# a1q123456/image_stitching

Hardware: AMD Instinct MI355X
Metric: 4K frames stitched/sec (higher is better)
Workload: dtype u8

## Files before the change

### host/job.cpp

```cpp
#include "job.hpp"
#include <cstring>

namespace mis {

StitchJob::StitchJob(int device, int width, int height, const std::vector<CameraParams>& cameras, const StitchConfig& cfg)
    : JobCore("mis::StitchJob", "", device, nullptr, width, height, cameras, cfg) {}

StitchJob::~StitchJob() {
    mis_image_free(cctx_, &pano_);
    mis_image_free(cctx_, &mask_);
}

void StitchJob::finalize() {
    if (pano_.data && (pano_.width != key_.pano.width || pano_.height != key_.pano.height)) { mis_image_free(cctx_, &pano_); mis_image_free(cctx_, &mask_); pano_ = MisImage{}; mask_ = MisImage{}; }
    if (!pano_.data) { pano_ = MisImage{}; mask_ = MisImage{}; pano_.mem = mask_.mem = MIS_MEM_DEVICE; }
    check(cctx_, mis_blender_blend(blender_, &pano_, &mask_), "mis_blender_blend");
}

JobOutput StitchJob::run(const std::vector<MisImage>& frames) {
    if ((int)frames.size() != n_) throw std::runtime_error("StitchJob::run: one frame per camera");
    JobOutput out;
    check(cctx_, mis_context_wait(cctx_, ctx_), "mis_context_wait");
    const MisImage* work = work_frames(frames);
    prep_.arm([this] { if (spec_ok_) prepare(everyone_); });
    check(ctx_, mis_orb_on_enqueued(orb_, &Hook::fire, &prep_), "mis_orb_on_enqueued");
    std::vector<MisFeatures> feats(n_);
    std::memset(feats.data(), 0, sizeof(MisFeatures) * n_);
    const int rc_f = mis_orb_detect_batch(orb_, work, n_, feats.data());
    mis_orb_on_enqueued(orb_, nullptr, nullptr);
    check(ctx_, rc_f, "mis_orb_detect_batch");
    prep_.finish();
    for (int i = 0; i < n_; i++) { feats[i].img_idx = i; out.num_features.push_back(feats[i].n); }
    const MisMatchParams mp = reset_matches();
    match_.arm([this, &frames] {
        if (!spec_ok_) return;
        fence_knn();
        compose(frames, everyone_, everyone_);
        finalize();
    });
    check(ctx_, mis_match_on_enqueued(ctx_, &Hook::fire, &match_), "mis_match_on_enqueued");
    const int rc = mis_match_pairs_model(ctx_, feats.data(), n_, &mp, model_, nullptr, cfg_.range_width, 0, 1, pairwise_.data());
    mis_match_on_enqueued(ctx_, nullptr, nullptr);
    for (auto& f : feats) mis_features_free(ctx_, &f);
    check(ctx_, rc, "mis_match_pairs_model");
    match_.finish();
    out.confidence.resize((size_t)n_ * n_);
    for (int k = 0; k < n_ * n_; k++) out.confidence[k] = pairwise_[k].confidence;
    std::vector<int> idx(n_);
    int kept = 0;
    check(ctx_, mis_leave_biggest_component(pairwise_.data(), n_, cfg_.conf_thresh, idx.data(), &kept), "mis_leave_biggest_component");
    idx.resize(kept);
    if (kept < 2) throw std::runtime_error("Need more images");
    out.indices = idx;
    out.speculation_kept = spec_ok_ && kept == n_;
    if (!out.speculation_kept) {
        prepare(idx);
        compose(frames, everyone_, idx);
        finalize();
    }
    check(cctx_, mis_context_synchronize(cctx_), "mis_context_synchronize (compose)");
    out.pano = pano_; out.mask = mask_;
    out.num_bands = key_.bands; out.pano_width = key_.pano.width; out.pano_height = key_.pano.height;
    out.matches = pairwise_;
    return out;
}

}
```

### host/job_core.cpp

```cpp
#include "job_core.hpp"
#include <algorithm>
#include <numeric>

namespace mis {

static float median_focal(const std::vector<CameraParams>& cams, const std::vector<int>& idx) {
    std::vector<double> f;
    for (int i : idx) f.push_back(cams[i].focal);
    std::sort(f.begin(), f.end());
    return f.size() % 2 == 1 ? static_cast<float>(f[f.size() / 2]) : static_cast<float>(f[f.size() / 2 - 1] + f[f.size() / 2]) * 0.5f;
}

void JobCore::Hook::fire(void* self_) {
    Hook* self = static_cast<Hook*>(self_);
    self->ran_ = true;
    try { self->body_(); } catch (const std::exception& e) { self->error_ = e.what(); }
}

void JobCore::Hook::arm(std::function<void()> body) {
    body_ = std::move(body);
    ran_ = false;
    error_.clear();
}

void JobCore::Hook::finish() {
    if (!ran_) fire(this);
    if (!error_.empty()) throw std::runtime_error(error_);
}

void JobCore::check(MisContext* c, int rc, const char* what) const {
    if (rc != MIS_OK) throw std::runtime_error(std::string(what) + " failed" + where_ + ": " + mis_last_error(c));
}

JobCore::JobCore(const char* who, std::string where, int device, void* main_stream, int width, int height, const std::vector<CameraParams>& cameras,
                 const StitchConfig& cfg)
    : w_(width), h_(height), n_((int)cameras.size()), wg_(work_geometry(cfg, width, height)), cams_(cameras), cfg_(cfg), everyone_(n_), mstream_(main_stream),
      where_(std::move(where)) {
    std::iota(everyone_.begin(), everyone_.end(), 0);
    if (wg_.scale != 1.0) {
        for (auto& c : cams_) { c.focal *= wg_.scale; c.ppx *= wg_.scale; c.ppy *= wg_.scale; }
        compose_work_aspect_ = 1.0 / wg_.scale;
    }
    try {
        if (cfg_.features_type != "orb" || cfg_.ba_cost_func != "no" || cfg_.expos_comp_type != "no" || cfg_.seam_find_type != "no")
            throw std::runtime_error(std::string(who) + " runs the hot path (ORB, supplied cameras, no seam-scale step); use mis::Stitcher for the other options");
        kind_ = warp_kind(cfg_.warp_type);
        check_range_width(cfg_.range_width);
        model_ = matcher_model(cfg_.matcher_type, cfg_.range_width);
        if (mis_context_create(device, mstream_, &ctx_) != MIS_OK) throw std::runtime_error("mis_context_create failed: no HIP device (there is no CPU fallback)");
        check(ctx_, mis_stream_create(device, 0, &cstream_), "mis_stream_create");
        if (mis_context_create(device, cstream_, &cctx_) != MIS_OK) throw std::runtime_error("mis_context_create (compose stream) failed");
        MisOrbParams op;
        mis_orb_default_params(&op);
        check(ctx_, mis_orb_create(ctx_, &op, wg_.width, wg_.height, &orb_), "mis_orb_create");
    } catch (...) {
        release();
        throw;
    }
    Ks_.resize((size_t)n_ * 9); Rs_.resize((size_t)n_ * 9);
    for (int i = 0; i < n_; i++) {
        CameraParams cc = cams_[i];
        if (compose_work_aspect_ != 1.0) { cc.focal *= compose_work_aspect_; cc.ppx *= compose_work_aspect_; cc.ppy *= compose_work_aspect_; }
        const Mat3<float> K = cc.K().cast<float>(), R = cams_[i].R.cast<float>();
        std::copy(K.m.begin(), K.m.end(), Ks_.begin() + 9 * i);
        std::copy(R.m.begin(), R.m.end(), Rs_.begin() + 9 * i);
    }
    if (kind_ != MIS_WARP_SPHERICAL) {
        const float scale = warp_scale(everyone_);
        MisRect r;
        if (MIS_WARP_ROI_IS_FULL_SCAN(kind_)) {
            std::vector<MisRect> rr((size_t)n_);
            spec_ok_ = n_ == 0 || mis_warper_roi_batch(cctx_, kind_, scale, w_, h_, n_, Ks_.data(), Rs_.data(), rr.data()) == MIS_OK;
        } else
            for (int i = 0; i < n_ && spec_ok_; i++) spec_ok_ = mis_warper_roi(kind_, scale, w_, h_, &Ks_[9 * i], &Rs_[9 * i], &r) == MIS_OK;
    }
}

JobCore::~JobCore() { release(); }

float JobCore::warp_scale(const std::vector<int>& idx) const {
    const float scale = median_focal(cams_, idx);
    return compose_work_aspect_ != 1.0 ? scale * static_cast<float>(compose_work_aspect_) : scale;
}

const MisImage* JobCore::work_frames(const std::vector<MisImage>& frames) {
    if (wg_.scale == 1.0 || frames.empty()) return frames.data();
    if (work_.size() < frames.size()) work_.resize(frames.size(), MisImage{});
    check(ctx_, mis_resize_linear_exact_batch(ctx_, frames.data(), (int)frames.size(), 0, 0, wg_.scale, wg_.scale, work_.data()), "mis_resize_linear_exact_batch");
    return work_.data();
}

void JobCore::release() {
    if (cctx_) mis_context_synchronize(cctx_);
    if (ctx_) mis_context_synchronize(ctx_);
    if (!pairwise_.empty()) mis_matches_free(pairwise_.data(), (int)pairwise_.size());
    if (ctx_) for (auto& im : work_) mis_image_free(ctx_, &im);
    if (blender_) mis_blender_destroy(blender_);
    if (orb_) mis_orb_destroy(orb_);
    if (cctx_) mis_context_destroy(cctx_);
    if (ctx_) mis_context_destroy(ctx_);
    if (cstream_) mis_stream_destroy(cstream_);
    if (mstream_) mis_stream_destroy(mstream_);
}

void JobCore::synchronize() {
    check(ctx_, mis_context_synchronize(ctx_), "mis_context_synchronize");
    check(cctx_, mis_context_synchronize(cctx_), "mis_context_synchronize (compose)");
}

JobCore::Compose JobCore::prepare(const std::vector<int>& idx) {
    const int m = (int)idx.size();
    const float scale = warp_scale(idx);
    std::vector<float> Ks((size_t)m * 9), Rs((size_t)m * 9);
    for (int k = 0; k < m; k++) {
        std::copy(Ks_.begin() + 9 * idx[k], Ks_.begin() + 9 * idx[k] + 9, Ks.begin() + 9 * k);
        std::copy(Rs_.begin() + 9 * idx[k], Rs_.begin() + 9 * idx[k] + 9, Rs.begin() + 9 * k);
    }
    rois_.assign(m, MisRect{});
    check(cctx_, mis_warper_roi_batch(cctx_, kind_, scale, w_, h_, m, Ks.data(), Rs.data(), rois_.data()), "mis_warper_roi_batch");
    std::vector<MisPoint> corners(m);
    std::vector<MisSize> sizes(m);
    for (int k = 0; k < m; k++) { corners[k] = {rois_[k].x, rois_[k].y}; sizes[k] = {rois_[k].width, rois_[k].height}; }
    Compose c;
    check(cctx_, mis_result_roi(corners.data(), sizes.data(), m, &c.pano), "mis_result_roi");
    check(cctx_, mis_blend_config(cfg_.blend_type, cfg_.blend_strength, c.pano.width, c.pano.height, &c.type, &c.bands, &c.sharp), "mis_blend_config");
    if (!blender_ || c.type != key_.type || c.bands != key_.bands || c.sharp != key_.sharp) {
        if (blender_) { mis_blender_destroy(blender_); blender_ = nullptr; }
        check(cctx_, mis_blender_create(cctx_, c.type, c.bands, c.sharp, &blender_), "mis_blender_create");
    }
    key_ = c;
    check(cctx_, mis_blender_prepare(blender_, corners.data(), sizes.data(), m), "mis_blender_prepare");
    return c;
}

void JobCore::fence_knn() {
    const int rc = mis_match_knn_fence(ctx_, cstream_, mis_match_sequence(ctx_), 0);
    if (rc < 0) check(ctx_, rc, "mis_match_knn_fence");
}

void JobCore::compose(const std::vector<MisImage>& frames, const std::vector<int>& frame_ids, const std::vector<int>& idx) {
    std::vector<MisImage> fr;
    std::vector<float> Ks, Rs;
    std::vector<MisRect> rois;
    for (size_t q = 0; q < frame_ids.size(); q++) {
        const auto it = std::find(idx.begin(), idx.end(), frame_ids[q]);
        if (it == idx.end()) continue;
        fr.push_back(frames[q]);
        Ks.insert(Ks.end(), Ks_.begin() + 9 * frame_ids[q], Ks_.begin() + 9 * frame_ids[q] + 9);
        Rs.insert(Rs.end(), Rs_.begin() + 9 * frame_ids[q], Rs_.begin() + 9 * frame_ids[q] + 9);
        rois.push_back(rois_[it - idx.begin()]);
    }
    if (fr.empty()) return;
    check(cctx_, mis_compose_frames_kind(blender_, kind_, fr.data(), (int)fr.size(), warp_scale(idx), Ks.data(), Rs.data(), rois.data()),
          "mis_compose_frames_kind");
}

MisMatchParams JobCore::reset_matches() {
    if (!pairwise_.empty()) { mis_matches_free(pairwise_.data(), (int)pairwise_.size()); pairwise_.clear(); }
    pairwise_.assign((size_t)n_ * n_, MisMatchesInfo{});
    return match_params(model_, cfg_.match_conf);
}

}
```

### host/job_core.hpp

```cpp
#pragma once
#include <functional>
#include <string>
#include <vector>
#include "stitcher.hpp"

namespace mis {

struct JobOutput {
    std::vector<int> indices;
    std::vector<double> confidence;
    std::vector<int> num_features;
    MisImage pano{}, mask{};
    int num_bands = 0, pano_width = 0, pano_height = 0;
    bool speculation_kept = false;
    std::vector<MisMatchesInfo> matches;
};

class JobCore {
protected:
    struct Compose { int type = 0, bands = 0; float sharp = 0; MisRect pano{}; };

    class Hook {
    public:
        static void fire(void* self);
        void arm(std::function<void()> body);
        void finish();
    private:
        std::function<void()> body_;
        bool ran_ = false;
        std::string error_;
    };

    JobCore(const char* who, std::string where, int device, void* main_stream, int width, int height, const std::vector<CameraParams>& cameras,
            const StitchConfig& cfg);
    ~JobCore();
    JobCore(const JobCore&) = delete;
    JobCore& operator=(const JobCore&) = delete;

    void check(MisContext* c, int rc, const char* what) const;
    void synchronize();
    Compose prepare(const std::vector<int>& idx);
    void fence_knn();
    const MisImage* work_frames(const std::vector<MisImage>& frames);
    float warp_scale(const std::vector<int>& idx) const;
    void compose(const std::vector<MisImage>& frames, const std::vector<int>& frame_ids, const std::vector<int>& idx);
    MisMatchParams reset_matches();

    int w_, h_, n_;
    WorkGeometry wg_;
    double compose_work_aspect_ = 1;
    std::vector<CameraParams> cams_;
    std::vector<MisImage> work_;
    StitchConfig cfg_;
    std::vector<int> everyone_;
    int kind_ = MIS_WARP_SPHERICAL;
    int model_ = MIS_MATCH_HOMOGRAPHY;
    bool spec_ok_ = true;
    void* mstream_ = nullptr;
    void* cstream_ = nullptr;
    MisContext* ctx_ = nullptr;
    MisContext* cctx_ = nullptr;
    MisOrb* orb_ = nullptr;
    MisBlender* blender_ = nullptr;
    Compose key_{};
    std::vector<float> Ks_, Rs_;
    std::vector<MisRect> rois_;
    std::vector<MisMatchesInfo> pairwise_;

private:
    void release();
    std::string where_;
};

}
```

### host/sharded_job.cpp

```cpp
#include "sharded_job.hpp"
#include <hip/hip_runtime_api.h>
#include <algorithm>
#include <cstring>
#include <numeric>

namespace mis {

std::vector<int> frame_block(int n, int rank, int world) {
    const int base = n / world, rem = n % world;
    const int lo = rank * base + std::min(rank, rem), cnt = base + (rank < rem ? 1 : 0);
    std::vector<int> out(cnt);
    std::iota(out.begin(), out.end(), lo);
    return out;
}

void* ShardedJob::reserve(DevBuf& b, size_t bytes) {
    bytes = std::max<size_t>(bytes, 256);
    if (b.bytes < bytes) {
        if (b.p) (void)hipFree(b.p);
        b.p = nullptr; b.bytes = 0;
        if (hipMalloc(&b.p, bytes) != hipSuccess) throw std::runtime_error("hipMalloc of an exchange buffer failed");
        b.bytes = bytes;
    }
    return b.p;
}

static void* new_stream(int device) {
    void* s = nullptr;
    if (mis_stream_create(device, 0, &s) != MIS_OK) throw std::runtime_error("mis_stream_create failed: no HIP device (there is no CPU fallback)");
    return s;
}

ShardedJob::ShardedJob(int device, int width, int height, const std::vector<CameraParams>& cameras, Communicator& comm, const StitchConfig& cfg)
    : JobCore("mis::ShardedJob", " on rank " + std::to_string(comm.rank()), device, new_stream(device), width, height, cameras, cfg), comm_(comm) {
    if (n_ % comm_.world() != 0) throw std::runtime_error("the frame count must divide evenly over the ranks");
    mine_ = frame_block(n_, comm_.rank(), comm_.world());
    send_.resize(comm_.world()); recv_.resize(comm_.world());
}

ShardedJob::~ShardedJob() {
    for (DevBuf* b : {&kps_send_, &desc_send_, &kps_all_, &desc_all_, &strip_mine_, &strips_all_, &pano_buf_, &mask_buf_}) if (b->p) (void)hipFree(b->p);
    for (auto& b : send_) if (b.p) (void)hipFree(b.p);
    for (auto& b : recv_) if (b.p) (void)hipFree(b.p);
}

void ShardedJob::prepare_multi_band(const std::vector<int>& idx) {
    if (prepare(idx).type != MIS_BLEND_MULTI_BAND) throw std::runtime_error("mis::ShardedJob exchanges the multi-band blender's pyramids");
}

void ShardedJob::exchange_finalize(const std::vector<int>& idx) {
    const int world = comm_.world(), me = comm_.rank(), bands = key_.bands;
    std::vector<int> lw(bands + 1), lh(bands + 1);
    for (int l = 0; l <= bands; l++) check(cctx_, mis_blender_level_info(blender_, l, &lw[l], &lh[l], nullptr, nullptr), "mis_blender_level_info");
    const int w0 = lw[0], h0 = lh[0];
    const int q = 1 << bands, nq = w0 / q;
    std::vector<std::pair<int, int>> bounds(world);
    for (int k = 0; k < world; k++) bounds[k] = {(int)((long long)k * nq / world) * q, k + 1 < world ? (int)((long long)(k + 1) * nq / world) * q : w0};
    std::vector<std::vector<std::pair<int, int>>> need(world);
    for (int k = 0; k < world; k++) {
        int lo = bounds[k].first, hi = bounds[k].second;
        need[k].push_back({lo, hi});
        for (int l = 1; l <= bands; l++) { lo = std::max(0, (lo >> 1) - 1); hi = std::min(lw[l], ((hi - 1) >> 1) + 2); need[k].push_back({lo, hi}); }
    }
    int px = 1 << 30, py = 1 << 30;
    for (size_t k = 0; k < idx.size(); k++) { px = std::min(px, rois_[k].x); py = std::min(py, rois_[k].y); }
    struct Region { bool any; int x0, y0, x1, y1; };
    std::vector<Region> region(world);
    const int gap = 3 << bands, a = q - 1;
    for (int r = 0; r < world; r++) {
        Region g{false, 1 << 30, 1 << 30, -(1 << 30), -(1 << 30)};
        for (int i : frame_block(n_, r, world)) {
            const auto it = std::find(idx.begin(), idx.end(), i);
            if (it == idx.end()) continue;
            const MisRect& rc = rois_[it - idx.begin()];
            g.any = true;
            g.x0 = std::min(g.x0, rc.x); g.y0 = std::min(g.y0, rc.y); g.x1 = std::max(g.x1, rc.x + rc.width); g.y1 = std::max(g.y1, rc.y + rc.height);
        }
        if (g.any) {
            g.x0 = std::max(0, g.x0 - px - gap) & ~a; g.y0 = std::max(0, g.y0 - py - gap) & ~a;
            g.x1 = std::min(w0, (g.x1 - px + gap + a) & ~a); g.y1 = std::min(h0, (g.y1 - py + gap + a) & ~a);
        }
        region[r] = g;
    }
    auto rects_of = [&](int src, int dst, std::vector<MisLevelRect>& out) -> size_t {
        out.clear();
        size_t off = 0;
        const Region& g = region[src];
        if (!g.any) return 0;
        for (int l = 0; l <= bands; l++) {
            const int x0 = std::max(std::min(g.x0 >> l, lw[l]), need[dst][l].first), x1 = std::min(std::min(-((-g.x1) >> l), lw[l]), need[dst][l].second);
            const int y0 = std::min(g.y0 >> l, lh[l]), y1 = std::min(-((-g.y1) >> l), lh[l]);
            if (x1 <= x0 || y1 <= y0) continue;
            const size_t m = (size_t)(x1 - x0) * (y1 - y0);
            out.push_back(MisLevelRect{l, x0, y0, x1, y1, (unsigned long long)off});
            off += (m * 6 + 15) / 16 * 16 + (m * 4 + 15) / 16 * 16;
        }
        return off;
    };
    std::vector<MisLevelRect> rects;
    std::vector<const void*> sp(world);
    std::vector<void*> rp(world);
    std::vector<size_t> sb(world), rb(world);
    for (int k = 0; k < world; k++) {
        sb[k] = rects_of(me, k, rects);
        sp[k] = reserve(send_[k], sb[k]);
        if (!rects.empty()) check(cctx_, mis_blender_pack_rects(blender_, rects.data(), (int)rects.size(), send_[k].p, send_[k].bytes), "mis_blender_pack_rects");
        rb[k] = rects_of(k, me, rects);
        rp[k] = reserve(recv_[k], rb[k]);
    }
    comm_.all_to_all(sp.data(), sb.data(), rp.data(), rb.data(), cstream_);
    std::vector<MisLevelRect> full;
    for (int l = 0; l <= bands; l++)
        if (need[me][l].second > need[me][l].first) full.push_back(MisLevelRect{l, need[me][l].first, 0, need[me][l].second, lh[l], 0ull});
    if (!full.empty()) check(cctx_, mis_blender_zero_rects(blender_, full.data(), (int)full.size()), "mis_blender_zero_rects");
    for (int r = 0; r < world; r++) {
        rects_of(r, me, rects);
        if (!rects.empty()) check(cctx_, mis_blender_add_rects(blender_, rects.data(), (int)rects.size(), recv_[r].p, recv_[r].bytes), "mis_blender_add_rects");
    }
    const int pw = key_.pano.width, ph = key_.pano.height;
    int cap_w = 0;
    for (int k = 0; k < world; k++) cap_w = std::max(cap_w, std::min(bounds[k].second, pw) - bounds[k].first);
    cap_w = std::max(cap_w, 1);
    const size_t strip_bytes = (size_t)ph * cap_w * 7;
    uint8_t* mine = (uint8_t*)reserve(strip_mine_, strip_bytes);
    const int x0 = bounds[me].first, x1 = std::min(bounds[me].second, pw);
    if (x1 > x0) {
        MisImage img{mine, x1 - x0, ph, 3, (size_t)cap_w * 6, MIS_S16, MIS_MEM_DEVICE};
        MisImage msk{mine + (size_t)ph * cap_w * 6, x1 - x0, ph, 1, (size_t)cap_w, MIS_U8, MIS_MEM_DEVICE};
        check(cctx_, mis_blender_blend_columns(blender_, x0, x1, &img, &msk), "mis_blender_blend_columns");
    }
    uint8_t* all = (uint8_t*)reserve(strips_all_, strip_bytes * world);
    comm_.all_gather(mine, all, strip_bytes, cstream_);
    uint8_t* pano = (uint8_t*)reserve(pano_buf_, (size_t)ph * pw * 6);
    uint8_t* mask = (uint8_t*)reserve(mask_buf_, (size_t)ph * pw);
    for (int k = 0; k < world; k++) {
        const int b0 = bounds[k].first, b1 = std::min(bounds[k].second, pw);
        if (b1 <= b0) continue;
        const uint8_t* base = all + (size_t)k * strip_bytes;
        check(cctx_, mis_copy_2d(cctx_, pano + (size_t)b0 * 6, (size_t)pw * 6, base, (size_t)cap_w * 6, (size_t)(b1 - b0) * 6, ph), "mis_copy_2d");
        check(cctx_, mis_copy_2d(cctx_, mask + b0, (size_t)pw, base + (size_t)ph * cap_w * 6, (size_t)cap_w, (size_t)(b1 - b0), ph), "mis_copy_2d");
    }
    pano_ = MisImage{pano, pw, ph, 3, (size_t)pw * 6, MIS_S16, MIS_MEM_DEVICE};
    mask_ = MisImage{mask, pw, ph, 1, (size_t)pw, MIS_U8, MIS_MEM_DEVICE};
}

JobOutput ShardedJob::run(const std::vector<MisImage>& frames) {
    const int m = (int)mine_.size(), world = comm_.world();
    if ((int)frames.size() != m) throw std::runtime_error("ShardedJob::run: one frame per camera of this rank's block");
    JobOutput out;
    check(cctx_, mis_context_wait(cctx_, ctx_), "mis_context_wait");
    const MisImage* work = work_frames(frames);
    prep_.arm([this] { if (spec_ok_) prepare_multi_band(everyone_); });
    check(ctx_, mis_orb_on_enqueued(orb_, &Hook::fire, &prep_), "mis_orb_on_enqueued");
    std::vector<MisFeatures> local(m);
    std::memset(local.data(), 0, sizeof(MisFeatures) * m);
    const int rc_f = m > 0 ? mis_orb_detect_batch(orb_, work, m, local.data()) : MIS_OK;
    mis_orb_on_enqueued(orb_, nullptr, nullptr);
    check(ctx_, rc_f, "mis_orb_detect_batch");
    prep_.finish();
    std::vector<int> cnt_mine(m), cnt_all(n_);
    for (int k = 0; k < m; k++) cnt_mine[k] = local[k].n;
    comm_.all_gather_host(cnt_mine.data(), cnt_all.data(), sizeof(int) * m);
    const int cap = std::max(1, *std::max_element(cnt_all.begin(), cnt_all.end()));
    const size_t kb = (size_t)cap * sizeof(MisKeyPoint), db = (size_t)cap * 32;
    reserve(kps_send_, kb * m); reserve(desc_send_, db * m); reserve(kps_all_, kb * n_); reserve(desc_all_, db * n_);
    if (m > 0) check(ctx_, mis_features_pack(ctx_, local.data(), m, cap, 32, kps_send_.p, desc_send_.p), "mis_features_pack");
    comm_.all_gather(kps_send_.p, kps_all_.p, kb * m, mstream_);
    comm_.all_gather(desc_send_.p, desc_all_.p, db * m, mstream_);
    std::vector<MisFeatures> feats(n_);
    for (int i = 0; i < n_; i++) {
        MisFeatures& f = feats[i];
        f.img_idx = i; f.img_w = wg_.width; f.img_h = wg_.height; f.n = cnt_all[i];
        f.keypoints = reinterpret_cast<MisKeyPoint*>((uint8_t*)kps_all_.p + kb * i);
        f.descriptors = (uint8_t*)desc_all_.p + db * i;
        f.desc_cols = 32; f.desc_dtype = MIS_U8; f.owner_ = nullptr;
    }
    out.num_features = cnt_all;
    const MisMatchParams mp = reset_matches();
    match_.arm([this, &frames] {
        if (!spec_ok_) return;
        fence_knn();
        compose(frames, mine_, everyone_);
    });
    check(ctx_, mis_match_on_enqueued(ctx_, &Hook::fire, &match_), "mis_match_on_enqueued");
    const int rc = mis_match_pairs_model(ctx_, feats.data(), n_, &mp, model_, nullptr, cfg_.range_width, comm_.rank(), world, pairwise_.data());
    mis_match_on_enqueued(ctx_, nullptr, nullptr);
    for (auto& f : local) mis_features_free(ctx_, &f);
    check(ctx_, rc, "mis_match_pairs_model");
    match_.finish();
    out.confidence.resize((size_t)n_ * n_);
    for (int k = 0; k < n_ * n_; k++) out.confidence[k] = pairwise_[k].confidence;
    comm_.all_reduce_sum_host(out.confidence.data(), out.confidence.size());
    std::vector<int> idx(n_);
    int kept = 0;
    check(ctx_, mis_leave_biggest_component_conf(out.confidence.data(), n_, cfg_.conf_thresh, idx.data(), &kept), "mis_leave_biggest_component_conf");
    idx.resize(kept);
    if (kept < 2) throw std::runtime_error("Need more images");
    out.indices = idx;
    out.speculation_kept = spec_ok_ && kept == n_;
    if (!out.speculation_kept) {
        prepare_multi_band(idx);
        compose(frames, mine_, idx);
    }
    exchange_finalize(idx);
    check(cctx_, mis_context_synchronize(cctx_), "mis_context_synchronize (compose)");
    out.pano = pano_; out.mask = mask_;
    out.num_bands = key_.bands; out.pano_width = key_.pano.width; out.pano_height = key_.pano.height;
    return out;
}

}
```

### image_stitching_amd/_capi.py

```python
import ctypes as C
import os
import re

_HERE = os.path.dirname(os.path.abspath(__file__))
LIB_PATH = os.path.join(_HERE, "libmistitch.so")
HEADER_PATH = os.path.join(os.path.dirname(_HERE), "include", "mistitch.h")

MIS_OK = 0
MIS_FENCE_TIMEOUT = 1
MEM_HOST, MEM_DEVICE = 0, 1
U8, S16, F32 = 0, 1, 2
INTER_NEAREST, INTER_LINEAR = 0, 1
BORDER_CONSTANT, BORDER_REFLECT = 0, 2
BLEND_NO, BLEND_FEATHER, BLEND_MULTI_BAND = 0, 1, 2
WARP_SPHERICAL, WARP_CYLINDRICAL, WARP_PLANE, WARP_MERCATOR, WARP_FISHEYE, WARP_STEREOGRAPHIC = 0, 1, 2, 3, 4, 5


def roi_is_full_scan(kind):
    return WARP_MERCATOR <= kind <= WARP_STEREOGRAPHIC


MATH_LOG, MATH_TAN, MATH_SINH, MATH_ASIN, MATH_ATAN, MATH_EXP = 0, 1, 2, 3, 4, 5
MATCH_HOMOGRAPHY, MATCH_AFFINE_PARTIAL = 0, 1
EXPOS_NO, EXPOS_GAIN, EXPOS_GAIN_BLOCKS, EXPOS_CHANNELS, EXPOS_CHANNELS_BLOCKS = 0, 1, 2, 3, 4


class MisPoint(C.Structure):
    _fields_ = [("x", C.c_int), ("y", C.c_int)]


class MisSize(C.Structure):
    _fields_ = [("width", C.c_int), ("height", C.c_int)]


class MisRect(C.Structure):
    _fields_ = [("x", C.c_int), ("y", C.c_int), ("width", C.c_int), ("height", C.c_int)]


class MisLevelRect(C.Structure):
    _fields_ = [("level", C.c_int), ("x0", C.c_int), ("y0", C.c_int), ("x1", C.c_int), ("y1", C.c_int), ("offset", C.c_ulonglong)]


class MisImage(C.Structure):
    _fields_ = [("data", C.c_void_p), ("width", C.c_int), ("height", C.c_int), ("channels", C.c_int),
                ("stride", C.c_size_t), ("dtype", C.c_int), ("mem", C.c_int)]


class MisKeyPoint(C.Structure):
    _fields_ = [("x", C.c_float), ("y", C.c_float), ("size", C.c_float), ("angle", C.c_float),
                ("response", C.c_float), ("octave", C.c_int)]


class MisOrbParams(C.Structure):
    _fields_ = [("nfeatures", C.c_int), ("scale_factor", C.c_float), ("nlevels", C.c_int),
                ("edge_threshold", C.c_int), ("first_level", C.c_int), ("wta_k", C.c_int),
                ("score_type", C.c_int), ("patch_size", C.c_int), ("fast_threshold", C.c_int)]


class MisSiftParams(C.Structure):
    _fields_ = [("nfeatures", C.c_int), ("n_octave_layers", C.c_int), ("contrast_threshold", C.c_double),
                ("edge_threshold", C.c_double), ("sigma", C.c_double)]


class MisCameraParams(C.Structure):
    _fields_ = [("focal", C.c_double), ("aspect", C.c_double), ("ppx", C.c_double), ("ppy", C.c_double), ("R", C.c_double * 9),
                ("t", C.c_double * 3)]


class MisFeatures(C.Structure):
    _fields_ = [("img_idx", C.c_int), ("img_w", C.c_int), ("img_h", C.c_int), ("n", C.c_int),
                ("keypoints", C.c_void_p), ("descriptors", C.c_void_p), ("desc_cols", C.c_int),
                ("desc_dtype", C.c_int), ("owner_", C.c_void_p)]


class MisMatchParams(C.Structure):
    _fields_ = [("match_conf", C.c_float), ("num_matches_thresh1", C.c_int), ("num_matches_thresh2", C.c_int),
                ("ransac_thresh", C.c_double), ("max_iters", C.c_int), ("confidence", C.c_double)]


class MisCompensatorParams(C.Structure):
    _fields_ = [("type", C.c_int), ("nr_feeds", C.c_int), ("block_width", C.c_int), ("block_height", C.c_int),
                ("nr_gain_filtering_iterations", C.c_int)]


class MisDMatch(C.Structure):
    _fields_ = [("query_idx", C.c_int), ("train_idx", C.c_int), ("img_idx", C.c_int), ("distance", C.c_float)]


class MisMatchesInfo(C.Structure):
    _fields_ = [("src_img_idx", C.c_int), ("dst_img_idx", C.c_int), ("n_matches", C.c_int),
                ("matches", C.POINTER(MisDMatch)), ("inliers_mask", C.POINTER(C.c_uint8)), ("num_inliers", C.c_int),
                ("has_H", C.c_int), ("H", C.c_double * 9), ("confidence", C.c_double)]


_vp, _i, _f, _d = C.c_void_p, C.c_int, C.c_float, C.c_double
_P = C.POINTER

PROTOTYPES = {
    "mis_context_create": (_i, [_i, _vp, _P(_vp)]),
    "mis_stream_create": (_i, [_i, _i, _P(_vp)]),
    "mis_stream_destroy": (_i, [_vp]),
    "mis_context_destroy": (_i, [_vp]),
    "mis_context_synchronize": (_i, [_vp]),
    "mis_context_wait": (_i, [_vp, _vp]),
    "mis_last_error": (C.c_char_p, [_vp]),
    "mis_version": (C.c_char_p, []),
    "mis_image_free": (_i, [_vp, _P(MisImage)]),
    "mis_orb_default_params": (None, [_P(MisOrbParams)]),
    "mis_orb_create": (_i, [_vp, _P(MisOrbParams), _i, _i, _P(_vp)]),
    "mis_orb_destroy": (_i, [_vp]),
    "mis_orb_detect": (_i, [_vp, _P(MisImage), _P(MisFeatures)]),
    "mis_orb_detect_batch": (_i, [_vp, _P(MisImage), _i, _P(MisFeatures)]),
    "mis_orb_on_enqueued": (_i, [_vp, _vp, _vp]),
    "mis_features_download": (_i, [_vp, _P(MisFeatures), _vp, _vp]),
    "mis_features_upload": (_i, [_vp, _i, _i, _i, _vp, _vp, _i, _i, _P(MisFeatures)]),
    "mis_features_free": (_i, [_vp, _P(MisFeatures)]),
    "mis_orb_debug_level": (_i, [_vp, _i, _i, _vp, _P(_i), _P(_i)]),
    "mis_sift_default_params": (None, [_P(MisSiftParams)]),
    "mis_sift_create": (_i, [_vp, _P(MisSiftParams), _i, _i, _P(_vp)]),
    "mis_sift_destroy": (_i, [_vp]),
    "mis_sift_detect": (_i, [_vp, _P(MisImage), _P(MisFeatures)]),
    "mis_sift_detect_batch": (_i, [_vp, _P(MisImage), _i, _P(MisFeatures)]),
    "mis_sift_debug_level": (_i, [_vp, _P(MisImage), _i, _i, _i, _vp, _P(_i), _P(_i)]),
    "mis_sift_debug_counts": (_i, [_vp, _P(C.c_uint)]),
    "mis_match_default_params": (None, [_P(MisMatchParams)]),
    "mis_match_all_pairs": (_i, [_vp, _P(MisFeatures), _i, _P(MisMatchParams), _P(MisMatchesInfo)]),
    "mis_match_pairs_sharded": (_i, [_vp, _P(MisFeatures), _i, _P(MisMatchParams), _i, _i, _P(MisMatchesInfo)]),
    "mis_match_pairs_select": (_i, [_vp, _P(MisFeatures), _i, _P(MisMatchParams), _vp, _i, _i, _i, _P(MisMatchesInfo)]),
    "mis_match_affine_default_params": (None, [_P(MisMatchParams)]),
    "mis_match_pairs_model": (_i, [_vp, _P(MisFeatures), _i, _P(MisMatchParams), _i, _vp, _i, _i, _i, _P(MisMatchesInfo)]),
    "mis_estimate_affine_partial": (_i, [_vp, _vp, _vp, _i, _d, _i, _d, _i, _vp, _vp, _P(_i)]),
    "mis_matches_free": (_i, [_P(MisMatchesInfo), _i]),
    "mis_match_sequence": (C.c_longlong, [_vp]),
    "mis_match_knn_fence": (_i, [_vp, _vp, C.c_longlong, _i]),
    "mis_match_on_enqueued": (_i, [_vp, _vp, _vp]),
    "mis_knn2": (_i, [_vp, _P(MisFeatures), _P(MisFeatures), _vp, _vp]),
    "mis_find_homography": (_i, [_vp, _vp, _vp, _i, _d, _i, _d, _vp, _vp, _P(_i)]),
    "mis_leave_biggest_component": (_i, [_P(MisMatchesInfo), _i, _f, _vp, _P(_i)]),
    "mis_leave_biggest_component_conf": (_i, [_vp, _i, _f, _vp, _P(_i)]),
    "mis_bundle_adjust_reproj": (_i, [_vp, _P(MisFeatures), _P(MisMatchesInfo), _i, _f, C.c_char_p, _P(MisCameraParams)]),
    "mis_wave_correct": (_i, [_vp, _i, _i]),
    "mis_warp_roi": (_i, [_f, _i, _i, _vp, _vp, _P(MisRect)]),
    "mis_warp_spherical": (_i, [_vp, _P(MisImage), _f, _vp, _vp, _i, _i, _P(MisImage), _P(MisPoint)]),
    "mis_warp_roi_batch": (_i, [_vp, _f, _i, _i, _i, _vp, _vp, _P(MisRect)]),
    "mis_warp_spherical_fused_roi": (_i, [_vp, _P(MisImage), _f, _vp, _vp, _P(MisRect), _P(MisImage), _P(MisImage), _P(MisPoint)]),
    "mis_warp_spherical_fused_batch": (_i, [_vp, _P(MisImage), _i, C.c_float, _P(C.c_float), _P(C.c_float), _P(MisRect), _P(MisImage), _P(MisImage), _P(MisPoint)]),
    "mis_warp_spherical_fused_batch_timed": (_i, [_vp, _P(MisImage), _i, C.c_float, _P(C.c_float), _P(C.c_float), _P(MisRect), _P(MisImage), _P(MisImage), _P(MisPoint), _i,
                                               _P(C.c_float)]),
    "mis_debug_math_f32": (_i, [_vp, _i, _vp, _vp, _i]),
    "mis_warper_roi": (_i, [_i, _f, _i, _i, _vp, _vp, _P(MisRect)]),
    "mis_warper_roi_batch": (_i, [_vp, _i, _f, _i, _i, _i, _vp, _vp, _P(MisRect)]),
    "mis_warper_warp": (_i, [_vp, _i, _P(MisImage), _f, _vp, _vp, _i, _i, _P(MisImage), _P(MisPoint)]),
    "mis_warper_warp_roi": (_i, [_vp, _i, _P(MisImage), _f, _vp, _vp, _P(MisRect), _i, _i, _P(MisImage), _P(MisPoint)]),
    "mis_warper_warp_fused": (_i, [_vp, _i, _P(MisImage), _f, _vp, _vp, _P(MisImage), _P(MisImage), _P(MisPoint)]),
    "mis_warper_warp_fused_roi": (_i, [_vp, _i, _P(MisImage), _f, _vp, _vp, _P(MisRect), _P(MisImage), _P(MisImage), _P(MisPoint)]),
    "mis_warper_warp_fused_batch": (_i, [_vp, _i, _P(MisImage), _i, C.c_float, _P(C.c_float), _P(C.c_float), _P(MisRect), _P(MisImage), _P(MisImage), _P(MisPoint)]),
    "mis_warp_spherical_fused": (_i, [_vp, _P(MisImage), _f, _vp, _vp, _P(MisImage), _P(MisImage), _P(MisPoint)]),
    "mis_resize_linear_exact": (_i, [_vp, _P(MisImage), _i, _i, C.c_double, C.c_double, _P(MisImage)]),
    "mis_resize_linear_exact_batch": (_i, [_vp, _P(MisImage), _i, _i, _i, C.c_double, C.c_double, _P(MisImage)]),
    "mis_rotate": (_i, [_vp, _P(MisImage), _i, _P(MisImage)]),
    "mis_seam_mask_apply": (_i, [_vp, _P(MisImage), _P(MisImage)]),
    "mis_compensator_create": (_i, [_vp, _i, _i, _i, _P(_vp)]),
    "mis_compensator_default_params": (None, [_P(MisCompensatorParams)]),
    "mis_compensator_create_ex": (_i, [_vp, _P(MisCompensatorParams), _P(_vp)]),
    "mis_compensator_destroy": (_i, [_vp]),
    "mis_compensator_gains": (_i, [_vp, _i, _P(_d)]),
    "mis_compensator_gain_map_channels": (_i, [_vp, _i, _P(C.c_float), _i, _P(_i), _P(_i), _P(_i)]),
    "mis_compensator_debug_stats": (_i, [_vp, _i, _i, _i, _P(_i), _P(_d), _P(_d)]),
    "mis_compensator_feed": (_i, [_vp, _P(MisPoint), _P(MisImage), _P(MisImage), _i]),
    "mis_compensator_gain_map": (_i, [_vp, _i, _P(C.c_float), _i, _P(_i), _P(_i)]),
    "mis_compensator_apply": (_i, [_vp, _i, _P(MisImage)]),
    "mis_seam_voronoi": (_i, [_vp, _P(MisPoint), _P(MisImage), _i]),
    "mis_seam_dp": (_i, [_vp, _P(MisPoint), _P(MisImage), _P(MisImage), _i, _i]),
    "mis_warp_spherical_fused_timed": (_i, [_vp, _P(MisImage), _f, _vp, _vp, _P(MisImage), _P(MisImage), _P(MisPoint), _i, _P(C.c_float)]),
    "mis_blend_config": (_i, [_i, _f, _i, _i, _P(_i), _P(_i), _P(_f)]),
    "mis_result_roi": (_i, [_P(MisPoint), _P(MisSize), _i, _P(MisRect)]),
    "mis_blender_create": (_i, [_vp, _i, _i, _f, _P(_vp)]),
    "mis_blender_destroy": (_i, [_vp]),
    "mis_blender_prepare": (_i, [_vp, _P(MisPoint), _P(MisSize), _i]),
    "mis_blender_num_bands": (_i, [_vp]),
    "mis_blender_feed": (_i, [_vp, _P(MisImage), _P(MisImage), MisPoint]),
    "mis_blender_feed_batch": (_i, [_vp, _P(MisImage), _P(MisImage), _P(MisPoint), _i]),
    "mis_blender_blend": (_i, [_vp, _P(MisImage), _P(MisImage)]),
    "mis_compose_frames": (_i, [_vp, _P(MisImage), _i, _f, _vp, _vp, _P(MisRect)]),
    "mis_compose_frames_kind": (_i, [_vp, _i, _P(MisImage), _i, _f, _vp, _vp, _P(MisRect)]),
    "mis_blender_blend_columns": (_i, [_vp, _i, _i, _P(MisImage), _P(MisImage)]),
    "mis_blender_pack_rects": (_i, [_vp, _P(MisLevelRect), _i, _vp, C.c_size_t]),
    "mis_blender_add_rects": (_i, [_vp, _P(MisLevelRect), _i, _vp, C.c_size_t]),
    "mis_blender_zero_rects": (_i, [_vp, _P(MisLevelRect), _i]),
    "mis_features_pack": (_i, [_vp, _P(MisFeatures), _i, _i, _i, _vp, _vp]),
    "mis_copy_2d": (_i, [_vp, _vp, C.c_size_t, _vp, C.c_size_t, C.c_size_t, C.c_size_t]),
    "mis_blender_feed_rect": (_i, [_vp, _i, _i, MisPoint, _P(MisRect)]),
    "mis_blender_level_info": (_i, [_vp, _i, _P(_i), _P(_i), _P(_vp), _P(_vp)]),
}


def header_functions():
    txt = open(HEADER_PATH).read()
    txt = re.sub(r"/\*.*?\*/", "", txt, flags=re.S)
    return sorted(set(re.findall(r"\b(mis_[a-z0-9_]+)\s*\(", txt)))


_lib = None


def load():
    global _lib
    if _lib is not None:
        return _lib
    if not os.path.exists(LIB_PATH):
        raise ImportError("libmistitch.so is not built (%s missing): run `python -c 'import __graft_entry__ as g; g.build()'` "
                          "or `make -C image_stitching_amd/csrc`; there is no CPU fallback" % LIB_PATH)
    lib = C.CDLL(LIB_PATH)
    for name, (res, args) in PROTOTYPES.items():
        fn = getattr(lib, name)
        fn.restype = res
        fn.argtypes = args
    _lib = lib
    return lib
```

### image_stitching_amd/csrc/blend.hip

```cpp
#include "common.h"
#include "dev_math.h"
#include <algorithm>
#include <cmath>
#include <utility>
#include <vector>

#define MIS_MAX_BANDS 16

struct MisBlender {
    MisContext* ctx = nullptr;
    int type = MIS_BLEND_MULTI_BAND, actual_bands = 5, num_bands = 0;
    float sharpness = 0.02f;
    MisRect roi{0, 0, 0, 0};
    int fw = 0, fh = 0;
    int lw[MIS_MAX_BANDS + 1], lh[MIS_MAX_BANDS + 1];
    int16_t* lap[MIS_MAX_BANDS + 1];
    float* wgt[MIS_MAX_BANDS + 1];
    uint8_t* dst_mask = nullptr;
    void* pano_mem = nullptr;
    size_t pano_bytes = 0;
    bool prepared = false;
    bool fresh = false;
    void* scratch = nullptr;
    size_t scratch_bytes = 0;
};

namespace {

constexpr float WEIGHT_EPS = 1e-5f;
#ifndef FEED_TAIL_PIXELS_N
#define FEED_TAIL_PIXELS_N 8192
#endif
constexpr size_t FEED_TAIL_PIXELS = FEED_TAIL_PIXELS_N;

__device__ __forceinline__ int16_t sat_s16(int v) { return (int16_t)(v < -32768 ? -32768 : (v > 32767 ? 32767 : v)); }

struct FrameView {
    const int16_t* img;
    size_t istride;
    const uint8_t* mask;
    size_t mstride;
    int w, h;
    int left, top;
    int tw, th;
};

__device__ __forceinline__ int reflect101_near(int p, int len) {
    if ((unsigned)(p + len - 1) < (unsigned)(3 * len - 2)) { const int a = p < 0 ? -p : p; return a >= len ? 2 * len - 2 - a : a; }
    return mis_reflect101(p, len);
}
__device__ __forceinline__ int reflect_near(int p, int len) {
    if ((unsigned)(p + len) < (unsigned)(3 * len)) return mis_reflect1(p, len);
    return mis_reflect(p, len);
}

__device__ __forceinline__ void view_px(const FrameView& v, int tx, int ty, int* c) {
    const int16_t* p = v.img + (size_t)reflect_near(ty - v.top, v.h) * v.istride + 3 * (size_t)reflect_near(tx - v.left, v.w);
    c[0] = p[0]; c[1] = p[1]; c[2] = p[2];
}
__device__ __forceinline__ float view_w(const FrameView& v, int tx, int ty) {
    int x = tx - v.left, y = ty - v.top;
    if ((unsigned)x >= (unsigned)v.w || (unsigned)y >= (unsigned)v.h) return 0.f;
    return (float)v.mask[(size_t)y * v.mstride + x] * (float)(1. / 255.);
}

template <bool OK>
__device__ __forceinline__ void load_px3_t(const int16_t* __restrict__ row, int p, int* c) {
    if (OK) {
        const int e = 3 * p;
        const uint2 d = *reinterpret_cast<const uint2*>(row + (e & ~1));
        const unsigned sh = (unsigned)(e & 1) << 4;
        const unsigned lo = __builtin_amdgcn_alignbit(d.y, d.x, sh);
        c[0] = (int)(int16_t)(unsigned short)lo; c[1] = (int)lo >> 16; c[2] = (int)(int16_t)(unsigned short)(d.y >> sh);
    } else {
        c[0] = row[3 * p]; c[1] = row[3 * p + 1]; c[2] = row[3 * p + 2];
    }
}
__device__ __forceinline__ void load_px3(const int16_t* __restrict__ row, int p, bool ok, int* c) {
    if (ok) load_px3_t<true>(row, p, c); else load_px3_t<false>(row, p, c);
}

constexpr int PD_W = 32, PD_H = 16, PD_SW = 2 * PD_W + 3, PD_SH = 2 * PD_H + 3;

constexpr int PDV_ROW_DW = 104;
static_assert(PDV_ROW_DW * 2 >= 7 + 3 * PD_SW && PDV_ROW_DW % 4 == 0, "an LDS row holds the footprint from any 16-byte phase");
constexpr int PDV_MROW_B = 96;
constexpr int PDV_MROW_DW = (PD_SW + 3 + 3) / 4 + 1;
__device__ __forceinline__ void pd_dma16(const void* base, unsigned voff, uint32_t lds_off) {
    asm volatile("s_mov_b32 m0, %2\n\ts_nop 0\n\tglobal_load_lds_dwordx4 %0, %1" ::"v"(voff), "s"(base), "s"(lds_off) : "memory", "m0");
}

template <bool FROM_VIEW>
__device__ __forceinline__ void pyr_down_view_tile(const FrameView& v, const int16_t* __restrict__ src, const float* __restrict__ wsrc, int psw, int psh,
                                                   int16_t* __restrict__ dst, float* __restrict__ wdst, int dw, int dh, int bx, int by) {
    constexpr int WT_BYTES = (int)sizeof(float) * PD_SH * PD_SW;
    static_assert(WT_BYTES <= (int)sizeof(int16_t) * PD_SH * PDV_ROW_DW * 2, "the weights fit the spent image tile");
    __shared__ __attribute__((aligned(16))) int16_t tile[PD_SH * PDV_ROW_DW * 2];
    __shared__ __attribute__((aligned(16))) uint8_t wmem[FROM_VIEW ? PD_SH * PDV_MROW_B : WT_BYTES];
    __shared__ int vbuf[PD_H * PDV_ROW_DW];
    __shared__ int sflag;
    uint8_t* const mraw = wmem;
    float* const wt = FROM_VIEW ? reinterpret_cast<float*>(tile) : reinterpret_cast<float*>(wmem);
    int moff = 0;
    bool rowchk = false;
    unsigned wide_bits = 0;
    int wconst = 0;
    const int x0 = bx * PD_W, y0 = by * PD_H, t = threadIdx.x;
    const int sw = FROM_VIEW ? v.tw : psw, sh = FROM_VIEW ? v.th : psh;
    const int tx0 = 2 * x0 - 2, ty0 = 2 * y0 - 2;
    const int ix0 = tx0 - v.left, iy0 = ty0 - v.top;
    const bool interior = FROM_VIEW && tx0 >= 0 && ty0 >= 0 && tx0 + PD_SW <= sw && ty0 + PD_SH <= sh && ix0 >= 0 && iy0 >= 0 && ix0 + PD_SW + 12 <= v.w && iy0 + PD_SH <= v.h &&
                          (v.istride & 1) == 0 && ((uintptr_t)v.img & 3) == 0 && (v.mstride & 3) == 0 && ((uintptr_t)v.mask & 3) == 0;
    int toff;
    bool dma = false, mir = false;
    int cs = ix0;
    if (FROM_VIEW && tx0 >= 0 && ty0 >= 0 && tx0 + PD_SW <= sw && ty0 + PD_SH <= sh) {
        bool cols = true;
        if (ix0 >= 0 && ix0 + PD_SW <= v.w) cs = ix0;
        else if (ix0 + PD_SW <= 0 && -ix0 <= v.w) { cs = -ix0 - PD_SW; mir = true; }
        else if (ix0 >= v.w && 2 * v.w - PD_SW - ix0 >= 0) { cs = 2 * v.w - PD_SW - ix0; mir = true; }
        else cols = false;
        const size_t ia = ((size_t)3 * cs * 2) & ~(size_t)15, ma = (size_t)cs & ~(size_t)15;
        dma = cols && (((uintptr_t)v.img | (v.istride * 2)) & 15) == 0 && ia + PDV_ROW_DW * 4 <= v.istride * 2 && (size_t)v.h * v.istride * 2 < (1ull << 32) &&
              (mir || ((((uintptr_t)v.mask | v.mstride) & 15) == 0 && ma + PDV_MROW_B <= v.mstride && (size_t)v.h * v.mstride < (1ull << 32)));
        if (!dma) mir = false;
    }
    if (dma) {
        const size_t ib = (size_t)3 * cs * 2, ia = ib & ~(size_t)15;
        toff = (int)((ib - ia) >> 1);
        moff = cs & 15;
        rowchk = true;
        const uint8_t* ibase = reinterpret_cast<const uint8_t*>(v.img) + ia;
        const uint8_t* mbase = v.mask + ((size_t)cs & ~(size_t)15);
        const uint32_t tile_lds = (uint32_t)(uintptr_t)(__attribute__((address_space(3))) void*)tile;
        const uint32_t mraw_lds = (uint32_t)(uintptr_t)(__attribute__((address_space(3))) void*)mraw;
        const int wave = __builtin_amdgcn_readfirstlane(t >> 6), lane = t & 63;
        constexpr int IPR = PDV_ROW_DW / 4, IP = PD_SH * IPR, MPR = PDV_MROW_B / 16, MP = PD_SH * MPR;
#pragma unroll
        for (int k = 0; k < (IP + 255) / 256; k++) {
            const int p0 = (k * 4 + wave) * 64, p = p0 + lane;
            if (p0 < IP) {
                const int r = min(p / IPR, PD_SH - 1), c = p - r * IPR;
                const int iy = reflect_near(iy0 + r, v.h);
                if (p < IP) pd_dma16(ibase, (unsigned)iy * (unsigned)(v.istride * 2) + (unsigned)c * 16u, tile_lds + (uint32_t)p0 * 16u);
            }
        }
        if (!mir) {
            const int p0 = wave * 64, p = p0 + lane;
            if (p0 < MP) {
                const int r = min(p / MPR, PD_SH - 1), c = p - r * MPR;
                const int iy = min(max(iy0 + r, 0), v.h - 1);
                if (p < MP) pd_dma16(mbase, (unsigned)iy * (unsigned)v.mstride + (unsigned)c * 16u, mraw_lds + (uint32_t)p0 * 16u);
            }
        }
        if (t == 0) sflag = 0;
        asm volatile("s_waitcnt vmcnt(0)" ::: "memory");
        __syncthreads();
        unsigned all1 = mir ? 0u : 0xffffffffu, any = 0u, wide = 0u;
        if (!mir) {
            for (int i = t; i < PD_SH * (PDV_MROW_B / 4); i += 256) {
                const int r = i / (PDV_MROW_B / 4), c = i - r * (PDV_MROW_B / 4);
                const bool row_in = (unsigned)(iy0 + r) < (unsigned)v.h;
                const unsigned d = row_in ? reinterpret_cast<const unsigned*>(mraw)[i] : 0u;
                unsigned in = 0u;
#pragma unroll
                for (int q = 0; q < 4; q++) in |= ((unsigned)(4 * c + q - moff) < (unsigned)PD_SW) ? (0xffu << (8 * q)) : 0u;
                all1 &= d | ~in;
                any |= d & in;
            }
        }
        const int td0 = toff >> 1;
        constexpr int FDW = (3 * PD_SW + 1) / 2 + 1;
        for (int i = t; i < PD_SH * FDW; i += 256) {
            const int r = i / FDW, c = i - r * FDW;
            wide |= reinterpret_cast<const unsigned*>(tile)[r * PDV_ROW_DW + td0 + c];
        }
        const int bits = (__any(all1 != 0xffffffffu) ? 1 : 0) | (__any(any != 0u) ? 2 : 0) | (__any((wide & 0xFF00FF00u) != 0u) ? 4 : 0);
// ... 603 lines not shown
    int16_t* d = (int16_t*)((uint8_t*)dst + (size_t)y * dstride) + 3 * (size_t)x;
    d[0] = m ? s[0] : (int16_t)0; d[1] = m ? s[1] : (int16_t)0; d[2] = m ? s[2] : (int16_t)0;
    dmask[(size_t)y * mstride + x] = (uint8_t)m;
}

__global__ __launch_bounds__(256) void feed_plain_kernel(const int16_t* img, size_t istride, const uint8_t* mask, size_t mstride, int w, int h,
                                                         int16_t* dst, uint8_t* dmask, int pw, int dx, int dy) {
    int x = blockIdx.x * 64 + (threadIdx.x & 63), y = blockIdx.y * 4 + (threadIdx.x >> 6);
    if (x >= w || y >= h) return;
    unsigned m = mask[(size_t)y * mstride + x];
    size_t o = (size_t)(dy + y) * pw + dx + x;
    if (m) {
        const int16_t* s = img + (size_t)y * istride + 3 * (size_t)x;
        dst[o * 3] = s[0]; dst[o * 3 + 1] = s[1]; dst[o * 3 + 2] = s[2];
    }
    dmask[o] |= (uint8_t)m;
}

constexpr int FT_INF = 8192, FT_PX = 16, FT_TB = 256, FS_SEG = 32, FT_MAXCHUNK = 16;

__device__ __forceinline__ int wave_scan_max_incl(int v) {
#pragma unroll
    for (int d = 1; d < 64; d <<= 1) { const int o = __shfl_up(v, d); if ((int)(threadIdx.x & 63) >= d) v = max(v, o); }
    return v;
}
__device__ __forceinline__ int wave_scan_min_incl_rev(int v) {
#pragma unroll
    for (int d = 1; d < 64; d <<= 1) { const int o = __shfl_down(v, d); if ((int)(threadIdx.x & 63) + d < 64) v = min(v, o); }
    return v;
}

__global__ __launch_bounds__(FT_TB) void feather_rows_kernel(const uint8_t* __restrict__ mask, size_t mstride, int w, int h, uint16_t* __restrict__ g, int gp) {
    __shared__ int s_last[FT_TB / 64], s_first[FT_TB / 64], s_cfirst[FT_MAXCHUNK];
    const int y = blockIdx.x, t = threadIdx.x, lane = t & 63, wv = t >> 6;
    const uint8_t* row = mask + (size_t)y * mstride;
    uint16_t* grow = g + (size_t)y * gp;
    const bool vec_in = (((uintptr_t)mask | mstride) & 15) == 0;
    constexpr int NONE_L = -(1 << 20), NONE_R = 1 << 20;
    const int nchunk = (w + FT_TB * FT_PX - 1) / (FT_TB * FT_PX);
    if (nchunk > 1) {
        for (int c = t; c < FT_MAXCHUNK; c += FT_TB) s_cfirst[c] = NONE_R;
        __syncthreads();
        for (int c = 1; c < nchunk; c++) {
            const int x0 = c * FT_TB * FT_PX + t * FT_PX;
            int first = NONE_R;
            for (int i = FT_PX - 1; i >= 0; i--) if (x0 + i < w && row[x0 + i] == 0) first = x0 + i;
            first = wave_scan_min_incl_rev(first);
            if (lane == 0 && first != NONE_R) atomicMin(&s_cfirst[c], first);
        }
        __syncthreads();
    }
    int carry_last = NONE_L;
    for (int c = 0; c < nchunk; c++) {
        const int x0 = c * FT_TB * FT_PX + t * FT_PX;
        unsigned m[FT_PX];
        if (vec_in && x0 + FT_PX <= w) {
            const uint4 q = *reinterpret_cast<const uint4*>(row + x0);
            const unsigned qq[4] = {q.x, q.y, q.z, q.w};
#pragma unroll
            for (int i = 0; i < FT_PX; i++) m[i] = (qq[i >> 2] >> (8 * (i & 3))) & 255u;
        } else {
#pragma unroll
            for (int i = 0; i < FT_PX; i++) m[i] = x0 + i < w ? row[x0 + i] : 1u;
        }
        int last = NONE_L, first = NONE_R;
#pragma unroll
        for (int i = 0; i < FT_PX; i++) if (m[i] == 0 && x0 + i < w) { last = x0 + i; first = min(first, x0 + i); }
        int il = wave_scan_max_incl(last), ir = wave_scan_min_incl_rev(first);
        if (lane == 63) s_last[wv] = il;
        if (lane == 0) s_first[wv] = ir;
        __syncthreads();
        int before = carry_last, behind = NONE_R;
        for (int k = 0; k < wv; k++) before = max(before, s_last[k]);
        for (int k = wv + 1; k < FT_TB / 64; k++) behind = min(behind, s_first[k]);
        const int pl = __shfl_up(il, 1), pr = __shfl_down(ir, 1);
        if (lane > 0) before = max(before, pl);
        if (lane < 63) behind = min(behind, pr);
        int chunk_last = carry_last;
        for (int k = 0; k < FT_TB / 64; k++) chunk_last = max(chunk_last, s_last[k]);
        for (int k = c + 1; k < nchunk; k++) behind = min(behind, s_cfirst[k]);
        __syncthreads();
        carry_last = chunk_last;
        int lz = before;
        int dl[FT_PX];
#pragma unroll
        for (int i = 0; i < FT_PX; i++) { if (m[i] == 0) lz = x0 + i; dl[i] = min(x0 + i - lz, FT_INF); }
        int rz = behind;
        unsigned out[FT_PX];
#pragma unroll
        for (int i = FT_PX - 1; i >= 0; i--) { if (m[i] == 0) rz = x0 + i; out[i] = (unsigned)min(dl[i], min(rz - (x0 + i), FT_INF)); }
        if (x0 + FT_PX <= w && (gp & 7) == 0) {
            uint4 o0, o1;
            o0.x = out[0] | (out[1] << 16); o0.y = out[2] | (out[3] << 16); o0.z = out[4] | (out[5] << 16); o0.w = out[6] | (out[7] << 16);
            o1.x = out[8] | (out[9] << 16); o1.y = out[10] | (out[11] << 16); o1.z = out[12] | (out[13] << 16); o1.w = out[14] | (out[15] << 16);
            reinterpret_cast<uint4*>(grow + x0)[0] = o0; reinterpret_cast<uint4*>(grow + x0)[1] = o1;
        } else {
#pragma unroll
            for (int i = 0; i < FT_PX; i++) if (x0 + i < w) grow[x0 + i] = (uint16_t)out[i];
        }
    }
}

__global__ __launch_bounds__(FT_TB) void feather_colseg_kernel(const uint16_t* __restrict__ g, int gp, int w, int h, uint16_t* __restrict__ F, uint16_t* __restrict__ B) {
    const int x = blockIdx.x * FT_TB + threadIdx.x, s = blockIdx.y;
    if (x >= w) return;
    const int y0 = s * FS_SEG, n = min(FS_SEG, h - y0);
    int f = FT_INF, b = FT_INF;
    unsigned v[FS_SEG];
#pragma unroll
    for (int i = 0; i < FS_SEG; i++) v[i] = g[(size_t)min(y0 + i, h - 1) * gp + x];
#pragma unroll
    for (int i = 0; i < FS_SEG; i++) if (i < n) { f = min(f + 1, (int)v[i]); b = min(b, (int)v[i] + i); }
    F[(size_t)s * w + x] = (uint16_t)min(f, FT_INF);
    B[(size_t)s * w + x] = (uint16_t)min(b, FT_INF);
}

__global__ __launch_bounds__(FT_TB) void feather_feed_kernel(const uint16_t* __restrict__ g, int gp, const uint16_t* __restrict__ F, const uint16_t* __restrict__ B, int nseg,
                                                            const int16_t* __restrict__ img, size_t istride, int w, int h, float sharpness,
                                                            int16_t* __restrict__ dst, float* __restrict__ dwgt, int pw, int dx, int dy) {
    const int x = blockIdx.x * FT_TB + threadIdx.x, s = blockIdx.y;
    if (x >= w) return;
    const int y0 = s * FS_SEG, n = min(FS_SEG, h - y0);
    int cf = FT_INF, cb = FT_INF;
    for (int k = 0; k < s; k++) cf = min((int)F[(size_t)k * w + x], cf + FS_SEG);
    for (int k = nseg - 1; k > s; k--) cb = min((int)B[(size_t)k * w + x], cb + min(FS_SEG, h - k * FS_SEG));
    cf = min(cf, FT_INF); cb = min(cb, FT_INF);
    int d[FS_SEG];
#pragma unroll
    for (int i = 0; i < FS_SEG; i++) d[i] = g[(size_t)min(y0 + i, h - 1) * gp + x];
    int run = cf;
#pragma unroll
    for (int i = 0; i < FS_SEG; i++) { run = min(run + 1, d[i]); d[i] = run; }
    run = cb;
#pragma unroll
    for (int i = FS_SEG - 1; i >= 0; i--) if (i < n) { run = min(run + 1, d[i]); d[i] = run; }
#pragma unroll
    for (int i = 0; i < FS_SEG; i++) {
        if (i >= n) break;
        const float wv0 = (float)min(d[i], FT_INF) * sharpness;
        const float wv = wv0 > 1.f ? 1.f : wv0;
        const int y = y0 + i;
        const size_t o = (size_t)(dy + y) * pw + dx + x;
        const int16_t* sp = img + (size_t)y * istride + 3 * (size_t)x;
        int16_t* dp = dst + o * 3;
        dp[0] = (int16_t)(dp[0] + (int16_t)((float)sp[0] * wv));
        dp[1] = (int16_t)(dp[1] + (int16_t)((float)sp[1] * wv));
        dp[2] = (int16_t)(dp[2] + (int16_t)((float)sp[2] * wv));
        dwgt[o] += wv;
    }
}

inline dim3 grid2d(int w, int h) { return dim3((w + 63) / 64, (h + 3) / 4); }

int release(MisBlender* b, bool free_memory) {
    MisContext* ctx = b->ctx;
    if (free_memory && b->pano_mem) {
        MIS_HIP(ctx, hipStreamSynchronize(ctx->stream));
        MIS_HIP(ctx, hipFree(b->pano_mem));
        b->pano_mem = nullptr; b->pano_bytes = 0;
    }
    b->prepared = false;
    return MIS_OK;
}

int ensure_scratch(MisBlender* b, size_t bytes) {
    MisContext* ctx = b->ctx;
    if (bytes <= b->scratch_bytes) return MIS_OK;
    if (b->scratch) {
        MIS_HIP(ctx, hipStreamSynchronize(ctx->stream));
        MIS_HIP(ctx, hipFree(b->scratch));
        b->scratch = nullptr; b->scratch_bytes = 0;
    }
    MIS_HIP(ctx, hipMalloc(&b->scratch, bytes));
    b->scratch_bytes = bytes;
    return MIS_OK;
}

void feed_tile_rect(const MisBlender* b, int w, int h, MisPoint tl, int* otnx, int* otny, int* owidth, int* oheight) {
    const int nb = b->num_bands, q = 1 << nb, gap = 3 * q;
    const MisRect& R = b->roi;
    int brx_roi = R.x + R.width, bry_roi = R.y + R.height;
    int tnx = std::max(R.x, tl.x - gap), tny = std::max(R.y, tl.y - gap);
    int bnx = std::min(brx_roi, tl.x + w + gap), bny = std::min(bry_roi, tl.y + h + gap);
    tnx = R.x + (((tnx - R.x) >> nb) << nb);
    tny = R.y + (((tny - R.y) >> nb) << nb);
    int width = bnx - tnx, height = bny - tny;
    width += (q - width % q) % q;
    height += (q - height % q) % q;
    bnx = tnx + width; bny = tny + height;
    int dy = std::max(bny - bry_roi, 0), dx = std::max(bnx - brx_roi, 0);
    tnx -= dx; tny -= dy;
    *otnx = tnx; *otny = tny; *owidth = width; *oheight = height;
}

int feed_multiband_batch(MisBlender* b, const MisImage* imgs, const DevView* dimg, const DevView* dmask, const MisPoint* tls, int n) {
    MisContext* ctx = b->ctx;
    const int nb = b->num_bands;
    const MisRect& R = b->roi;
    struct Frame { FrameView v; int x_tl, y_tl, view_ok; };
    std::vector<Frame> fr(n);
    int mtw = 0, mth = 0;
    for (int k = 0; k < n; k++) {
        const int w = imgs[k].width, h = imgs[k].height;
        int tnx, tny, width, height;
        feed_tile_rect(b, w, h, tls[k], &tnx, &tny, &width, &height);
        const int bnx = tnx + width, bny = tny + height;
        FrameView& v = fr[k].v;
        v.img = (const int16_t*)dimg[k].data; v.istride = dimg[k].stride / 2;
        v.mask = (const uint8_t*)dmask[k].data; v.mstride = dmask[k].stride;
        v.w = w; v.h = h; v.left = tls[k].x - tnx; v.top = tls[k].y - tny; v.tw = width; v.th = height;
        const int bottom = bny - tls[k].y - h, right = bnx - tls[k].x - w;
        MIS_CHECK(ctx, v.left >= 0 && v.top >= 0 && bottom >= 0 && right >= 0, MIS_E_INVALID, "frame %d does not fit the prepared panorama roi", k);
        fr[k].x_tl = tnx - R.x; fr[k].y_tl = tny - R.y;
        fr[k].view_ok = ((uintptr_t)v.img & 3) == 0 && (v.istride & 1) == 0 && v.istride >= (size_t)3 * w + 1;
        mtw = std::max(mtw, width); mth = std::max(mth, height);
    }
    dim3 blk(256);
    if (nb == 0) {
        b->fresh = false;
        for (int k = 0; k < n; k++)
            hipLaunchKernelGGL((laplace_accumulate_kernel<true, true>), grid2d(fr[k].v.tw, fr[k].v.th), blk, 0, ctx->stream, fr[k].v, nullptr, nullptr, fr[k].v.tw, fr[k].v.th,
                               (const int16_t*)nullptr, 0, 0, b->lap[0], b->wgt[0], b->lw[0], fr[k].x_tl, fr[k].y_tl);
        MIS_HIP(ctx, hipGetLastError());
        return MIS_OK;
    }
    FeedLayout lay;
    lay.nb = nb;
    size_t region = 0;
    {
        int tw = mtw, th = mth;
        for (int i = 1; i <= nb; i++) {
            tw = (tw + 1) / 2; th = (th + 1) / 2;
            lay.goff[i] = region; region += mis_align_up((size_t)tw * th * 6, 256);
            lay.woff[i] = region; region += mis_align_up((size_t)tw * th * 4, 256);
        }
        lay.goff[0] = lay.woff[0] = 0;
    }
    int rc = ensure_scratch(b, region ? region * n : 256);
    if (rc != MIS_OK) return rc;
    int first = 0;
    for (int k = 0; k < n; k++) {
        int tw[MIS_MAX_BANDS + 1], th[MIS_MAX_BANDS + 1];
        tw[0] = fr[k].v.tw; th[0] = fr[k].v.th;
        for (int i = 1; i <= nb; i++) { tw[i] = (tw[i - 1] + 1) / 2; th[i] = (th[i - 1] + 1) / 2; }
        int f = nb + 1;
        for (int i = nb; i >= 2 && (size_t)tw[i] * th[i] <= FEED_TAIL_PIXELS; i--) f = i;
        if (f >= nb) f = nb + 1;
        first = std::max(first, f);
    }
    lay.first = first;
    for (int g0 = 0; g0 < n; g0 += FB_MAX) {
        const int ng = std::min(FB_MAX, n - g0);
        FeedBatch fb;
        fb.n = ng;
        int gtw = 0, gth = 0;
        for (int k = 0; k < ng; k++) {
            fb.v[k] = fr[g0 + k].v; fb.base[k] = (uint8_t*)b->scratch + (size_t)(g0 + k) * region;
            gtw = std::max(gtw, fb.v[k].tw); gth = std::max(gth, fb.v[k].th);
        }
        for (int k = ng; k < FB_MAX; k++) { fb.v[k] = fb.v[0]; fb.base[k] = fb.base[0]; }
        int lw = (gtw + 1) / 2, lh = (gth + 1) / 2;
        hipLaunchKernelGGL(pyr_down_l1_batch_kernel, dim3((lw + PD_W - 1) / PD_W, (lh + PD_H - 1) / PD_H, ng), blk, 0, ctx->stream, fb, lay);
        for (int i = 1; i < nb && i < first; i++) {
            lw = (lw + 1) / 2; lh = (lh + 1) / 2;
            hipLaunchKernelGGL(pyr_down_level_batch_kernel, dim3((lw + PD_W - 1) / PD_W, (lh + PD_H - 1) / PD_H, ng), blk, 0, ctx->stream, fb, lay, i);
        }
        if (first <= nb) hipLaunchKernelGGL(feed_tail_build_kernel, dim3(ng), dim3(1024), 0, ctx->stream, fb, lay);
    }
    for (int g0 = 0; g0 < n; g0 += FB_MAX) {
        const int ng = std::min(FB_MAX, n - g0);
        FeedGather ga;
        ga.n = ng; ga.nb = nb; ga.fresh = b->fresh ? 1 : 0;
        int x0 = INT32_MAX, y0 = INT32_MAX, x1 = INT32_MIN, y1 = INT32_MIN;
        for (int k = 0; k < FB_MAX; k++) {
            const Frame& f = fr[g0 + (k < ng ? k : 0)];
            ga.base[k] = (uint8_t*)b->scratch + (size_t)(g0 + (k < ng ? k : 0)) * region;
            ga.v[k] = f.v; ga.x_tl[k] = f.x_tl; ga.y_tl[k] = f.y_tl; ga.view_ok[k] = f.view_ok;
            if (k < ng) { x0 = std::min(x0, f.x_tl); y0 = std::min(y0, f.y_tl); x1 = std::max(x1, f.x_tl + f.v.tw); y1 = std::max(y1, f.y_tl + f.v.th); }
        }
        ga.bx0 = x0; ga.by0 = y0; ga.bw = x1 - x0; ga.bh = y1 - y0;
        int nblk = 0;
        for (int i = 0; i <= nb; i++) {
            ga.lap[i] = b->lap[i]; ga.wgt[i] = b->wgt[i]; ga.pw[i] = b->lw[i];
            ga.blk_off[i] = nblk;
            if (i < nb) nblk += (((ga.bw >> (i + 1)) + FG_BX - 1) / FG_BX) * (((ga.bh >> (i + 1)) + FG_BY - 1) / FG_BY);
            else nblk += ((ga.bw >> i) * (ga.bh >> i) + 255) / 256;
        }
        ga.blk_off[nb + 1] = nblk;
        hipLaunchKernelGGL(feed_gather_kernel, dim3(nblk), blk, 0, ctx->stream, ga, lay);
        b->fresh = false;
    }
    MIS_HIP(ctx, hipGetLastError());
    return MIS_OK;
}

int feed_feather(MisBlender* b, const DevView& dimg, const DevView& dmask, int w, int h, MisPoint tl) {
    MisContext* ctx = b->ctx;
    MIS_CHECK(ctx, w <= FT_MAXCHUNK * FT_TB * FT_PX, MIS_E_UNSUPPORTED, "feather blender: frames wider than %d pixels", FT_MAXCHUNK * FT_TB * FT_PX);
    const int gp = (w + 7) & ~7;
    const int nseg = (h + FS_SEG - 1) / FS_SEG;
    const size_t g_bytes = mis_align_up((size_t)gp * h * 2, 256), e_bytes = mis_align_up((size_t)nseg * w * 2, 256);
    int rc = ensure_scratch(b, g_bytes + 2 * e_bytes);
    if (rc != MIS_OK) return rc;
    uint16_t* g = (uint16_t*)b->scratch;
    uint16_t* F = (uint16_t*)((uint8_t*)b->scratch + g_bytes);
    uint16_t* B = (uint16_t*)((uint8_t*)b->scratch + g_bytes + e_bytes);
    hipLaunchKernelGGL(feather_rows_kernel, dim3(h), dim3(FT_TB), 0, ctx->stream, (const uint8_t*)dmask.data, dmask.stride, w, h, g, gp);
    const dim3 cg((w + FT_TB - 1) / FT_TB, nseg);
    hipLaunchKernelGGL(feather_colseg_kernel, cg, dim3(FT_TB), 0, ctx->stream, (const uint16_t*)g, gp, w, h, F, B);
    hipLaunchKernelGGL(feather_feed_kernel, cg, dim3(FT_TB), 0, ctx->stream, (const uint16_t*)g, gp, (const uint16_t*)F, (const uint16_t*)B, nseg,
                       (const int16_t*)dimg.data, dimg.stride / 2, w, h, b->sharpness, b->lap[0], b->wgt[0], b->lw[0], tl.x - b->roi.x, tl.y - b->roi.y);
    MIS_HIP(ctx, hipGetLastError());
    return MIS_OK;
}

}

extern "C" int mis_blend_config(int blend_type, float blend_strength, int pano_w, int pano_h, int* type_out, int* num_bands, float* sharpness) {
    if (!type_out || !num_bands || !sharpness) return MIS_E_INVALID;
    float blend_width = sqrtf((float)(pano_w * pano_h)) * blend_strength / 100.f;
    *num_bands = 0; *sharpness = 0.f; *type_out = blend_type;
    if (blend_width < 1.f) *type_out = MIS_BLEND_NO;
    else if (blend_type == MIS_BLEND_MULTI_BAND) *num_bands = (int)(ceil(logf(blend_width) / log(2.)) - 1.);
    else if (blend_type == MIS_BLEND_FEATHER) *sharpness = 1.f / blend_width;
    return MIS_OK;
}

extern "C" int mis_result_roi(const MisPoint* c, const MisSize* s, int n, MisRect* roi) {
    if (!c || !s || !roi || n < 1) return MIS_E_INVALID;
    int tlx = INT32_MAX, tly = INT32_MAX, brx = INT32_MIN, bry = INT32_MIN;
    for (int i = 0; i < n; i++) {
        tlx = std::min(tlx, c[i].x); tly = std::min(tly, c[i].y);
        brx = std::max(brx, c[i].x + s[i].width); bry = std::max(bry, c[i].y + s[i].height);
    }
    roi->x = tlx; roi->y = tly; roi->width = brx - tlx; roi->height = bry - tly;
    return MIS_OK;
}

extern "C" int mis_blender_create(MisContext* ctx, int type, int num_bands, float sharpness, MisBlender** out) {
    if (!ctx || !out) return MIS_E_INVALID;
    MIS_CHECK(ctx, type == MIS_BLEND_NO || type == MIS_BLEND_FEATHER || type == MIS_BLEND_MULTI_BAND, MIS_E_INVALID, "unknown blender type %d", type);
    MisBlender* b = new MisBlender();
    b->ctx = ctx; b->type = type; b->actual_bands = num_bands; b->sharpness = sharpness;
    for (int i = 0; i <= MIS_MAX_BANDS; i++) { b->lap[i] = nullptr; b->wgt[i] = nullptr; }
    *out = b;
    return MIS_OK;
}

extern "C" int mis_blender_destroy(MisBlender* b) {
    if (!b) return MIS_OK;
    hipSetDevice(b->ctx->device);
    release(b, true);
    if (b->scratch) { hipStreamSynchronize(b->ctx->stream); hipFree(b->scratch); }
    delete b;
    return MIS_OK;
}

extern "C" int mis_blender_num_bands(const MisBlender* b) { return b ? b->num_bands : MIS_E_INVALID; }

extern "C" int mis_blender_prepare(MisBlender* b, const MisPoint* corners, const MisSize* sizes, int n) {
    if (!b) return MIS_E_INVALID;
    MisContext* ctx = b->ctx;
    MIS_CHECK(ctx, corners && sizes && n >= 1, MIS_E_INVALID, "prepare needs at least one corner/size");
    MIS_HIP(ctx, hipSetDevice(ctx->device));
    int rc = release(b, false);
    if (rc != MIS_OK) return rc;
    mis_result_roi(corners, sizes, n, &b->roi);
    MIS_CHECK(ctx, b->roi.width > 0 && b->roi.height > 0, MIS_E_INVALID, "empty panorama roi");
    b->fw = b->roi.width; b->fh = b->roi.height;
    b->num_bands = 0;
    if (b->type == MIS_BLEND_MULTI_BAND) {
        double max_len = (double)std::max(b->roi.width, b->roi.height);
        b->num_bands = std::min(b->actual_bands, (int)ceil(log(max_len) / log(2.0)));
        MIS_CHECK(ctx, b->num_bands >= 0 && b->num_bands <= MIS_MAX_BANDS, MIS_E_INVALID, "number of bands %d out of range", b->num_bands);
        int q = 1 << b->num_bands;
        b->roi.width += (q - b->roi.width % q) % q;
        b->roi.height += (q - b->roi.height % q) % q;
    }
    b->lw[0] = b->roi.width; b->lh[0] = b->roi.height;
    for (int i = 1; i <= b->num_bands; i++) { b->lw[i] = (b->lw[i - 1] + 1) / 2; b->lh[i] = (b->lh[i - 1] + 1) / 2; }
    size_t total = 0, loff[MIS_MAX_BANDS + 1], woff[MIS_MAX_BANDS + 1], moff = 0;
    for (int i = 0; i <= b->num_bands; i++) {
        size_t px = (size_t)b->lw[i] * b->lh[i];
        loff[i] = total; total += mis_align_up(px * 6, 256);
        woff[i] = total; total += mis_align_up(px * 4, 256);
    }
    if (b->type == MIS_BLEND_NO) { moff = total; total += mis_align_up((size_t)b->lw[0] * b->lh[0], 256); }
    if (total > b->pano_bytes) {
        if ((rc = release(b, true)) != MIS_OK) return rc;
        MIS_HIP(ctx, hipMalloc(&b->pano_mem, total));
        b->pano_bytes = total;
    }
    MIS_HIP(ctx, hipMemsetAsync(b->pano_mem, 0, total, ctx->stream));
    for (int i = 0; i <= b->num_bands; i++) {
        b->lap[i] = (int16_t*)((uint8_t*)b->pano_mem + loff[i]);
        b->wgt[i] = (float*)((uint8_t*)b->pano_mem + woff[i]);
    }
    b->dst_mask = b->type == MIS_BLEND_NO ? (uint8_t*)b->pano_mem + moff : nullptr;
    b->prepared = true;
    b->fresh = true;
    return MIS_OK;
}

static int feed_check(MisBlender* b, const MisImage* img, const MisImage* mask, MisPoint tl) {
    MisContext* ctx = b->ctx;
    MIS_CHECK(ctx, img && mask && img->dtype == MIS_S16 && img->channels == 3 && mask->dtype == MIS_U8 && mask->channels == 1,
              MIS_E_INVALID, "feed needs a 16SC3 image and an 8U mask");
    MIS_CHECK(ctx, img->width == mask->width && img->height == mask->height, MIS_E_INVALID, "image / mask size mismatch");
    MIS_CHECK(ctx, tl.x >= b->roi.x && tl.y >= b->roi.y && tl.x + img->width <= b->roi.x + b->fw && tl.y + img->height <= b->roi.y + b->fh,
              MIS_E_INVALID, "frame at (%d,%d) %dx%d lies outside the prepared roi", tl.x, tl.y, img->width, img->height);
    MIS_CHECK(ctx, img->stride % 2 == 0, MIS_E_INVALID, "16SC3 stride must be even");
    return MIS_OK;
}

extern "C" int mis_blender_feed(MisBlender* b, const MisImage* img, const MisImage* mask, MisPoint tl) {
    if (!b) return MIS_E_INVALID;
    MisContext* ctx = b->ctx;
    MIS_CHECK(ctx, b->prepared, MIS_E_STATE, "feed before prepare");
    int rc = feed_check(b, img, mask, tl);
    if (rc != MIS_OK) return rc;
    MIS_HIP(ctx, hipSetDevice(ctx->device));
    DevView di, dm;
    if ((rc = di.read(ctx, img)) != MIS_OK || (rc = dm.read(ctx, mask)) != MIS_OK) return rc;
    const int w = img->width, h = img->height;
    if (b->type != MIS_BLEND_MULTI_BAND) b->fresh = false;
    if (b->type == MIS_BLEND_MULTI_BAND) rc = feed_multiband_batch(b, img, &di, &dm, &tl, 1);
    else if (b->type == MIS_BLEND_FEATHER) rc = feed_feather(b, di, dm, w, h, tl);
    else {
        hipLaunchKernelGGL(feed_plain_kernel, grid2d(w, h), dim3(256), 0, ctx->stream, (const int16_t*)di.data, di.stride / 2,
                           (const uint8_t*)dm.data, dm.stride, w, h, b->lap[0], b->dst_mask, b->lw[0], tl.x - b->roi.x, tl.y - b->roi.y);
        rc = hipGetLastError() == hipSuccess ? MIS_OK : mis_set_error(ctx, MIS_E_HIP, "feed_plain launch failed");
    }
    return rc;
}

extern "C" int mis_blender_feed_batch(MisBlender* b, const MisImage* imgs, const MisImage* masks, const MisPoint* tls, int n) {
    if (!b) return MIS_E_INVALID;
    MisContext* ctx = b->ctx;
    MIS_CHECK(ctx, b->prepared, MIS_E_STATE, "feed before prepare");
    MIS_CHECK(ctx, n >= 0 && (n == 0 || (imgs && masks && tls)), MIS_E_INVALID, "null argument");
    if (n == 0) return MIS_OK;
    if (b->type != MIS_BLEND_MULTI_BAND) {
        for (int k = 0; k < n; k++) { int rc = mis_blender_feed(b, &imgs[k], &masks[k], tls[k]); if (rc != MIS_OK) return rc; }
        return MIS_OK;
    }
    int rc = MIS_OK;
    for (int k = 0; k < n; k++) if ((rc = feed_check(b, &imgs[k], &masks[k], tls[k])) != MIS_OK) return rc;
    MIS_HIP(ctx, hipSetDevice(ctx->device));
    std::vector<DevView> di(n), dm(n);
    for (int k = 0; k < n; k++)
        if ((rc = di[k].read(ctx, &imgs[k])) != MIS_OK || (rc = dm[k].read(ctx, &masks[k])) != MIS_OK) return rc;
    return feed_multiband_batch(b, imgs, di.data(), dm.data(), tls, n);
}

extern "C" int mis_compose_frames_kind(MisBlender* b, int kind, const MisImage* frames, int n, float scale, const float* Ks, const float* Rs,
                                       const MisRect* rois) {
    if (!b) return MIS_E_INVALID;
    MisContext* ctx = b->ctx;
    MIS_CHECK(ctx, kind >= MIS_WARP_SPHERICAL && kind <= MIS_WARP_STEREOGRAPHIC, MIS_E_UNSUPPORTED, "unknown warp kind %d", kind);
    MIS_CHECK(ctx, b->prepared, MIS_E_STATE, "compose before prepare");
    MIS_CHECK(ctx, frames && Ks && Rs && rois && n >= 0, MIS_E_INVALID, "null argument");
    MIS_HIP(ctx, hipSetDevice(ctx->device));
    std::vector<MisImage> imgs(n), msks(n);
    std::vector<MisPoint> tls(n);
    std::vector<std::pair<void*, size_t>> blocks;
    int rc = MIS_OK;
    for (int i = 0; i < n && rc == MIS_OK; i++) {
        const MisRect& r = rois[i];
        if (!(r.width > 0 && r.height > 0)) { rc = mis_set_error(ctx, MIS_E_INVALID, "frame %d: empty warp roi", i); break; }
        const size_t ipitch = mis_align_up((size_t)r.width * 6 + 2, 256), mpitch = mis_align_up((size_t)r.width, 256);
        const size_t ibytes = ipitch * r.height, mbytes = mpitch * r.height;
        void* blk = nullptr; size_t got = 0;
        if ((rc = mis_pool_alloc(ctx, ibytes + mbytes, &blk, &got)) != MIS_OK) break;
        blocks.emplace_back(blk, got);
        imgs[i] = MisImage{blk, r.width, r.height, 3, ipitch, MIS_S16, MIS_MEM_DEVICE};
        msks[i] = MisImage{(uint8_t*)blk + ibytes, r.width, r.height, 1, mpitch, MIS_U8, MIS_MEM_DEVICE};
    }
    if (rc == MIS_OK && n > 0) rc = mis_warper_warp_fused_batch(ctx, kind, frames, n, scale, Ks, Rs, rois, imgs.data(), msks.data(), tls.data());
    if (rc == MIS_OK) rc = mis_blender_feed_batch(b, imgs.data(), msks.data(), tls.data(), n);
    for (auto& bl : blocks) mis_pool_free(ctx, bl.first, bl.second);
    return rc;
}

extern "C" int mis_compose_frames(MisBlender* b, const MisImage* frames, int n, float scale, const float* Ks, const float* Rs, const MisRect* rois) {
    return mis_compose_frames_kind(b, MIS_WARP_SPHERICAL, frames, n, scale, Ks, Rs, rois);
}

static int blend_columns(MisBlender* b, int x0, int x1, MisImage* dst, MisImage* dmask) {
    MisContext* ctx = b->ctx;
    MIS_CHECK(ctx, b->prepared, MIS_E_STATE, "blend before prepare");
    x1 = std::min(x1, b->fw);
    MIS_CHECK(ctx, x0 >= 0 && x0 < x1, MIS_E_INVALID, "empty column range %d..%d (panorama width %d)", x0, x1, b->fw);
    MIS_HIP(ctx, hipSetDevice(ctx->device));
    DevView dd, dm;
    int rc;
    if ((rc = dd.write(ctx, dst, x1 - x0, b->fh, 3, MIS_S16)) != MIS_OK) return rc;
    if ((rc = dm.write(ctx, dmask, x1 - x0, b->fh, 1, MIS_U8)) != MIS_OK) return rc;
    MIS_CHECK(ctx, dd.stride % 2 == 0, MIS_E_INVALID, "16SC3 stride must be even");
    const int nb = b->num_bands;
    if (b->type != MIS_BLEND_NO) {
        int lo[MIS_MAX_BANDS + 1], hi[MIS_MAX_BANDS + 1];
        lo[0] = x0; hi[0] = x1;
        for (int l = 1; l <= nb; l++) { lo[l] = std::max(0, (lo[l - 1] >> 1) - 1); hi[l] = std::min(b->lw[l], ((hi[l - 1] - 1) >> 1) + 2); }
        size_t n = (size_t)b->lw[nb] * b->lh[nb];
        hipLaunchKernelGGL(normalize_kernel, dim3((unsigned)((n + 255) / 256)), dim3(256), 0, ctx->stream, b->lap[nb], b->wgt[nb], n);
        for (int i = nb; i > 0; i--) {
            MIS_CHECK(ctx, b->lw[i - 1] == 2 * b->lw[i] && b->lh[i - 1] == 2 * b->lh[i], MIS_E_STATE, "pyramid level %d is not twice level %d", i - 1, i);
            const int cx0 = lo[i - 1] >> 1, cx1 = ((hi[i - 1] - 1) >> 1) + 1;
            if (i == 1) {
                const int vec = (b->lw[0] & 1) == 0 && (x0 & 1) == 0 && dd.stride % 4 == 0 && ((uintptr_t)dd.data & 3) == 0 && dm.stride % 2 == 0 && ((uintptr_t)dm.data & 1) == 0;
                hipLaunchKernelGGL(collapse2x2_final_kernel, grid2d(cx1 - cx0, b->lh[1]), dim3(256), 0, ctx->stream, (const int16_t*)b->lap[0], (const float*)b->wgt[0], b->lw[0],
                                   (const int16_t*)b->lap[1], b->lw[1], b->lh[1], cx0, cx1, x0, x1 - x0, b->fh, (int16_t*)dd.data, dd.stride, (uint8_t*)dm.data, dm.stride, vec);
                break;
            }
            hipLaunchKernelGGL(collapse2x2_kernel, grid2d(cx1 - cx0, b->lh[i]), dim3(256), 0, ctx->stream, b->lap[i - 1], b->wgt[i - 1], b->lw[i - 1], b->lh[i - 1],
                               (const int16_t*)b->lap[i], b->lw[i], b->lh[i], cx0, cx1);
        }
    }
    if (b->type == MIS_BLEND_NO || nb == 0)
    hipLaunchKernelGGL(finalize_kernel, grid2d(x1 - x0, b->fh), dim3(256), 0, ctx->stream, b->lap[0], b->wgt[0], b->dst_mask, b->lw[0], x1 - x0,
                       b->fh, (int16_t*)dd.data, dd.stride, (uint8_t*)dm.data, dm.stride, x0);
    MIS_HIP(ctx, hipGetLastError());
    if ((rc = dd.commit()) != MIS_OK || (rc = dm.commit()) != MIS_OK) return rc;
    b->prepared = false;
    return MIS_OK;
}

extern "C" int mis_blender_blend(MisBlender* b, MisImage* dst, MisImage* dmask) {
    if (!b) return MIS_E_INVALID;
    return blend_columns(b, 0, b->fw, dst, dmask);
}

extern "C" int mis_blender_blend_columns(MisBlender* b, int x0, int x1, MisImage* dst, MisImage* dmask) {
    if (!b) return MIS_E_INVALID;
    return blend_columns(b, x0, x1, dst, dmask);
}

struct RectBatch { int n; MisLevelRect r[MIS_MAX_BANDS + 1]; int16_t* lap[MIS_MAX_BANDS + 1]; float* wgt[MIS_MAX_BANDS + 1]; int pw[MIS_MAX_BANDS + 1]; };
template <int MODE>
__global__ __launch_bounds__(256) void rect_exchange_kernel(RectBatch rb, uint8_t* buf) {
    const MisLevelRect r = rb.r[blockIdx.z];
    const int w = r.x1 - r.x0, h = r.y1 - r.y0;
    const int y = blockIdx.y, x = blockIdx.x * 256 + threadIdx.x;
    if (y >= h) return;
    int16_t* lap = rb.lap[blockIdx.z] + ((size_t)(r.y0 + y) * rb.pw[blockIdx.z] + r.x0) * 3;
    float* wgt = rb.wgt[blockIdx.z] + (size_t)(r.y0 + y) * rb.pw[blockIdx.z] + r.x0;
    int16_t* bl = reinterpret_cast<int16_t*>(buf + r.offset) + (size_t)y * w * 3;
    float* bw = reinterpret_cast<float*>(buf + r.offset + (((size_t)w * h * 6 + 15) & ~(size_t)15)) + (size_t)y * w;
    if (x < 3 * w) {
        if (MODE == 0) bl[x] = lap[x];
        else if (MODE == 1) lap[x] = (int16_t)(lap[x] + bl[x]);
        else lap[x] = 0;
    }
    if (x < w) {
        if (MODE == 0) bw[x] = wgt[x];
        else if (MODE == 1) wgt[x] = wgt[x] + bw[x];
        else wgt[x] = 0.f;
    }
}

static int rect_exchange(MisBlender* b, const MisLevelRect* rects, int n, void* buf, size_t bytes, int mode) {
    if (b && mode == 1) b->fresh = false;
    if (!b) return MIS_E_INVALID;
    MisContext* ctx = b->ctx;
    MIS_CHECK(ctx, b->prepared && b->type != MIS_BLEND_NO, MIS_E_STATE, "no prepared accumulator pyramids");
    MIS_CHECK(ctx, rects && n >= 0 && (buf || mode == 2), MIS_E_INVALID, "null argument");
    MIS_HIP(ctx, hipSetDevice(ctx->device));
    for (int i0 = 0; i0 < n; i0 += MIS_MAX_BANDS + 1) {
        RectBatch rb;
        rb.n = std::min(n - i0, MIS_MAX_BANDS + 1);
        int maxw = 0, maxh = 0;
        for (int i = 0; i < rb.n; i++) {
            const MisLevelRect& r = rects[i0 + i];
            MIS_CHECK(ctx, r.level >= 0 && r.level <= b->num_bands && r.x0 >= 0 && r.y0 >= 0 && r.x0 <= r.x1 && r.y0 <= r.y1 && r.x1 <= b->lw[r.level] && r.y1 <= b->lh[r.level],
                      MIS_E_INVALID, "rectangle %d outside level %d", i0 + i, r.level);
            const size_t px = (size_t)(r.x1 - r.x0) * (r.y1 - r.y0);
            MIS_CHECK(ctx, mode == 2 || r.offset + ((px * 6 + 15) & ~(size_t)15) + ((px * 4 + 15) & ~(size_t)15) <= bytes, MIS_E_INVALID, "rectangle %d overruns the buffer", i0 + i);
            rb.r[i] = r; rb.lap[i] = b->lap[r.level]; rb.wgt[i] = b->wgt[r.level]; rb.pw[i] = b->lw[r.level];
            maxw = std::max(maxw, r.x1 - r.x0); maxh = std::max(maxh, r.y1 - r.y0);
        }
        if (maxw == 0 || maxh == 0) continue;
        const dim3 grid((3 * maxw + 255) / 256, maxh, rb.n);
        if (mode == 0) hipLaunchKernelGGL(rect_exchange_kernel<0>, grid, dim3(256), 0, ctx->stream, rb, (uint8_t*)buf);
        else if (mode == 1) hipLaunchKernelGGL(rect_exchange_kernel<1>, grid, dim3(256), 0, ctx->stream, rb, (uint8_t*)buf);
        else hipLaunchKernelGGL(rect_exchange_kernel<2>, grid, dim3(256), 0, ctx->stream, rb, (uint8_t*)buf);
    }
    MIS_HIP(ctx, hipGetLastError());
    return MIS_OK;
}

extern "C" int mis_blender_pack_rects(MisBlender* b, const MisLevelRect* rects, int n, void* dev_buf, size_t bytes) { return rect_exchange(b, rects, n, dev_buf, bytes, 0); }
extern "C" int mis_blender_add_rects(MisBlender* b, const MisLevelRect* rects, int n, const void* dev_buf, size_t bytes) { return rect_exchange(b, rects, n, (void*)dev_buf, bytes, 1); }
extern "C" int mis_blender_zero_rects(MisBlender* b, const MisLevelRect* rects, int n) { return rect_exchange(b, rects, n, nullptr, 0, 2); }

extern "C" int mis_blender_feed_rect(const MisBlender* b, int width, int height, MisPoint tl, MisRect* tile) {
    if (!b || !tile || !b->prepared || width < 1 || height < 1) return MIS_E_INVALID;
    if (b->type != MIS_BLEND_MULTI_BAND) { tile->x = tl.x; tile->y = tl.y; tile->width = width; tile->height = height; return MIS_OK; }
    feed_tile_rect(b, width, height, tl, &tile->x, &tile->y, &tile->width, &tile->height);
    return MIS_OK;
}

extern "C" int mis_blender_level_info(const MisBlender* b, int level, int* width, int* height, void** lap_dev, void** weight_dev) {
    if (!b || level < 0 || level > b->num_bands) return MIS_E_INVALID;
    if (width) *width = b->lw[level];
    if (height) *height = b->lh[level];
    if (lap_dev) *lap_dev = b->lap[level];
    if (weight_dev) *weight_dev = b->wgt[level];
    if (lap_dev || weight_dev) const_cast<MisBlender*>(b)->fresh = false;
    return MIS_OK;
}
```

### image_stitching_amd/csrc/orb.hip

```cpp
#include "common.h"
#include "dev_math.h"
#include <algorithm>
#include <cmath>
#include <mutex>
#include <unordered_map>

#define ORB_MAX_LEVELS 16
#define ORB_BORDER 32

namespace {

struct LevelDesc {
    int w, h;
    int pp;
    int sp;
    size_t pad_off;
    size_t map_off;
    float scale;
    int nfeat;
    int n2;
    int tiles_x, tiles_y, tile_off;
    int cap1, cand_off;
    int cap2, fin_off;
    int tab_off;
// ... 722 lines not shown
#pragma unroll
    for (int k = 0; k < TR / 4; k++) {
        const int r = r0 + k, py = ty0 + r;
        if (py >= ph) break;
        const int x = px - ORB_BORDER, y = py - ORB_BORDER;
        uint8_t o;
        if ((unsigned)x < (unsigned)d.w && (unsigned)y < (unsigned)d.h) {
            int acc = 0;
#pragma unroll
            for (int j = 0; j < 7; j++) acc += kq[j] * hv[k + j];
            o = (uint8_t)((acc + (1 << 15)) >> 16);
        } else o = tile[(r + 3) * TP + c + 4];
        dst[(size_t)py * d.pp + px] = o;
    }
}

__global__ __launch_bounds__(256) void describe_kernel(Levels L, const uint8_t* blur, const MisKeyPoint* kps, const uint32_t* kp_lxy,
                                                       const int* n_ptr, const int8_t* pattern, uint8_t* desc) {
    const int i = blockIdx.x * 8 + (threadIdx.x >> 5), b = threadIdx.x & 31;
    if (i >= *n_ptr) return;
    const MisKeyPoint kp = kps[i];
    const LevelDesc& d = L.d[kp.octave];
    const float inv = 1.f / d.scale;
    const int cx = mis_round_f(kp.x * inv), cy = mis_round_f(kp.y * inv);
    float ang = kp.angle * (float)(3.14159265358979323846 / 180.f);
    float sa, ca;
    mis_sincosf(ang, &sa, &ca);
    const int pp = d.pp;
    const uint8_t* ctr = blur + d.pad_off + (size_t)(cy + ORB_BORDER) * pp + (cx + ORB_BORDER);
    const int8_t* pat = pattern + b * 32;
    int val = 0;
#pragma unroll
    for (int bit = 0; bit < 8; bit++) {
        float x0 = (float)pat[4 * bit], y0 = (float)pat[4 * bit + 1], x1 = (float)pat[4 * bit + 2], y1 = (float)pat[4 * bit + 3];
        int ix0 = mis_round_f(x0 * ca - y0 * sa), iy0 = mis_round_f(x0 * sa + y0 * ca);
        int ix1 = mis_round_f(x1 * ca - y1 * sa), iy1 = mis_round_f(x1 * sa + y1 * ca);
        int t0 = ctr[iy0 * pp + ix0], t1 = ctr[iy1 * pp + ix1];
        val |= (t0 < t1) << bit;
    }
    desc[(size_t)i * 32 + b] = (uint8_t)val;
}

constexpr int DD_R = 28, DD_P = DD_R + 3, DD_N = 2 * DD_P + 1, DD_ROW_DW = (DD_N + 3 + 3) / 4, DD_PITCH = 4 * DD_ROW_DW + 4;
struct UMax16 { int v[16]; };
__global__ __launch_bounds__(256) void describe_direct_kernel(Levels L, const uint8_t* pad, OrbIO io, const int8_t* pattern, const int* umax, UMax16 um16, size_t ws) {
    __shared__ __attribute__((aligned(16))) uint8_t patch[4][DD_N * DD_PITCH];
    const int wave = threadIdx.x >> 6, lane = threadIdx.x & 63;
    const int i = blockIdx.x * 4 + wave, fr = blockIdx.y;
    WS_OFF(pad, fr, ws);
    MisKeyPoint* kps = io.kps[fr];
    const uint32_t* kp_lxy = io.lxy[fr];
    const int* n_ptr = io.n_dev[fr];
    uint8_t* desc = io.desc[fr];
    if (i >= *n_ptr) return;
    const MisKeyPoint kp = kps[i];
    const LevelDesc& d = L.d[kp.octave];
    const float inv = 1.f / d.scale;
    const int cx = mis_round_f(kp.x * inv), cy = mis_round_f(kp.y * inv);
    const int pp = d.pp;
    const uint8_t* org = pad + d.pad_off + (size_t)(cy + ORB_BORDER - DD_P) * pp + (cx + ORB_BORDER - DD_P);
    const int shift = (int)((uintptr_t)org & 3);
    const uint8_t* abase = org - shift;
    uint8_t* P = patch[wave];
    for (int k = lane; k < DD_N * DD_ROW_DW; k += 64) {
        const int r = k / DD_ROW_DW, c = k - r * DD_ROW_DW;
        reinterpret_cast<unsigned*>(P + r * DD_PITCH)[c] = *reinterpret_cast<const unsigned*>(abase + (size_t)r * pp + 4 * c);
    }
    __builtin_amdgcn_fence(__ATOMIC_ACQ_REL, "wavefront");
    __builtin_amdgcn_wave_barrier();
    const int c0 = DD_P * DD_PITCH + DD_P + shift;
    float kp_angle;
    {
        const int hp = L.half_patch;
        const uint8_t* ctr = P + c0;
        int m01 = 0, m10 = 0;
        const int u = lane - hp;
        if (lane <= 2 * hp) {
            m10 = u * ctr[u];
            if (hp <= 15) {
#pragma unroll 3
                for (int v = 1; v <= hp; ++v) {
                    const int vp = ctr[u + v * DD_PITCH], vm = ctr[u - v * DD_PITCH];
                    const bool in = abs(u) <= um16.v[v];
                    m10 += in ? u * (vp + vm) : 0;
                    m01 += in ? v * (vp - vm) : 0;
                }
            } else {
                for (int v = 1; v <= hp; ++v) {
                    if (abs(u) <= umax[v]) {
                        const int vp = ctr[u + v * DD_PITCH], vm = ctr[u - v * DD_PITCH];
                        m10 += u * (vp + vm);
                        m01 += v * (vp - vm);
                    }
                }
            }
        }
#pragma unroll
        for (int o = 32; o > 0; o >>= 1) { m01 += __shfl_xor(m01, o); m10 += __shfl_xor(m10, o); }
        kp_angle = mis_fast_atan2((float)m01, (float)m10);
        if (lane == 0) kps[i].angle = kp_angle;
    }
    float ang = kp_angle * (float)(3.14159265358979323846 / 180.f);
    float sa, ca;
    mis_sincosf(ang, &sa, &ca);
    const int b = lane & 31, h = lane >> 5;
    const int8_t* pat = pattern + b * 32 + h * 16;
    const unsigned* P32 = reinterpret_cast<const unsigned*>(P);
    auto blurred = [&](int ix, int iy) {
        const int a = c0 + (iy - 3) * DD_PITCH + (ix - 3);
        const bool inside = (unsigned)(cx + ix) < (unsigned)d.w && (unsigned)(cy + iy) < (unsigned)d.h;
        const unsigned* q = P32 + (a >> 2);
        const unsigned sh = (unsigned)(a & 3) << 3;
        const int kq[7] = {18, 34, 48, 56, 48, 34, 18};
        unsigned acc = 0, centre = 0;
#pragma unroll
        for (int j = 0; j < 7; j++) {
            const unsigned d0 = q[j * (DD_PITCH / 4)], d1 = q[j * (DD_PITCH / 4) + 1], d2 = q[j * (DD_PITCH / 4) + 2];
            const unsigned lo = __builtin_amdgcn_alignbit(d1, d0, sh), hi = __builtin_amdgcn_alignbit(d2, d1, sh);
            const unsigned hs = __builtin_amdgcn_udot4(lo, 0x38302212u, __builtin_amdgcn_udot4(hi, 0x00122230u, 0u, false), false);
            acc += (unsigned)kq[j] * hs;
            if (j == 3) centre = lo >> 24;
        }
        return inside ? (int)((acc + (1u << 15)) >> 16) : (int)centre;
    };
    int val = 0;
#ifndef DD_UNROLL
#define DD_UNROLL 1
#endif
#pragma unroll DD_UNROLL
    for (int bit = 0; bit < 4; bit++) {
        float x0 = (float)pat[4 * bit], y0 = (float)pat[4 * bit + 1], x1 = (float)pat[4 * bit + 2], y1 = (float)pat[4 * bit + 3];
        int ix0 = mis_round_f(x0 * ca - y0 * sa), iy0 = mis_round_f(x0 * sa + y0 * ca);
        int ix1 = mis_round_f(x1 * ca - y1 * sa), iy1 = mis_round_f(x1 * sa + y1 * ca);
        const int t0 = blurred(ix0, iy0), t1 = blurred(ix1, iy1);
        val |= (t0 < t1) << (bit + 4 * h);
    }
    val |= __shfl_xor(val, 32);
    if (h == 0) desc[(size_t)i * 32 + b] = (uint8_t)val;
}

constexpr int ORB_GATHER_MAX = 96;
struct GatherPtrs { const int* p[ORB_GATHER_MAX]; };
__global__ void gather_ints_kernel(GatherPtrs g, int n, int* __restrict__ out) {
    const int i = blockIdx.x * blockDim.x + threadIdx.x;
    if (i < n) out[i] = *g.p[i];
}

}

struct MisOrb {
    MisContext* ctx = nullptr;
    void (*enqueued_cb)(void*) = nullptr;
    void* enqueued_user = nullptr;
    MisOrbParams p;
    int max_w = 0, max_h = 0;
    int cur_w = 0, cur_h = 0;
    Levels L;
    Work w;
    size_t ws_stride = 0;
    int ws_frames = 0;
    int umax_host[64] = {0};
    int8_t pattern_host[1024] = {0};
    void* mem = nullptr;
    size_t pad_bytes = 0, map_bytes = 0;
    int cand_total = 0, fin_total = 0, tab_total = 0, surv_total = 0, out_cap = 0;
    std::vector<int> tab_host;
    int* host_counts = nullptr;
    bool direct_describe = false;
};

namespace {

void linear_exact_coeffs(int dlen, int slen, int* ofs, int* m1) {
    double inv = (double)dlen / (double)slen, scale = 1.0 / inv;
    for (int i = 0; i < dlen; i++) {
        double v = ((double)i + 0.5) * scale - 0.5;
        int iv = (int)floor(v);
        if (iv < 0) { ofs[i] = 0; m1[i] = 0; }
        else if (iv >= slen - 1) { ofs[i] = slen - 1; m1[i] = 0; }
        else { ofs[i] = iv; m1[i] = (int)lrint((v - (double)iv) * 256.0); }
    }
}

constexpr int ORB_MAX_LEVEL_FEATURES = 2048 - 128;

inline float level_scale(const MisOrbParams& p, int l) { return (float)pow((double)p.scale_factor, (double)l); }
inline int level_dim(int len, float sc) { return (int)lrint((double)((float)len / sc)); }

void level_budgets(const MisOrbParams& p, int* nfeat) {
    float factor = (float)(1.0 / (double)p.scale_factor);
    float nd = (float)p.nfeatures * (1 - factor) / (1 - (float)pow((double)factor, (double)p.nlevels));
    int sum = 0;
    for (int l = 0; l < p.nlevels - 1; l++) { nfeat[l] = (int)lrintf(nd); sum += nfeat[l]; nd *= factor; }
    nfeat[p.nlevels - 1] = std::max(p.nfeatures - sum, 0);
}

int check_level_sizes(MisContext* ctx, const MisOrbParams& p, int w, int h) {
    for (int l = 0; l < p.nlevels; l++) {
        const float sc = level_scale(p, l);
        MIS_CHECK(ctx, level_dim(w, sc) >= 1 && level_dim(h, sc) >= 1, MIS_E_UNSUPPORTED,
                  "ORB level %d of a %dx%d frame is empty (scale_factor %g, nlevels %d)", l, w, h, (double)p.scale_factor, p.nlevels);
    }
    return MIS_OK;
}

void plan_levels(MisOrb* o, int w, int h) {
    Levels& L = o->L;
    const MisOrbParams& p = o->p;
    L.n = p.nlevels; L.fast_t = p.fast_threshold; L.patch = p.patch_size; L.half_patch = p.patch_size / 2; L.edge = p.edge_threshold;
    size_t pad_off = 0, map_off = 0;
    int cand_off = 0, fin_off = 0, tab_off = 0, surv_off = 0;
    int nfeat[ORB_MAX_LEVELS];
    level_budgets(p, nfeat);
    for (int l = 0; l < L.n; l++) {
        LevelDesc& d = L.d[l];
        float sc = level_scale(p, l);
        d.scale = sc;
        d.w = level_dim(w, sc);
        d.h = level_dim(h, sc);
        d.pp = (int)mis_align_up((size_t)d.w + 2 * ORB_BORDER, 64);
        d.sp = (int)mis_align_up((size_t)d.w, 64);
        d.pad_off = pad_off; pad_off += (size_t)d.pp * (d.h + 2 * ORB_BORDER);
        d.map_off = map_off; map_off += (size_t)d.sp * d.h;
        d.nfeat = nfeat[l];
        d.n2 = p.score_type == 0 ? 2 * d.nfeat : d.nfeat;
        d.tiles_x = (d.w + FT_COLS - 1) / FT_COLS; d.tiles_y = (d.h + FT_ROWS - 1) / FT_ROWS;
        d.tile_off = surv_off; surv_off += d.tiles_x * d.tiles_y;
        d.cap1 = 4 * d.n2 + 4096;
        d.cap2 = std::min(d.nfeat + 128, 2048);
        d.cand_off = cand_off; cand_off += d.cap1;
        d.fin_off = fin_off; fin_off += d.cap2;
        d.tab_off = tab_off; tab_off += (2 * ((d.w + 3) & ~3) + 2 * d.h + 3) & ~3;
    }
    o->pad_bytes = pad_off; o->map_bytes = map_off; o->cand_total = cand_off; o->fin_total = fin_off; o->tab_total = tab_off; o->surv_total = surv_off;
    o->tab_host.assign(tab_off, 0);
    for (int l = 1; l < L.n; l++) {
        int* t = o->tab_host.data() + L.d[l].tab_off;
        const int dw4 = (L.d[l].w + 3) & ~3;
        linear_exact_coeffs(L.d[l].w, L.d[l - 1].w, t, t + dw4);
        linear_exact_coeffs(L.d[l].h, L.d[l - 1].h, t + 2 * dw4, t + 2 * dw4 + L.d[l].h);
    }
}

int upload_tables(MisOrb* o) {
    MisContext* ctx = o->ctx;
    if (o->tab_total)
        MIS_HIP(ctx, hipMemcpyAsync(o->w.tab, o->tab_host.data(), sizeof(int) * o->tab_total, hipMemcpyHostToDevice, ctx->stream));
    MIS_HIP(ctx, hipStreamSynchronize(ctx->stream));
    return MIS_OK;
}

std::mutex g_feat_mutex;
std::unordered_map<void*, size_t> g_feat_sizes;

int alloc_features(MisContext* ctx, int cap, int desc_cols, int desc_dtype, MisFeatures* f) {
    size_t kb = mis_align_up(sizeof(MisKeyPoint) * (size_t)cap, 256), db = mis_align_up((size_t)cap * desc_cols * mis_dtype_size(desc_dtype), 256);
    size_t lb = mis_align_up(sizeof(uint32_t) * (size_t)cap, 256);
    void* mem = nullptr;
    size_t got = 0;
    int rc = mis_pool_alloc(ctx, kb + db + lb + 256, &mem, &got);
    if (rc != MIS_OK) return rc;
    f->keypoints = (MisKeyPoint*)mem;
    f->descriptors = (uint8_t*)mem + kb;
    f->desc_cols = desc_cols; f->desc_dtype = desc_dtype;
    f->owner_ = mem;
    f->n = 0;
    std::lock_guard<std::mutex> lock(g_feat_mutex);
    g_feat_sizes[mem] = got;
    return MIS_OK;
}

inline uint32_t* feat_lxy(const MisFeatures* f, int cap) {
    size_t kb = mis_align_up(sizeof(MisKeyPoint) * (size_t)cap, 256), db = mis_align_up((size_t)cap * f->desc_cols * mis_dtype_size(f->desc_dtype), 256);
    return (uint32_t*)((uint8_t*)f->owner_ + kb + db);
}
inline int* feat_count(const MisFeatures* f, int cap) {
    size_t kb = mis_align_up(sizeof(MisKeyPoint) * (size_t)cap, 256), db = mis_align_up((size_t)cap * f->desc_cols * mis_dtype_size(f->desc_dtype), 256);
    size_t lb = mis_align_up(sizeof(uint32_t) * (size_t)cap, 256);
    return (int*)((uint8_t*)f->owner_ + kb + db + lb);
}

int enqueue_detect_group(MisOrb* o, const DevView* img, int w, int h, MisFeatures* out, int ng) {
    MisContext* ctx = o->ctx;
    const Levels& L = o->L;
    const Work& W = o->w;
    hipStream_t st = ctx->stream;
    const LevelDesc& d0 = L.d[0];
    const size_t ws = o->ws_stride;
    const unsigned nf = (unsigned)ng;
    OrbIO io;
    for (int k = 0; k < ORB_BATCH; k++) {
        const int q = k < ng ? k : 0;
        io.src[k] = (const uint8_t*)img[q].data; io.sstride[k] = img[q].stride;
        io.aligned[k] = (img[q].stride % 4 == 0) && ((uintptr_t)img[q].data % 4 == 0);
        io.kps[k] = out[q].keypoints; io.lxy[k] = feat_lxy(&out[q], o->out_cap); io.n_dev[k] = feat_count(&out[q], o->out_cap);
        io.desc[k] = (uint8_t*)out[q].descriptors;
    }
    MIS_HIP(ctx, hipMemset2DAsync(W.hist, ws ? ws : sizeof(int) * (256 * HIST_COPIES * ORB_MAX_LEVELS + 4 * ORB_MAX_LEVELS), 0,
                                  sizeof(int) * (256 * HIST_COPIES * ORB_MAX_LEVELS + 4 * ORB_MAX_LEVELS), nf, st));
    hipLaunchKernelGGL(gray_kernel, dim3((w + 1023) / 1024, (h + GRAY_ROWS - 1) / GRAY_ROWS, nf), dim3(256), 0, st, io, w, h, W.pad + d0.pad_off, d0.pp, ws);
    for (int l = 1; l < L.n; l++) {
        const LevelDesc &s = L.d[l - 1], &d = L.d[l];
        hipLaunchKernelGGL(resize_kernel, dim3((d.w + 255) / 256, (d.h + 4 * RS_ROWS - 1) / (4 * RS_ROWS), nf), dim3(256), 0, st, W.pad + s.pad_off, s.w, s.h, s.pp, W.pad + d.pad_off, d.w,
                           d.h, d.pp, W.tab + d.tab_off, ws);
    }
    const int pw0 = d0.w + 2 * ORB_BORDER, ph0 = d0.h + 2 * ORB_BORDER;
// ... 32 lines not shown
    MIS_CHECK(ctx, bgr->width <= o->max_w && bgr->height <= o->max_h && bgr->width >= 64 && bgr->height >= 64, MIS_E_INVALID,
              "image %dx%d outside the finder's range (64x64 .. %dx%d)", bgr->width, bgr->height, o->max_w, o->max_h);
    return MIS_OK;
}

int replan_if_needed(MisOrb* o, int w, int h) {
    if (w == o->cur_w && h == o->cur_h) return MIS_OK;
    const int rc = check_level_sizes(o->ctx, o->p, w, h);
    if (rc != MIS_OK) return rc;
    MIS_HIP(o->ctx, hipStreamSynchronize(o->ctx->stream));
    plan_levels(o, w, h);
    o->cur_w = w; o->cur_h = h;
    return upload_tables(o);
}

int orb_alloc_workspace(MisOrb* o, int frames) {
    MisContext* ctx = o->ctx;
    size_t off = 0;
    auto carve = [&](size_t bytes) { size_t o_ = off; off += mis_align_up(bytes, 256); return o_; };
    const bool frame_blur = !o->direct_describe;
    size_t o_pad = carve(o->pad_bytes), o_blur = frame_blur ? carve(o->pad_bytes) : 0;
    size_t o_hist = carve(sizeof(int) * (256 * HIST_COPIES * ORB_MAX_LEVELS + 4 * ORB_MAX_LEVELS)), o_flags = carve(256);
    size_t o_sxy = carve(sizeof(uint32_t) * FT_SLOTS * (size_t)o->surv_total), o_ssc = carve(FT_SLOTS * (size_t)o->surv_total), o_tc = carve(sizeof(int) * (size_t)o->surv_total);
    size_t o_cxy = carve(sizeof(uint32_t) * o->cand_total), o_cr = carve(sizeof(float) * o->cand_total);
    size_t o_fxy = carve(sizeof(uint32_t) * o->fin_total), o_fr = carve(sizeof(float) * o->fin_total);
    size_t o_tab = carve(sizeof(int) * (o->tab_total + 4)), o_umax = carve(sizeof(int) * 64), o_pat = carve(1024);
    const size_t tail = mis_align_up(o->map_bytes, 256) + (frame_blur ? 0 : mis_align_up(o->pad_bytes, 256));
    void* mem = nullptr;
    if (hipMalloc(&mem, off * (size_t)frames + tail) != hipSuccess) return mis_set_error(ctx, MIS_E_NOMEM, "hipMalloc of %zu bytes failed", off * (size_t)frames + tail);
    o->mem = mem; o->ws_stride = off; o->ws_frames = frames;
    uint8_t* m = (uint8_t*)o->mem;
    uint8_t* shared = m + off * (size_t)frames;
    Work& W = o->w;
    W.pad = m + o_pad; W.nms = shared; W.blur = frame_blur ? m + o_blur : shared + mis_align_up(o->map_bytes, 256); W.score = nullptr;
    W.hist = (int*)(m + o_hist); W.thr = W.hist + 256 * HIST_COPIES * ORB_MAX_LEVELS; W.cnt1 = W.thr + ORB_MAX_LEVELS; W.cnt2 = W.cnt1 + ORB_MAX_LEVELS;
    W.surv_xy = (uint32_t*)(m + o_sxy); W.surv_sc = m + o_ssc; W.tile_cnt = (int*)(m + o_tc);
    W.flags = (int*)(m + o_flags);
    W.cand_xy = (uint32_t*)(m + o_cxy); W.cand_resp = (float*)(m + o_cr); W.fin_xy = (uint32_t*)(m + o_fxy); W.fin_resp = (float*)(m + o_fr);
    W.tab = (int*)(m + o_tab); W.umax = (int*)(m + o_umax); W.pattern = (int8_t*)(m + o_pat);
    return MIS_OK;
}

int orb_init_workspace(MisOrb* o) {
    MisContext* ctx = o->ctx;
    const Work& W = o->w;
    MIS_HIP(ctx, hipMemcpyAsync(W.umax, o->umax_host, sizeof(o->umax_host), hipMemcpyHostToDevice, ctx->stream));
    MIS_HIP(ctx, hipMemcpyAsync(W.pattern, o->pattern_host, sizeof(o->pattern_host), hipMemcpyHostToDevice, ctx->stream));
    MIS_HIP(ctx, hipMemset2DAsync(W.flags, o->ws_stride, 0, 256, (size_t)o->ws_frames, ctx->stream));
    MIS_HIP(ctx, hipStreamSynchronize(ctx->stream));
    return upload_tables(o);
}

int orb_ensure_frames(MisOrb* o, int frames) {
    frames = std::min(frames, ORB_BATCH);
    if (o->ws_frames >= frames) return MIS_OK;
    MisContext* ctx = o->ctx;
    MIS_HIP(ctx, hipStreamSynchronize(ctx->stream));
    void* old = o->mem;
    const Work oldw = o->w;
    const size_t olds = o->ws_stride;
    const int oldf = o->ws_frames;
    int rc = MIS_E_NOMEM;
    for (int f = frames; f > oldf; f = std::max(oldf, f / 2)) {
        if ((rc = orb_alloc_workspace(o, f)) == MIS_OK) break;
    }
    if (rc != MIS_OK) {
        o->mem = old; o->w = oldw; o->ws_stride = olds; o->ws_frames = oldf;
        return oldf >= 1 ? MIS_OK : rc;
    }
    if (old) MIS_HIP(ctx, hipFree(old));
    return orb_init_workspace(o);
}

}

int mis_feat_block_alloc(MisContext* ctx, size_t bytes, void** out, MisContext* errs) {
    size_t got = 0;
    const int rc = mis_pool_alloc(ctx, bytes, out, &got, errs);
    if (rc != MIS_OK) return rc;
    std::lock_guard<std::mutex> lock(g_feat_mutex);
    g_feat_sizes[*out] = got;
    return MIS_OK;
}


extern "C" void mis_orb_default_params(MisOrbParams* p) {
    if (p) *p = MisOrbParams{4000, 1.2f, 8, 1, 0, 2, 0, 40, 20};
}

extern "C" int mis_orb_create(MisContext* ctx, const MisOrbParams* p, int max_w, int max_h, MisOrb** out) {
    if (!ctx || !out) return MIS_E_INVALID;
    MIS_CHECK(ctx, p, MIS_E_INVALID, "null params");
    MIS_CHECK(ctx, p->nlevels >= 1 && p->nlevels <= ORB_MAX_LEVELS && p->first_level == 0 && p->wta_k == 2 && p->patch_size >= 2 &&
                       p->patch_size <= 40 && p->nfeatures >= 1 && p->scale_factor > 1.f && (p->score_type == 0 || p->score_type == 1) &&
                       p->edge_threshold >= 0 && p->fast_threshold >= 1 && p->fast_threshold < 255,
              MIS_E_UNSUPPORTED, "unsupported ORB parameters (need first_level 0, wta_k 2, patch <= 40, nlevels <= 16)");
    MIS_CHECK(ctx, p->patch_size != 31, MIS_E_UNSUPPORTED, "ORB patch_size 31 (OpenCV's fixed bit_pattern_31_) is not supported");
    {
        int nfeat[ORB_MAX_LEVELS];
        level_budgets(*p, nfeat);
        for (int l = 0; l < p->nlevels; l++)
            MIS_CHECK(ctx, nfeat[l] <= ORB_MAX_LEVEL_FEATURES, MIS_E_UNSUPPORTED,
                      "ORB nfeatures %d gives level %d a budget of %d keypoints (at most %d per level)", p->nfeatures, l, nfeat[l], ORB_MAX_LEVEL_FEATURES);
    }
    MIS_CHECK(ctx, max_w >= 64 && max_h >= 64 && max_w <= 32767 && max_h <= 32767, MIS_E_INVALID, "bad maximum size");
    if (int rc = check_level_sizes(ctx, *p, max_w, max_h)) return rc;
    MIS_HIP(ctx, hipSetDevice(ctx->device));
    MisOrb* o = new MisOrb();
    o->ctx = ctx; o->p = *p; o->max_w = max_w; o->max_h = max_h;
    plan_levels(o, max_w, max_h);
    o->out_cap = o->fin_total;
    int umax[64] = {0};
    {
        int hp = p->patch_size / 2, v, v0;
        int vmax = (int)floor((double)((float)hp * sqrtf(2.f) / 2 + 1));
        int vmin = (int)ceil((double)((float)hp * sqrtf(2.f) / 2));
        for (v = 0; v <= vmax; ++v) umax[v] = (int)lrint(sqrt((double)hp * hp - (double)v * v));
        for (v = hp, v0 = 0; v >= vmin; --v) {
            while (umax[v0] == umax[v0 + 1]) ++v0;
            umax[v] = v0;
            ++v0;
        }
    }
    int8_t pat[1024];
    {
        uint64_t state = 0x34985739u;
        auto next = [&]() { state = (uint64_t)(uint32_t)state * 4164903690u + (uint32_t)(state >> 32); return (uint32_t)state; };
        int hp = p->patch_size / 2;
        for (int i = 0; i < 1024; i++) pat[i] = (int8_t)(int)(next() % (uint32_t)(2 * hp + 1) + (uint32_t)(-hp));
    }
    {
        int max_sq = 0;
        for (int i = 0; i < 512; i++) max_sq = std::max(max_sq, (int)pat[2 * i] * pat[2 * i] + (int)pat[2 * i + 1] * pat[2 * i + 1]);
        const int reach = (int)floor(sqrt((double)max_sq) + 0.5);
        o->direct_describe = reach <= DD_R && 3 + ORB_BORDER >= DD_P;
    }
    int rc0 = orb_alloc_workspace(o, 1);
    if (rc0 != MIS_OK) { delete o; return rc0; }
    memcpy(o->umax_host, umax, sizeof(umax));
    memcpy(o->pattern_host, pat, sizeof(pat));
    o->cur_w = max_w; o->cur_h = max_h;
    int rc = orb_init_workspace(o);
    if (rc != MIS_OK) { hipFree(o->mem); delete o; return rc; }
    *out = o;
    return MIS_OK;
}

extern "C" int mis_orb_destroy(MisOrb* o) {
    if (!o) return MIS_OK;
    hipSetDevice(o->ctx->device);
    hipStreamSynchronize(o->ctx->stream);
    if (o->mem) hipFree(o->mem);
    if (o->host_counts) hipHostFree(o->host_counts);
    delete o;
    return MIS_OK;
}


extern "C" int mis_orb_detect_batch(MisOrb* o, const MisImage* imgs, int n, MisFeatures* out) {
    if (!o) return MIS_E_INVALID;
    MisContext* ctx = o->ctx;
    MIS_CHECK(ctx, imgs && out && n >= 1, MIS_E_INVALID, "null argument");
    MIS_HIP(ctx, hipSetDevice(ctx->device));
    int rc;
    for (int i = 0; i < n; i++) {
        if ((rc = check_image(o, &imgs[i])) != MIS_OK) return rc;
        MIS_CHECK(ctx, imgs[i].width == imgs[0].width && imgs[i].height == imgs[0].height, MIS_E_INVALID, "batch frames must share one size");
    }
    if ((rc = replan_if_needed(o, imgs[0].width, imgs[0].height)) != MIS_OK) return rc;
    if ((rc = orb_ensure_frames(o, n)) != MIS_OK) return rc;
    std::vector<DevView> dimg(n);
    for (int i = 0; i < n; i++) memset(&out[i], 0, sizeof(MisFeatures));
    auto fail = [&](int code) {
        hipStreamSynchronize(ctx->stream);
        for (int i = 0; i < n; i++)
            if (out[i].keypoints || out[i].descriptors) mis_features_free(ctx, &out[i]);
        return code;
    };
    for (int i = 0; i < n; i++) {
        out[i].img_idx = i; out[i].img_w = imgs[i].width; out[i].img_h = imgs[i].height;
        if ((rc = alloc_features(ctx, o->out_cap, 32, MIS_U8, &out[i])) != MIS_OK) return fail(rc);
        if ((rc = dimg[i].read(ctx, &imgs[i])) != MIS_OK) return fail(rc);
    }
    const bool trace = getenv("MIS_ORB_TRACE") != nullptr;
    const auto t_enq0 = std::chrono::steady_clock::now();
    for (int g0 = 0; g0 < n; g0 += o->ws_frames) {
        const int ng = std::min(o->ws_frames, n - g0);
        if ((rc = enqueue_detect_group(o, &dimg[g0], imgs[0].width, imgs[0].height, &out[g0], ng)) != MIS_OK) return fail(rc);
    }
    if (trace) fprintf(stderr, "orb batch: %d frames enqueued in %.0f us\n", n, (double)std::chrono::duration_cast<std::chrono::microseconds>(std::chrono::steady_clock::now() - t_enq0).count());
    if (o->enqueued_cb) {
        void (*cb)(void*) = o->enqueued_cb;
        void* user = o->enqueued_user;
        o->enqueued_cb = nullptr; o->enqueued_user = nullptr;
        cb(user);
        MIS_HIP(ctx, hipSetDevice(ctx->device));
    }
    std::vector<int> counts(n);
    const int nl = o->ws_frames;
    std::vector<int> ws_flags(nl, 0);
    if (!o->host_counts) MIS_HIP(ctx, hipHostMalloc((void**)&o->host_counts, sizeof(int) * ORB_GATHER_MAX, hipHostMallocMapped));
    for (int i0 = 0; i0 < n + nl; i0 += ORB_GATHER_MAX) {
        const int m = std::min(ORB_GATHER_MAX, n + nl - i0);
        GatherPtrs gp;
        for (int k = 0; k < m; k++)
            gp.p[k] = i0 + k < n ? feat_count(&out[i0 + k], o->out_cap) : (const int*)((const char*)o->w.flags + (size_t)(i0 + k - n) * o->ws_stride);
        int* dev_view = nullptr;
        MIS_HIP(ctx, hipHostGetDevicePointer((void**)&dev_view, o->host_counts, 0));
        hipLaunchKernelGGL(gather_ints_kernel, dim3(1), dim3(ORB_GATHER_MAX), 0, ctx->stream, gp, m, dev_view);
        MIS_HIP(ctx, hipStreamSynchronize(ctx->stream));
        for (int k = 0; k < m; k++) (i0 + k < n ? counts[i0 + k] : ws_flags[i0 + k - n]) = o->host_counts[k];
    }
    int flags = 0;
    for (int k = 0; k < nl; k++) flags |= ws_flags[k];
    if (flags) hipMemset2DAsync(o->w.flags, o->ws_stride, 0, sizeof(int), (size_t)nl, ctx->stream);
    for (int i = 0; i < n; i++) out[i].n = counts[i];
    if (flags) {
        return mis_set_error(ctx, MIS_E_OVERFLOW, "ORB candidate buffers overflowed (flags %d): too many tied scores", flags);
    }
    return MIS_OK;
}

extern "C" int mis_orb_detect(MisOrb* o, const MisImage* bgr, MisFeatures* out) { return mis_orb_detect_batch(o, bgr, 1, out); }

extern "C" int mis_orb_on_enqueued(MisOrb* o, void (*fn)(void*), void* user) {
    if (!o) return MIS_E_INVALID;
    o->enqueued_cb = fn; o->enqueued_user = user;
    return MIS_OK;
}

extern "C" int mis_features_download(MisContext* ctx, const MisFeatures* f, MisKeyPoint* kps, void* desc) {
    if (!ctx || !f) return MIS_E_INVALID;
    MIS_HIP(ctx, hipSetDevice(ctx->device));
    if (f->n > 0) {
        if (kps) MIS_HIP(ctx, hipMemcpyAsync(kps, f->keypoints, sizeof(MisKeyPoint) * (size_t)f->n, hipMemcpyDeviceToHost, ctx->stream));
        if (desc) MIS_HIP(ctx, hipMemcpyAsync(desc, f->descriptors, (size_t)f->n * f->desc_cols * mis_dtype_size(f->desc_dtype), hipMemcpyDeviceToHost, ctx->stream));
    }
    MIS_HIP(ctx, hipStreamSynchronize(ctx->stream));
    return MIS_OK;
}

extern "C" int mis_features_upload(MisContext* ctx, int img_w, int img_h, int n, const MisKeyPoint* kps, const void* desc, int desc_cols,
                                   int desc_dtype, MisFeatures* out) {
    if (!ctx || !out) return MIS_E_INVALID;
    MIS_CHECK(ctx, n >= 0 && (n == 0 || (kps && desc)) && desc_cols > 0 && (desc_dtype == MIS_U8 || desc_dtype == MIS_F32), MIS_E_INVALID,
              "bad feature arrays");
    MIS_HIP(ctx, hipSetDevice(ctx->device));
    memset(out, 0, sizeof(*out));
    out->img_w = img_w; out->img_h = img_h;
    int rc = alloc_features(ctx, std::max(n, 1), desc_cols, desc_dtype, out);
    if (rc != MIS_OK) return rc;
    if (n) {
        MIS_HIP(ctx, hipMemcpyAsync(out->keypoints, kps, sizeof(MisKeyPoint) * (size_t)n, hipMemcpyHostToDevice, ctx->stream));
        MIS_HIP(ctx, hipMemcpyAsync(out->descriptors, desc, (size_t)n * desc_cols * mis_dtype_size(desc_dtype), hipMemcpyHostToDevice, ctx->stream));
        MIS_HIP(ctx, hipStreamSynchronize(ctx->stream));
    }
    out->n = n;
    return MIS_OK;
}

extern "C" int mis_features_free(MisContext* ctx, MisFeatures* f) {
    if (!ctx || !f) return MIS_E_INVALID;
    if (f->owner_) {
        size_t bytes = 0;
        {
            std::lock_guard<std::mutex> lock(g_feat_mutex);
            auto it = g_feat_sizes.find(f->owner_);
            if (it != g_feat_sizes.end()) { bytes = it->second; g_feat_sizes.erase(it); }
        }
        if (bytes) mis_pool_free(ctx, f->owner_, bytes);
        else {
            MIS_HIP(ctx, hipSetDevice(ctx->device));
            MIS_HIP(ctx, hipStreamSynchronize(ctx->stream));
            MIS_HIP(ctx, hipFree(f->owner_));
        }
    }
    f->owner_ = nullptr; f->keypoints = nullptr; f->descriptors = nullptr; f->n = 0;
    return MIS_OK;
}

extern "C" int mis_orb_debug_level(MisOrb* o, int level, int which, uint8_t* host_out, int* width, int* height) {
    if (!o) return MIS_E_INVALID;
    MisContext* ctx = o->ctx;
    MIS_CHECK(ctx, level >= 0 && level < o->L.n && which >= 0 && which <= 2, MIS_E_INVALID, "bad level / selector");
    const LevelDesc& d = o->L.d[level];
    int w = which == 2 ? d.w + 2 * ORB_BORDER : d.w, h = which == 2 ? d.h + 2 * ORB_BORDER : d.h;
    if (width) *width = w;
    if (height) *height = h;
    if (!host_out) return MIS_OK;
    MIS_HIP(ctx, hipSetDevice(ctx->device));
    const uint8_t* src;
    size_t pitch;
    if (which == 0) { src = o->w.pad + d.pad_off + (size_t)ORB_BORDER * d.pp + ORB_BORDER; pitch = d.pp; }
    else if (which == 1) {
        MIS_HIP(ctx, hipMemsetAsync(o->w.nms + d.map_off, 0, (size_t)d.sp * d.h, ctx->stream));
        hipLaunchKernelGGL(nms_raster_kernel, dim3(256), dim3(64), 0, ctx->stream, d, o->w.tile_cnt, o->w.surv_xy, o->w.surv_sc, o->w.nms);
        src = o->w.nms + d.map_off; pitch = d.sp;
    }
    else {
        if (o->direct_describe) {
            const int pw0 = o->L.d[0].w + 2 * ORB_BORDER, ph0 = o->L.d[0].h + 2 * ORB_BORDER;
            hipLaunchKernelGGL(blur_kernel, dim3((pw0 + 63) / 64, (ph0 + 31) / 32, o->L.n), dim3(256), 0, ctx->stream, o->L, o->w.pad, o->w.blur);
        }
        src = o->w.blur + d.pad_off; pitch = d.pp;
    }
    MIS_HIP(ctx, hipMemcpy2DAsync(host_out, w, src, pitch, w, h, hipMemcpyDeviceToHost, ctx->stream));
    MIS_HIP(ctx, hipStreamSynchronize(ctx->stream));
    return MIS_OK;
}

#ifdef MIS_ORB_STATS
extern "C" int mis_debug_orb_stats(unsigned long long* out, int reset) {
    hipDeviceSynchronize();
    hipMemcpyFromSymbol(out, HIP_SYMBOL(g_orb_stats), sizeof(unsigned long long) * 8);
    if (reset) { unsigned long long z[8] = {0}; hipMemcpyToSymbol(HIP_SYMBOL(g_orb_stats), z, sizeof(z)); }
    return 0;
}
#endif
```

### image_stitching_amd/distributed.py

```python
import ctypes as C
import os
import time

import numpy as np
import torch

from . import _capi as capi
from . import stitching as st


def frame_block(n, rank, world):
    base, rem = divmod(n, world)
    lo = rank * base + min(rank, rem)
    return list(range(lo, lo + base + (1 if rank < rem else 0)))


class Comm:

    def __init__(self, rank=0, world=1, group=None, always_collective=False):
        self.rank, self.world, self.group = rank, world, group
        self._stage = False
        self._solo = world == 1 and not always_collective
        if not self._solo:
            import torch.distributed as dist
# ... 114 lines not shown

    def feature_counts(self, feats):
        return torch.tensor([len(f) for f in feats], dtype=torch.int32, device=self.ctx.device)

    def pack_features(self, feats, cap):
        m = len(feats)
        dev = self.ctx.device
        rb = self._row_bytes(feats)
        kps = torch.empty((m, cap * 24), dtype=torch.uint8, device=dev)
        desc = torch.empty((m, cap * rb), dtype=torch.uint8, device=dev)
        if m:
            arr = (capi.MisFeatures * m)()
            for k, f in enumerate(feats):
                C.memmove(C.byref(arr[k]), C.byref(f.raw), C.sizeof(capi.MisFeatures))
            self.ctx.check(self.ctx.lib.mis_features_pack(self.ctx.h, arr, m, int(cap), int(rb), C.c_void_p(kps.data_ptr()), C.c_void_p(desc.data_ptr())))
        return kps, desc

    def _row_bytes(self, feats=None):
        return 512 if self.cfg.features_type == "sift" else 32

    def unpack_features(self, kps_all, desc_all, counts_all):
        self._keep = [kps_all, desc_all, counts_all]
        counts = counts_all.cpu().tolist()
        w, h = self.work_size
        sift = self.cfg.features_type == "sift"
        out = []
        for i, n in enumerate(counts):
            raw = capi.MisFeatures()
            raw.img_idx, raw.img_w, raw.img_h, raw.n = i, w, h, int(n)
            raw.keypoints = kps_all[i].data_ptr()
            raw.descriptors = desc_all[i].data_ptr()
            raw.desc_cols, raw.desc_dtype, raw.owner_ = (128, capi.F32, None) if sift else (32, capi.U8, None)
            out.append(st.ImageFeatures(self.ctx, raw))
        return out

    def match(self, feats, rank, world):
        return self.matcher(feats, rank, world)

    def confidence_tensor(self, pm, n, on_device=True):
        t = torch.from_numpy(pm.confidences()).view(n, n)
        return t.to(self.ctx.device) if on_device else t

    def refine_cameras(self, feats, pm, indices, cams):
        return st.refine_cameras(self.ctx, feats, pm, indices, cams, self.cfg)

    def match_entries(self, pm, conf_thresh):
        out = []
        n = pm.n
        for i in range(n):
            for j in range(i + 1, n):
                raw = pm._mis[i * n + j]
                if raw.src_img_idx < 0:
                    continue
                m = pm[i * n + j]
                strong = m.confidence > conf_thresh
                out.append((i, j, m.matches if strong else m.matches[:0], m.inliers_mask if strong else m.inliers_mask[:0], m.num_inliers, m.H is not None,
                            m.H, m.confidence))
        return out

    def matches_from_entries(self, per_rank, n):
        return st.PairwiseMatches.from_entries(self.ctx, n, [e for entries in per_rank for e in entries])

    def seam_local(self, frames, cams, scale):
        return [st.seam_scale_warp(self.cctx, self.cfg, self.frame_size, f, c, scale, self.work_scale) for f, c in zip(frames, cams)]

    def seam_pack(self, item, cap):
        _, iw, mw = item
        buf = torch.zeros(cap * 4, dtype=torch.uint8, device=self.ctx.device)
        n = mw.numel()
        buf[:3 * n] = iw.reshape(-1)
        buf[3 * cap:3 * cap + n] = mw.reshape(-1)
        return buf

    def seam_unpack(self, buf, w, h, cap):
        return buf[:3 * w * h].view(h, w, 3), buf[3 * cap:3 * cap + w * h].view(h, w)

    def seam_global(self, corners, images, masks):
        self._seam = st.seam_solve(self.cctx, self.cfg, corners, images, masks)

    def warp_feed_seam_many(self, frames, cams, rois, ks):
        if not frames:
            return
        warped = self.warper.warp_fused_batch(frames, cams, rois)
        compensator, seam_masks = self._seam
        for (tl, img_s, mask), k in zip(warped, ks):
            if compensator is not None:
                compensator.apply(k, tl, img_s, mask)
            st.seam_mask_apply(self.cctx, seam_masks[k], mask)
        self.blender.feed_batch([w[1] for w in warped], [w[2] for w in warped], [w[0] for w in warped])

    def warp_feed_seam(self, frame, cam, roi, k):
        tl, img_s, mask = self.warper.warp_fused(frame, cam["K"], cam["R"], roi)
        compensator, seam_masks = self._seam
        if compensator is not None:
            compensator.apply(k, tl, img_s, mask)
        st.seam_mask_apply(self.cctx, seam_masks[k], mask)
        self.blender.feed(img_s, mask, tl)

    def warp_roi(self, scale, cam, size=None):
        if capi.roi_is_full_scan(self.kind):
            return self.warp_rois(scale, [cam], size)[0]
        return st.warp_roi(scale, size or self.frame_size, cam["K"], cam["R"], self.kind)

    def warp_rois(self, scale, cams, size=None):
        return st.warp_rois(self.cctx, scale, size or self.frame_size, cams, self.kind)

    def resize_frame(self, frame, f):
        return st.resize(self.cctx, frame, fx=f, fy=f)

    def begin_compose(self, scale, corners, sizes):
        x, y, pw, ph = st.result_roi(corners, sizes)
        btype, bands, sharp = st.blend_config(self.cfg.blend_type, self.cfg.blend_strength, (pw, ph))
        key = (btype, bands, sharp)
        if self.blender is None or getattr(self, "_blender_key", None) != key:
            self._blender_key = key
            self.blender = {capi.BLEND_MULTI_BAND: lambda: st.MultiBandBlender(self.cctx, bands),
                            capi.BLEND_FEATHER: lambda: st.FeatherBlender(self.cctx, sharp), capi.BLEND_NO: lambda: st.Blender(self.cctx)}[btype]()
        self.blender.prepare(corners, sizes)
        self.warper = st.RotationWarper(self.cctx, scale, self.kind)
        self.pano_size = (pw, ph)
        return btype, bands

    def warp_feed(self, frame, cam, roi):
        tl, img_s, mask = self.warper.warp_fused(frame, cam["K"], cam["R"], roi)
        self.blender.feed(img_s, mask, tl)

    def match_fence_target(self):
        return int(self.ctx.lib.mis_match_sequence(self.ctx.h)) + 1

    def on_match_enqueued(self, fn):
        if fn is None:
            self._enqueued_fn = None
            self.ctx.lib.mis_match_on_enqueued(self.ctx.h, None, None)
            return
        self._enqueued_fn = fn
        if getattr(self, "_enqueued_cb", None) is None:
            self._enqueued_cb = C.CFUNCTYPE(None, C.c_void_p)(self._run_enqueued)
        self.ctx.check(self.ctx.lib.mis_match_on_enqueued(self.ctx.h, C.cast(self._enqueued_cb, C.c_void_p), None))

    def _run_enqueued(self, _user):
        fn, self._enqueued_fn = getattr(self, "_enqueued_fn", None), None
        if fn is not None:
            fn()

    def compose_after_knn(self, target_seq):
        rc = self.ctx.lib.mis_match_knn_fence(self.ctx.h, self._compose_stream_handle, target_seq, 50)
        if rc == 1:
            self.fence_timeouts = getattr(self, "fence_timeouts", 0) + 1
        elif rc != 0:
            self.ctx.check(rc)

    def warp_feed_many(self, frames, cams, rois):
        self.blender.compose_frames(frames, self.warper.scale, cams, rois, self.kind)

    def accumulators(self):
        out = []
        dev = self.ctx.device
        nb = self.ctx.lib.mis_blender_num_bands(self.blender.h)
        for l in range(nb + 1):
            w, h, lp, wp = C.c_int(), C.c_int(), C.c_void_p(), C.c_void_p()
            self.cctx.check(self.cctx.lib.mis_blender_level_info(self.blender.h, l, C.byref(w), C.byref(h), C.byref(lp), C.byref(wp)))
            out.append((dev_tensor(lp.value, (h.value, w.value * 3), "<i2", dev), dev_tensor(wp.value, (h.value, w.value), "<f4", dev)))
        return out

    def finalize(self):
        return self.blender.blend()

    def num_bands(self):
        return self.ctx.lib.mis_blender_num_bands(self.blender.h)

    def level_sizes(self):
        out = []
        for l in range(self.num_bands() + 1):
            w, h = C.c_int(), C.c_int()
            self.cctx.check(self.cctx.lib.mis_blender_level_info(self.blender.h, l, C.byref(w), C.byref(h), None, None))
            out.append((w.value, h.value))
        return out

    @staticmethod
    def _rect_array(rects):
        return (capi.MisLevelRect * max(len(rects), 1))(*[capi.MisLevelRect(*r) for r in rects])

    def pack_rects(self, rects, nbytes):
        buf = torch.empty(max(int(nbytes), 16), dtype=torch.uint8, device=self.ctx.device)
        if rects:
            self.cctx.check(self.cctx.lib.mis_blender_pack_rects(self.blender.h, self._rect_array(rects), len(rects), C.c_void_p(buf.data_ptr()), buf.numel()))
        return buf[:int(nbytes)]

    def add_rects(self, rects, buf):
        if rects:
            self.cctx.check(self.cctx.lib.mis_blender_add_rects(self.blender.h, self._rect_array(rects), len(rects), C.c_void_p(buf.data_ptr()), buf.numel()))

    def zero_rects(self, rects):
        if rects:
            self.cctx.check(self.cctx.lib.mis_blender_zero_rects(self.blender.h, self._rect_array(rects), len(rects)))

    def finalize_columns(self, x0, x1):
        w, h = self.blender._size
        x1 = min(x1, w)
        dst = st._empty_image(self.cctx, h, x1 - x0, 3, torch.int16)
        msk = st._empty_image(self.cctx, h, x1 - x0, 1, torch.uint8)
        d, m = st.as_image(dst), st.as_image(msk)
        self.cctx.check(self.cctx.lib.mis_blender_blend_columns(self.blender.h, int(x0), int(x1), C.byref(d), C.byref(m)))
        return dst, msk

    def strip_to_bytes(self, img, msk, cap_w):
        h, w = msk.shape
        out = torch.zeros(h * cap_w * 7, dtype=torch.uint8, device=self.ctx.device)
        lib, cx = self.cctx.lib, self.cctx
        cx.check(lib.mis_copy_2d(cx.h, C.c_void_p(out.data_ptr()), cap_w * 6, C.c_void_p(img.data_ptr()), img.stride(0) * 2, w * 6, h))
        cx.check(lib.mis_copy_2d(cx.h, C.c_void_p(out.data_ptr() + h * cap_w * 6), cap_w, C.c_void_p(msk.data_ptr()), msk.stride(0), w, h))
        return out

    def assemble(self, strips, bounds, cap_w, size):
        w, h = size
        pano = st._empty_image(self.cctx, h, w, 3, torch.int16)
        mask = st._empty_image(self.cctx, h, w, 1, torch.uint8)
        lib, cx = self.cctx.lib, self.cctx
        for k, (x0, x1) in enumerate(bounds):
            x1 = min(x1, w)
            if x1 <= x0:
                continue
            base = strips[k].data_ptr()
            cx.check(lib.mis_copy_2d(cx.h, C.c_void_p(pano.data_ptr() + x0 * 6), pano.stride(0) * 2, C.c_void_p(base), cap_w * 6, (x1 - x0) * 6, h))
            cx.check(lib.mis_copy_2d(cx.h, C.c_void_p(mask.data_ptr() + x0), mask.stride(0), C.c_void_p(base + h * cap_w * 6), cap_w, x1 - x0, h))
        return pano, mask

    def sync(self):
        torch.cuda.synchronize(self.ctx.device)


class StitchJob:

    def __init__(self, ctx, frame_size, cameras, rank=0, world_size=1, group=None, engine=None, config=None, force_collectives=False, always_collective=False):
        self.cfg = config or st.StitchConfig.hot_path()
        st.check_seam_config(self.cfg)
        self.kind = st.check_warp_config(self.cfg)
        st.check_range_config(self.cfg)
        st.check_matcher_config(self.cfg)
        self.engine = engine or HipEngine(ctx, frame_size, self.cfg)
        engine_warp = getattr(self.engine, "warp_type", "spherical")
        if engine_warp != self.cfg.warp_type:
            raise NotImplementedError("warp_type %r: the engine %s warps %r only" % (self.cfg.warp_type, type(self.engine).__name__, engine_warp))
        engine_range = getattr(self.engine, "range_width", -1)
        if engine_range != self.cfg.range_width:
            raise NotImplementedError("range_width %r: the engine %s matches with range_width %r only" % (self.cfg.range_width, type(self.engine).__name__, engine_range))
        engine_matcher = getattr(self.engine, "matcher_type", "homography")
        if engine_matcher != self.cfg.matcher_type:
            raise NotImplementedError("matcher_type %r: the engine %s matches with matcher_type %r only" % (self.cfg.matcher_type, type(self.engine).__name__, engine_matcher))
        self.work_scale, self.work_size = st.work_geometry(self.cfg, frame_size)
        if self.work_scale != 1.0 and getattr(self.engine, "work_scale", 1.0) != self.work_scale:
            raise NotImplementedError("work_megapix %r (work scale %.6f): the engine %s does not resize frames to work scale"
                                      % (self.cfg.work_megapix, self.work_scale, type(self.engine).__name__))
        self.cams0 = cameras
        self.work_cams0 = cameras if self.work_scale == 1.0 else [st.scaled_camera(c, self.work_scale) for c in cameras]
        self.cams = self.work_cams0
        self.n = len(cameras)
        self.rank, self.world = rank, world_size
        self.comm = Comm(rank, world_size, group, always_collective)
        self.my_frames = frame_block(self.n, rank, world_size)
        self.frame_size = frame_size
        self.scale = st.Stitcher.warped_image_scale(self.cams)
        self.force_collectives = force_collectives
        self.seam_needed = self.cfg.expos_comp_type != "no" or self.cfg.seam_find_type != "no"
        counts = {len(frame_block(self.n, r, world_size)) for r in range(world_size)}
        if len(counts) != 1:
            raise ValueError("the frame count must divide evenly over the ranks")

    def stage_features(self, frames):
        return self.engine.detect([frames[i] for i in self.my_frames])

    def stage_gather(self, local_feats):
        if self.world == 1 and not self.force_collectives:
            return local_feats
        counts_all = self.comm.all_gather(self.engine.feature_counts(local_feats)).flatten(0, 1)
        cap = max(int(counts_all.max()), 1)
        kps, desc = self.engine.pack_features(local_feats, cap)
        kps_all = self.comm.all_gather(kps).flatten(0, 1)
        desc_all = self.comm.all_gather(desc).flatten(0, 1)
        return self.engine.unpack_features(kps_all, desc_all, counts_all)

    def stage_match(self, feats):
        pm = self.engine.match(feats, self.rank, self.world)
        if self.world == 1 and not self.force_collectives and isinstance(self.engine, HipEngine):
            return pm, self.engine.confidence_tensor(pm, self.n, on_device=False)
        conf = self.engine.confidence_tensor(pm, self.n)
        conf = self.comm.all_reduce_sum(conf)
        return pm, conf

    def stage_prune(self, conf):
        return [int(i) for i in st.leaveBiggestComponentConf(conf.cpu().numpy().reshape(self.n, self.n), self.cfg.conf_thresh)]

    def stage_compose_prepare(self, indices):
        eng = self.engine
        self.scale = st.Stitcher.warped_image_scale([self.cams[i] for i in indices])
        g = st.compose_geometry(self.cfg, self.frame_size, self.scale, self.work_scale)
        self._geom = g
        ccams = {i: st.scaled_camera(self.cams[i], g.aspect) for i in indices} if g.aspect != 1.0 else {i: self.cams[i] for i in indices}
        if g.size != tuple(self.frame_size) and not hasattr(eng, "resize_frame"):
            raise NotImplementedError("this engine does not resize frames (compose_megapix > 0 needs resize_frame)")
        if hasattr(eng, "warp_rois"):
            rois = dict(zip(indices, eng.warp_rois(g.warp_scale, [ccams[i] for i in indices], g.size)))
        else:
            rois = {i: eng.warp_roi(g.warp_scale, ccams[i], g.size) for i in indices}
        corners = [(rois[i][0], rois[i][1]) for i in indices]
        sizes = [(rois[i][2], rois[i][3]) for i in indices]
        btype, bands = eng.begin_compose(g.warp_scale, corners, sizes)
        self._compose_indices, self._compose_rois, self._compose_cams = indices, rois, ccams
        return btype, bands

    def stage_compose(self, frames, indices, prepared=None):
        eng = self.engine
        btype, bands = prepared if prepared is not None else self.stage_compose_prepare(indices)
        rois, ccams, g = self._compose_rois, self._compose_cams, self._geom
        mine = [i for i in self.my_frames if i in rois]
        cframes = {i: eng.resize_frame(frames[i], g.compose_scale) for i in mine} if g.size != tuple(self.frame_size) else frames
        if self.seam_needed:
            marks = getattr(self, "marks", None)
            if marks is not None:
                marks.append(("compose: sized", time.perf_counter()))
            self.stage_seam(frames, indices)
            if marks is not None:
                marks.append(("compose: seams solved", time.perf_counter()))
            if hasattr(eng, "warp_feed_seam_many"):
                eng.warp_feed_seam_many([cframes[i] for i in mine], [ccams[i] for i in mine], [rois[i] for i in mine], [indices.index(i) for i in mine])
            else:
                for i in mine:
                    eng.warp_feed_seam(cframes[i], ccams[i], rois[i], indices.index(i))
            return btype, bands
        if hasattr(eng, "warp_feed_many"):
            eng.warp_feed_many([cframes[i] for i in mine], [ccams[i] for i in mine], [rois[i] for i in mine])
        else:
            for i in mine:
                eng.warp_feed(cframes[i], ccams[i], rois[i])
        return btype, bands

    def stage_seam(self, frames, indices):
        eng = self.engine
        mine = [i for i in self.my_frames if i in indices]
        local = eng.seam_local([frames[i] for i in mine], [self.cams[i] for i in mine], self.scale)
        if getattr(self, "marks", None) is not None:
            self.marks.append(("compose: seam-scale warps enqueued", time.perf_counter()))
        if self.world == 1 and not self.force_collectives:
            items = local
        else:
            per = len(self.my_frames)
            meta = torch.zeros((per, 5), dtype=torch.int32)
            for k, (i, it) in enumerate(zip(mine, local)):
                meta[k] = torch.tensor([i, it[0][0], it[0][1], it[2].shape[1], it[2].shape[0]], dtype=torch.int32)
            meta[len(mine):, 0] = -1
            dev = torch.device(getattr(eng, "exchange_device", None) or (local[0][1].device if local else "cpu"))
            meta_all = self.comm.all_gather(meta.to(dev)).flatten(0, 1).cpu()
            cap = max(int((meta_all[:, 3] * meta_all[:, 4]).max()), 1)
            bufs = [eng.seam_pack(it, cap) for it in local] + [torch.zeros(cap * 4, dtype=torch.uint8, device=dev) for _ in range(per - len(mine))]
            all_bufs = self.comm.all_gather(torch.stack(bufs)).flatten(0, 1)
            by_index = {}
            for row, buf in zip(meta_all.tolist(), all_bufs):
                if row[0] >= 0:
                    iw, mw = eng.seam_unpack(buf, row[3], row[4], cap)
                    by_index[row[0]] = ((row[1], row[2]), iw, mw)
            items = [by_index[i] for i in indices]
        eng.seam_global([it[0] for it in items], [it[1] for it in items], [it[2] for it in items])

    def rank_region(self, r, indices, rois, bands, w0, h0):
        mine = [i for i in frame_block(self.n, r, self.world) if i in rois]
        if not mine:
            return None
        px = min(rois[i][0] for i in indices)
        py = min(rois[i][1] for i in indices)
        gap, a = 3 << bands, (1 << bands) - 1
        x0 = max(0, min(rois[i][0] for i in mine) - px - gap) & ~a
        y0 = max(0, min(rois[i][1] for i in mine) - py - gap) & ~a
        x1 = min(w0, (max(rois[i][0] + rois[i][2] for i in mine) - px + gap + a) & ~a)
        y1 = min(h0, (max(rois[i][1] + rois[i][3] for i in mine) - py + gap + a) & ~a)
        return x0, y0, x1, y1

    @staticmethod
    def strip_bounds(w0, bands, world):
        q = 1 << bands
        nq = w0 // q
        c = [(k * nq // world) * q for k in range(world)] + [w0]
        return [(c[k], c[k + 1]) for k in range(world)]

    @staticmethod
    def need_ranges(strip, level_sizes):
        lo, hi = strip
        out = [(lo, hi)]
        for l in range(1, len(level_sizes)):
            lo, hi = max(0, (lo >> 1) - 1), min(level_sizes[l][0], ((hi - 1) >> 1) + 2)
            out.append((lo, hi))
        return out

    @staticmethod
    def exchange_rects(region, need, level_sizes):
        rects, off = [], 0
        if region is None:
            return rects, 0
        rx0, ry0, rx1, ry1 = region
        for l, ((lw, lh), (nlo, nhi)) in enumerate(zip(level_sizes, need)):
            x0, x1 = max(min(rx0 >> l, lw), nlo), min(min(-((-rx1) >> l), lw), nhi)
            y0, y1 = min(ry0 >> l, lh), min(-((-ry1) >> l), lh)
            if x1 <= x0 or y1 <= y0:
                continue
            m = (x1 - x0) * (y1 - y0)
            rects.append((l, x0, y0, x1, y1, off))
            off += (m * 6 + 15) // 16 * 16 + (m * 4 + 15) // 16 * 16
        return rects, off

    def stage_reduce_finalize(self):
        eng = self.engine
        sizes = eng.level_sizes()
        bands = len(sizes) - 1
        w0, h0 = sizes[0]
        indices, rois = self._compose_indices, self._compose_rois
        world = self.world
        bounds = self.strip_bounds(w0, bands, world)
        needs = [self.need_ranges(bnd, sizes) for bnd in bounds]
        regions = [self.rank_region(r, indices, rois, bands, w0, h0) for r in range(world)]
        plan = [[self.exchange_rects(regions[r], needs[k], sizes) for k in range(world)] for r in range(world)]
        me = self.rank
        send = [eng.pack_rects(*plan[me][k]) for k in range(world)]
        recv = self.comm.all_to_all_bytes(send, [plan[r][me][1] for r in range(world)])
        full_h = [(l, lo, 0, hi, sizes[l][1], 0) for l, (lo, hi) in enumerate(needs[me]) if hi > lo]
        eng.zero_rects(full_h)
        for r in range(world):
            eng.add_rects(plan[r][me][0], recv[r])
        pw, ph = eng.pano_size
        x0, x1 = bounds[me][0], min(bounds[me][1], pw)
        cap_w = max(min(b1, pw) - b0 for b0, b1 in bounds)
        if x1 > x0:
            img, msk = eng.finalize_columns(x0, x1)
            mine = eng.strip_to_bytes(img, msk, cap_w)
        else:
            mine = torch.zeros(ph * cap_w * 7, dtype=torch.uint8, device=send[0].device)
        strips = self.comm.all_gather(mine)
        if self.rank != 0:
            return None, None
        return eng.assemble(strips, bounds, cap_w, (pw, ph))

    def stage_finalize(self):
        if self.rank == 0:
            return self.engine.finalize()
        return None, None

    def stage_exchange_finalize(self):
        if self.world == 1 and not self.force_collectives:
            return self.stage_finalize()
        side = getattr(self.engine, "compose_stream", None)
        if side is None:
            return self.stage_reduce_finalize()
        with torch.cuda.stream(side):
            return self.stage_reduce_finalize()

    def speculation_roi_ok(self):
        if self.kind == capi.WARP_SPHERICAL:
            return True
        g = st.compose_geometry(self.cfg, self.frame_size, st.Stitcher.warped_image_scale(self.cams), self.work_scale)
        try:
            if capi.roi_is_full_scan(self.kind) and hasattr(self.engine, "warp_rois"):
                self.engine.warp_rois(g.warp_scale, [st.scaled_camera(c, g.aspect) if g.aspect != 1.0 else c for c in self.cams], g.size)
                return True
            for c in self.cams:
                c = st.scaled_camera(c, g.aspect) if g.aspect != 1.0 else c
                st.warp_roi(g.warp_scale, g.size, c["K"], c["R"], self.kind)
        except st.MisError:
            return False
        return True

    def _compose_on_side_stream(self, frames, indices, prepared=None):
        eng = self.engine
        if getattr(eng, "compose_stream", None) is None:
            return self.stage_compose(frames, indices, prepared)
        with torch.cuda.stream(eng.compose_stream):
            return self.stage_compose(frames, indices, prepared)

    def run(self, frames):
        marks = self.marks = [("start", time.perf_counter())] if os.environ.get("MIS_JOB_TRACE") else None

        def mark(name):
            if marks is not None:
                marks.append((name, time.perf_counter()))
        refine = self.cfg.ba_cost_func != "no"
        solo_rank = self.world == 1 and not self.force_collectives
        spec = getattr(self.engine, "speculative_compose", False) and not refine and (not self.seam_needed or solo_rank)
        spec = spec and self.speculation_roi_ok()
        prepared = None
        side = getattr(self.engine, "compose_stream", None)
        if side is not None:
            side.wait_stream(torch.cuda.current_stream(self.engine.ctx.device))
        if spec:
            finder = getattr(self.engine, "finder", None)
            box0 = {}

            def prep():
                try:
                    with torch.cuda.stream(self.engine.compose_stream):
                        box0["p"] = self.stage_compose_prepare(list(range(self.n)))
                except BaseException as e:
                    box0["e"] = e
            hooked = hasattr(finder, "on_enqueued") and len(self.my_frames) > 0
            if hooked:
                finder.on_enqueued(prep)
            else:
                prep()
            try:
                local = self.stage_features(frames)
            finally:
                if hooked:
                    finder.on_enqueued(None)
            if "p" not in box0 and "e" not in box0:
                prep()
            if "e" in box0:
                raise box0["e"]
            prepared = box0["p"]
            feats = self.stage_gather(local)
        else:
            feats = self.stage_gather(self.stage_features(frames))
        mark("features")
        if spec:
            import threading
            everyone = list(range(self.n))
            box = {}

            fence = self.engine.match_fence_target() if hasattr(self.engine, "match_fence_target") else None

            solo = self.world == 1 and not self.force_collectives

            def work():
                try:
                    if fence is not None:
                        self.engine.compose_after_knn(fence)
                    mark("compose: fence passed")
                    box["r"] = self._compose_on_side_stream(frames, everyone, prepared)
                    mark("compose: enqueued")
                    if solo:
                        with torch.cuda.stream(self.engine.compose_stream):
                            box["f"] = self.stage_finalize()
                    mark("compose: finalise enqueued")
                except BaseException as e:
                    box["e"] = e
            if hasattr(self.engine, "on_match_enqueued"):
                self.engine.on_match_enqueued(work)
                try:
                    pm, conf = self.stage_match(feats)
                finally:
                    self.engine.on_match_enqueued(None)
                mark("match returned")
                if not box:
                    work()
                indices = self.stage_prune(conf)
                mark("pruned")
            else:
                th = threading.Thread(target=work)
                th.start()
                try:
                    pm, conf = self.stage_match(feats)
                    indices = self.stage_prune(conf)
                finally:
                    th.join()
            if "e" in box:
                raise box["e"]
            if indices == everyone and "f" in box:
                (btype, bands), (pano, mask) = box["r"], box["f"]
            else:
                btype, bands = box["r"] if indices == everyone else self._compose_on_side_stream(frames, indices)
                with torch.cuda.stream(self.engine.compose_stream):
                    pano, mask = self.stage_exchange_finalize()
            box.clear()
        else:
            pm, conf = self.stage_match(feats)
            indices = self.stage_prune(conf)
            if refine:
                if self.cfg.ba_cost_func != "reproj":
                    raise ValueError("ba_cost_func must be 'no' or 'reproj'")
                if self.world > 1 or self.force_collectives:
                    pm = self.engine.matches_from_entries(self.comm.all_gather_objects(self.engine.match_entries(pm, self.cfg.conf_thresh)), self.n)
                refined = self.engine.refine_cameras(feats, pm, indices, self.work_cams0)
                self.cams = list(self.work_cams0)
                for i, c in zip(indices, refined):
                    self.cams[i] = c
                self.scale = st.Stitcher.warped_image_scale([self.cams[i] for i in indices])
            btype, bands = self._compose_on_side_stream(frames, indices)
            pano, mask = self.stage_exchange_finalize()
        self.engine.sync()
        mark("synchronised")
        return {"pano": pano, "mask": mask, "indices": indices, "confidence": conf, "matches": pm, "features": feats,
                "pano_size": self.engine.pano_size, "num_bands": bands}

    def breakdown(self, frames, reps=3):
        out = {}

        def timed(name, fn):
            self.engine.sync()
            t0 = time.perf_counter()
            r = fn()
            self.engine.sync()
            out[name] = out.get(name, 0.0) + (time.perf_counter() - t0) * 1e3 / reps
            return r
        for _ in range(reps):
            lf = timed("features (detect+describe)", lambda: self.stage_features(frames))
            feats = timed("feature all-gather", lambda: self.stage_gather(lf))
            pm, conf = timed("match + RANSAC", lambda: self.stage_match(feats))
            idx = timed("prune (host)", lambda: self.stage_prune(conf))
            side = getattr(self.engine, "compose_stream", None)

            def on_side(fn):
                if side is None:
                    return fn()
                with torch.cuda.stream(side):
                    return fn()
            timed("warp + blend feed", lambda: on_side(lambda: self.stage_compose(frames, idx)))
            timed("blend exchange + finalise", lambda: on_side(self.stage_exchange_finalize))
        return out
```

### image_stitching_amd/stitching.py

```python
import ctypes as C
import math
from dataclasses import dataclass, field

import numpy as np

from . import _capi as capi

try:
    import torch
except Exception:
    torch = None


class MisError(RuntimeError):
    def __init__(self, code, text):
        super().__init__("libmistitch error %d: %s" % (code, text))
        self.code = code


KP_DTYPE = np.dtype([("x", "f4"), ("y", "f4"), ("size", "f4"), ("angle", "f4"), ("response", "f4"), ("octave", "i4")])
DMATCH_DTYPE = np.dtype([("query_idx", "i4"), ("train_idx", "i4"), ("img_idx", "i4"), ("distance", "f4")])

_TORCH_DT = {}
if torch is not None:
# ... 320 lines not shown
            self.close()
        except Exception:
            pass

    def feed(self, corners, images, masks):
        n = len(images)
        cs = (capi.MisPoint * n)(*[capi.MisPoint(int(c[0]), int(c[1])) for c in corners])
        im = (capi.MisImage * n)(*[as_image(i) for i in images])
        mk = (capi.MisImage * n)(*[as_image(m) for m in masks])
        self.ctx.check(self.ctx.lib.mis_compensator_feed(self.h, cs, im, mk, n))

    def gains(self, index):
        g = (C.c_double * 3)()
        self.ctx.check(self.ctx.lib.mis_compensator_gains(self.h, index, g))
        return np.array(g[:], np.float64)

    def gain_map(self, index):
        bx, by, ch = C.c_int(), C.c_int(), C.c_int()
        self.ctx.check(self.ctx.lib.mis_compensator_gain_map_channels(self.h, index, None, 0, C.byref(bx), C.byref(by), C.byref(ch)))
        out = np.zeros((by.value, bx.value) if ch.value == 1 else (by.value, bx.value, ch.value), np.float32)
        self.ctx.check(self.ctx.lib.mis_compensator_gain_map_channels(self.h, index, out.ctypes.data_as(C.POINTER(C.c_float)), out.size, None, None, None))
        return out

    def debug_stats(self, i, j, channel=0):
        n, a, b = C.c_int(), C.c_double(), C.c_double()
        self.ctx.check(self.ctx.lib.mis_compensator_debug_stats(self.h, i, j, channel, C.byref(n), C.byref(a), C.byref(b)))
        return n.value, a.value, b.value

    def apply(self, index, corner, image, mask=None):
        img = as_image(image)
        self.ctx.check(self.ctx.lib.mis_compensator_apply(self.h, index, C.byref(img)))
        return image


class GainCompensator(_Compensator):
    TYPE = capi.EXPOS_GAIN

    def __init__(self, ctx, nr_feeds=1):
        self._create(ctx, nr_feeds)


class ChannelsCompensator(_Compensator):
    TYPE = capi.EXPOS_CHANNELS

    def __init__(self, ctx, nr_feeds=1):
        self._create(ctx, nr_feeds)


class BlocksGainCompensator(_Compensator):
    TYPE = capi.EXPOS_GAIN_BLOCKS

    def __init__(self, ctx, bl_width=64, bl_height=64, nr_gain_filtering_iterations=2, nr_feeds=1):
        self._create(ctx, nr_feeds, bl_width, bl_height, nr_gain_filtering_iterations)


class BlocksChannelsCompensator(_Compensator):
    TYPE = capi.EXPOS_CHANNELS_BLOCKS

    def __init__(self, ctx, bl_width=64, bl_height=64, nr_gain_filtering_iterations=2, nr_feeds=1):
        self._create(ctx, nr_feeds, bl_width, bl_height, nr_gain_filtering_iterations)


EXPOS_COMP_TYPES = ("no", "gain", "gain_blocks", "channels_blocks")


def make_compensator(ctx, cfg):
    t, feeds = cfg.expos_comp_type, cfg.expos_comp_nr_feeds
    blocks = (cfg.expos_comp_block_size, cfg.expos_comp_block_size, cfg.expos_comp_nr_filtering, feeds)
    if t == "gain":
        return GainCompensator(ctx, feeds)
    if t == "gain_blocks":
        return BlocksGainCompensator(ctx, *blocks)
    if t == "channels_blocks":
        return BlocksChannelsCompensator(ctx, *blocks)
    return None


class NoSeamFinder:

    def find(self, images, corners, masks):
        return masks


class VoronoiSeamFinder:

    def __init__(self, ctx):
        self.ctx = ctx

    def find(self, images, corners, masks):
        n = len(masks)
        cs = (capi.MisPoint * n)(*[capi.MisPoint(int(c[0]), int(c[1])) for c in corners])
        mk = (capi.MisImage * n)(*[as_image(m) for m in masks])
        self.ctx.check(self.ctx.lib.mis_seam_voronoi(self.ctx.h, cs, mk, n))
        return masks


class DpSeamFinder:
    COLOR = 0

    def __init__(self, ctx, cost_func=0):
        self.ctx, self.cost_func = ctx, cost_func

    def find(self, images, corners, masks):
        n = len(masks)
        cs = (capi.MisPoint * n)(*[capi.MisPoint(int(c[0]), int(c[1])) for c in corners])
        im = (capi.MisImage * n)(*[as_image(i) for i in images])
        mk = (capi.MisImage * n)(*[as_image(m) for m in masks])
        self.ctx.check(self.ctx.lib.mis_seam_dp(self.ctx.h, cs, im, mk, n, int(self.cost_func)))
        return masks


def result_roi(corners, sizes):
    lib = capi.load()
    n = len(corners)
    cs = (capi.MisPoint * n)(*[capi.MisPoint(int(c[0]), int(c[1])) for c in corners])
    ss = (capi.MisSize * n)(*[capi.MisSize(int(s[0]), int(s[1])) for s in sizes])
    r = capi.MisRect()
    rc = lib.mis_result_roi(cs, ss, n, C.byref(r))
    if rc != capi.MIS_OK:
        raise MisError(rc, "mis_result_roi: invalid arguments")
    return r.x, r.y, r.width, r.height


def blend_config(blend_type, blend_strength, pano_size):
    lib = capi.load()
    t, nb, sh = C.c_int(), C.c_int(), C.c_float()
    lib.mis_blend_config(int(blend_type), float(blend_strength), int(pano_size[0]), int(pano_size[1]), C.byref(t),
                         C.byref(nb), C.byref(sh))
    return t.value, nb.value, sh.value


class Blender:

    def __init__(self, ctx, btype=capi.BLEND_NO, num_bands=5, sharpness=0.02):
        self.ctx = ctx
        h = C.c_void_p()
        ctx.check(ctx.lib.mis_blender_create(ctx.h, btype, num_bands, sharpness, C.byref(h)))
        self.h = h
        self.type = btype
        self._size = None

    @staticmethod
    def createDefault(ctx, btype):
        return {capi.BLEND_NO: Blender, capi.BLEND_FEATHER: FeatherBlender, capi.BLEND_MULTI_BAND: MultiBandBlender}[btype](ctx)

    def prepare(self, corners, sizes):
        n = len(corners)
        cs = (capi.MisPoint * n)(*[capi.MisPoint(int(c[0]), int(c[1])) for c in corners])
        ss = (capi.MisSize * n)(*[capi.MisSize(int(s[0]), int(s[1])) for s in sizes])
        self.ctx.check(self.ctx.lib.mis_blender_prepare(self.h, cs, ss, n))
        x, y, w, h = result_roi(corners, sizes)
        self._size = (w, h)

    def compose_frames(self, frames, scale, cameras, rois, kind=capi.WARP_SPHERICAL):
        n = len(frames)
        if n == 0:
            return
        arr = (capi.MisImage * n)(*[as_image(f) for f in frames])
        Ks = np.ascontiguousarray(np.stack([np.asarray(c["K"], np.float32).reshape(9) for c in cameras]))
        Rs = np.ascontiguousarray(np.stack([np.asarray(c["R"], np.float32).reshape(9) for c in cameras]))
        rr = (capi.MisRect * n)(*[capi.MisRect(int(r[0]), int(r[1]), int(r[2]), int(r[3])) for r in rois])
        self.ctx.check(self.ctx.lib.mis_compose_frames_kind(self.h, int(kind), arr, n, float(scale), Ks.ctypes.data_as(C.c_void_p),
                                                            Rs.ctypes.data_as(C.c_void_p), rr))

    def feed(self, img, mask, tl):
        i, m = as_image(img), as_image(mask)
        self.ctx.check(self.ctx.lib.mis_blender_feed(self.h, C.byref(i), C.byref(m), capi.MisPoint(int(tl[0]), int(tl[1]))))

    def feed_batch(self, imgs, masks, tls):
        n = len(imgs)
        im = (capi.MisImage * n)(*[as_image(i) for i in imgs])
        mk = (capi.MisImage * n)(*[as_image(m) for m in masks])
        ts = (capi.MisPoint * n)(*[capi.MisPoint(int(t[0]), int(t[1])) for t in tls])
        self.ctx.check(self.ctx.lib.mis_blender_feed_batch(self.h, im, mk, ts, n))

    def blend(self):
        if self._size is None:
            raise MisError(-5, "blend before prepare")
        w, h = self._size
        dst = _empty_image(self.ctx, h, w, 3, torch.int16)
        msk = _empty_image(self.ctx, h, w, 1, torch.uint8)
        d, m = as_image(dst), as_image(msk)
        self.ctx.check(self.ctx.lib.mis_blender_blend(self.h, C.byref(d), C.byref(m)))
        return dst, msk

    def level(self, i):
        w, h, lp, wp = C.c_int(), C.c_int(), C.c_void_p(), C.c_void_p()
        self.ctx.check(self.ctx.lib.mis_blender_level_info(self.h, i, C.byref(w), C.byref(h), C.byref(lp), C.byref(wp)))
        self.ctx.synchronize()
        n = w.value * h.value
        lap = np.empty((h.value, w.value, 3), np.int16)
        wgt = np.empty((h.value, w.value), np.float32)
        _memcpy_dtoh(lap, lp.value, n * 6)
        _memcpy_dtoh(wgt, wp.value, n * 4)
        return lap, wgt

    def close(self):
        if getattr(self, "h", None) and self.ctx.h:
            self.ctx.lib.mis_blender_destroy(self.h)
        self.h = None

    def __del__(self):
        try:
            self.close()
        except Exception:
            pass


class MultiBandBlender(Blender):

    def __init__(self, ctx, num_bands=5):
        super().__init__(ctx, capi.BLEND_MULTI_BAND, num_bands, 0.0)

    def numBands(self):
        return self.ctx.lib.mis_blender_num_bands(self.h)


class FeatherBlender(Blender):

    def __init__(self, ctx, sharpness=0.02):
        super().__init__(ctx, capi.BLEND_FEATHER, 0, sharpness)


_hip = None


def _memcpy_dtoh(dst_np, dev_ptr, nbytes):
    global _hip
    if _hip is None:
        _hip = C.CDLL("libamdhip64.so")
        _hip.hipMemcpy.argtypes = [C.c_void_p, C.c_void_p, C.c_size_t, C.c_int]
    rc = _hip.hipMemcpy(dst_np.ctypes.data_as(C.c_void_p), C.c_void_p(dev_ptr), nbytes, 2)
    if rc:
        raise RuntimeError("hipMemcpy D2H failed: %d" % rc)


class ImageFeatures:

    def __init__(self, ctx, raw):
        self.ctx, self.raw = ctx, raw

    @property
    def img_idx(self):
        return self.raw.img_idx

    @img_idx.setter
    def img_idx(self, v):
        self.raw.img_idx = int(v)

    @property
    def img_size(self):
        return self.raw.img_w, self.raw.img_h

    def __len__(self):
        return self.raw.n

    def download(self):
        n = self.raw.n
        kps = np.zeros(n, KP_DTYPE)
        dt = np.uint8 if self.raw.desc_dtype == capi.U8 else np.float32
        desc = np.zeros((n, self.raw.desc_cols), dt)
        if n:
            self.ctx.check(self.ctx.lib.mis_features_download(self.ctx.h, C.byref(self.raw), kps.ctypes.data_as(C.c_void_p),
                                                              desc.ctypes.data_as(C.c_void_p)))
        return kps, desc

    @staticmethod
    def upload(ctx, img_size, kps, desc, img_idx=0):
        kps = np.ascontiguousarray(kps, KP_DTYPE)
        desc = np.ascontiguousarray(desc)
        raw = capi.MisFeatures()
        ctx.check(ctx.lib.mis_features_upload(ctx.h, int(img_size[0]), int(img_size[1]), len(kps),
                                              kps.ctypes.data_as(C.c_void_p), desc.ctypes.data_as(C.c_void_p), desc.shape[1],
                                              _NP_DT[desc.dtype], C.byref(raw)))
        raw.img_idx = img_idx
        return ImageFeatures(ctx, raw)

    def close(self):
        if self.raw is not None and self.ctx.h:
            self.ctx.lib.mis_features_free(self.ctx.h, C.byref(self.raw))
        self.raw = None

    def __del__(self):
        try:
            self.close()
        except Exception:
            pass


def orb_params(**kw):
    p = capi.MisOrbParams()
    capi.load().mis_orb_default_params(C.byref(p))
    for k, v in kw.items():
        setattr(p, k, v)
    return p


class OrbFeatureFinder:

    def __init__(self, ctx, max_size, params=None):
        self.ctx = ctx
        self.params = params or orb_params()
        h = C.c_void_p()
        ctx.check(ctx.lib.mis_orb_create(ctx.h, C.byref(self.params), int(max_size[0]), int(max_size[1]), C.byref(h)))
        self.h = h

    def detect(self, img):
        raw = capi.MisFeatures()
        i = as_image(img)
        self.ctx.check(self.ctx.lib.mis_orb_detect(self.h, C.byref(i), C.byref(raw)))
        return ImageFeatures(self.ctx, raw)

    def on_enqueued(self, fn):
        if fn is None:
            self._enqueued_fn = None
            self.ctx.lib.mis_orb_on_enqueued(self.h, None, None)
            return
        self._enqueued_fn = fn
        if getattr(self, "_enqueued_cb", None) is None:
            self._enqueued_cb = C.CFUNCTYPE(None, C.c_void_p)(self._run_enqueued)
        self.ctx.check(self.ctx.lib.mis_orb_on_enqueued(self.h, C.cast(self._enqueued_cb, C.c_void_p), None))

    def _run_enqueued(self, _user):
        fn, self._enqueued_fn = getattr(self, "_enqueued_fn", None), None
        if fn is not None:
            fn()

    def detect_batch(self, imgs):
        n = len(imgs)
        arr = (capi.MisImage * n)(*[as_image(i) for i in imgs])
        raws = (capi.MisFeatures * n)()
        self.ctx.check(self.ctx.lib.mis_orb_detect_batch(self.h, arr, n, raws))
        out = []
        for k in range(n):
            r = capi.MisFeatures()
            C.memmove(C.byref(r), C.byref(raws[k]), C.sizeof(capi.MisFeatures))
            r.img_idx = k
            out.append(ImageFeatures(self.ctx, r))
        return out

    def debug_level(self, level, which):
        w, h = C.c_int(), C.c_int()
        self.ctx.check(self.ctx.lib.mis_orb_debug_level(self.h, level, which, None, C.byref(w), C.byref(h)))
        out = np.zeros((h.value, w.value), np.uint8)
        self.ctx.check(self.ctx.lib.mis_orb_debug_level(self.h, level, which, out.ctypes.data_as(C.c_void_p), C.byref(w), C.byref(h)))
        return out

    def close(self):
        if getattr(self, "h", None) and self.ctx.h:
            self.ctx.lib.mis_orb_destroy(self.h)
        self.h = None

    def __del__(self):
        try:
            self.close()
        except Exception:
            pass


class SiftFeatureFinder:

    def __init__(self, ctx, max_size, params=None):
        self.ctx = ctx
        p = capi.MisSiftParams()
        ctx.lib.mis_sift_default_params(C.byref(p))
        for k, v in (params or {}).items():
            setattr(p, k, v)
        self.params = p
        h = C.c_void_p()
        ctx.check(ctx.lib.mis_sift_create(ctx.h, C.byref(p), int(max_size[0]), int(max_size[1]), C.byref(h)))
        self.h = h

    def detect(self, img):
        raw = capi.MisFeatures()
        i = as_image(img)
        self.ctx.check(self.ctx.lib.mis_sift_detect(self.h, C.byref(i), C.byref(raw)))
        return ImageFeatures(self.ctx, raw)

    def detect_batch(self, imgs):
        n = len(imgs)
        if n == 0:
            return []
        arr = (capi.MisImage * n)(*[as_image(im) for im in imgs])
        raws = (capi.MisFeatures * n)()
        self.ctx.check(self.ctx.lib.mis_sift_detect_batch(self.h, arr, n, raws))
        out = []
        for k in range(n):
            raw = capi.MisFeatures()
            C.memmove(C.byref(raw), C.byref(raws[k]), C.sizeof(capi.MisFeatures))
            out.append(ImageFeatures(self.ctx, raw))
        return out

    def debug_level(self, img, octave, layer, dog=False):
        i = as_image(img)
        w, h = C.c_int(), C.c_int()
        self.ctx.check(self.ctx.lib.mis_sift_debug_level(self.h, C.byref(i), octave, layer, int(dog), None, C.byref(w), C.byref(h)))
        out = np.zeros((h.value, w.value), np.float32)
        self.ctx.check(self.ctx.lib.mis_sift_debug_level(self.h, C.byref(i), octave, layer, int(dog), out.ctypes.data_as(C.c_void_p), C.byref(w), C.byref(h)))
        return out

    def debug_counts(self):
        c = (C.c_uint * 4)()
        self.ctx.check(self.ctx.lib.mis_sift_debug_counts(self.h, c))
        return dict(candidates=int(c[0]), raw=int(c[1]), keypoints=int(c[2]), refined=int(c[3]))

    def close(self):
        if getattr(self, "h", None) and self.ctx.h:
            self.ctx.lib.mis_sift_destroy(self.h)
        self.h = None

    def __del__(self):
        try:
            self.close()
        except Exception:
            pass


def computeImageFeatures(finder, img, img_idx=0):
    f = finder.detect(img)
    f.img_idx = img_idx
    return f


@dataclass
class MatchesInfo:
    src_img_idx: int = -1
    dst_img_idx: int = -1
    matches: np.ndarray = field(default_factory=lambda: np.zeros(0, DMATCH_DTYPE))
    inliers_mask: np.ndarray = field(default_factory=lambda: np.zeros(0, np.uint8))
    num_inliers: int = 0
    H: np.ndarray = None
    confidence: float = 0.0


def _unpack_mi(mi):
    n = mi.n_matches
    out = MatchesInfo(mi.src_img_idx, mi.dst_img_idx)
    if n and mi.matches:
        out.matches = np.frombuffer((C.c_char * (n * 16)).from_address(C.addressof(mi.matches.contents)), DMATCH_DTYPE).copy()
    if n and mi.inliers_mask:
        out.inliers_mask = np.frombuffer((C.c_char * n).from_address(C.addressof(mi.inliers_mask.contents)), np.uint8).copy()
    out.num_inliers = mi.num_inliers
    out.H = np.array(list(mi.H), np.float64).reshape(3, 3) if mi.has_H else None
    out.confidence = mi.confidence
    return out


class PairwiseMatches:

    def __init__(self, ctx, mis, n):
        self._ctx, self._mis, self.n = ctx, mis, n
        self._cache = {}

    @classmethod
    def from_entries(cls, ctx, n, entries):
        mis = (capi.MisMatchesInfo * (n * n))()
        keep = []
        for k in range(n * n):
            mis[k].src_img_idx = mis[k].dst_img_idx = -1
        for i, j, matches, mask, num_inliers, has_H, H, conf in entries:
            mm = np.ascontiguousarray(matches, DMATCH_DTYPE)
            mk = np.ascontiguousarray(mask, np.uint8)
            sw = mm.copy()
            sw["query_idx"], sw["train_idx"] = mm["train_idx"], mm["query_idx"]
            Hd = np.asarray(H, np.float64).reshape(3, 3) if has_H else None
            for (a, b, arr, Hm) in ((i, j, mm, Hd), (j, i, sw, np.linalg.inv(Hd) if has_H else None)):
                e = mis[a * n + b]
                e.src_img_idx, e.dst_img_idx, e.n_matches = a, b, len(arr)
                e.matches = C.cast(arr.ctypes.data, C.POINTER(capi.MisDMatch)) if len(arr) else None
                e.inliers_mask = C.cast(mk.ctypes.data, C.POINTER(C.c_uint8)) if len(mk) else None
                e.num_inliers, e.has_H, e.confidence = int(num_inliers), 1 if has_H else 0, float(conf)
                if has_H:
                    for q, v in enumerate(Hm.reshape(9)):
                        e.H[q] = v
            keep += [mm, mk, sw]
        obj = cls(ctx, mis, n)
        obj._keep, obj._borrowed = keep, True
        return obj

# ... 448 lines not shown
```

### include/mistitch.h

```cpp
#ifndef MISTITCH_H
#define MISTITCH_H

#include <stddef.h>
#include <stdint.h>

#ifdef __cplusplus
extern "C" {
#endif

#define MIS_OK 0
#define MIS_E_INVALID (-1)
#define MIS_E_HIP (-2)
#define MIS_E_NOMEM (-3)
#define MIS_E_OVERFLOW (-4)
#define MIS_E_STATE (-5)
#define MIS_E_UNSUPPORTED (-6)
#define MIS_FENCE_TIMEOUT 1

enum { MIS_MEM_HOST = 0, MIS_MEM_DEVICE = 1 };
enum { MIS_U8 = 0, MIS_S16 = 1, MIS_F32 = 2 };
enum { MIS_INTER_NEAREST = 0, MIS_INTER_LINEAR = 1 };
enum { MIS_BORDER_CONSTANT = 0, MIS_BORDER_REFLECT = 2 };
enum { MIS_WARP_SPHERICAL = 0, MIS_WARP_CYLINDRICAL = 1, MIS_WARP_PLANE = 2, MIS_WARP_MERCATOR = 3, MIS_WARP_FISHEYE = 4, MIS_WARP_STEREOGRAPHIC = 5 };
#define MIS_WARP_ROI_IS_FULL_SCAN(kind) ((kind) >= MIS_WARP_MERCATOR && (kind) <= MIS_WARP_STEREOGRAPHIC)
enum { MIS_BLEND_NO = 0, MIS_BLEND_FEATHER = 1, MIS_BLEND_MULTI_BAND = 2 };

typedef struct MisContext MisContext;
typedef struct MisOrb MisOrb;
typedef struct MisBlender MisBlender;

typedef struct { int x, y; } MisPoint;
typedef struct { int width, height; } MisSize;
typedef struct { int x, y, width, height; } MisRect;

typedef struct {
    void* data;
    int width, height, channels;
    size_t stride;
    int dtype;
    int mem;
} MisImage;

int mis_context_create(int device, void* stream, MisContext** out);
int mis_stream_create(int device, int priority, void** stream);
int mis_stream_destroy(void* stream);
int mis_context_destroy(MisContext* ctx);
int mis_context_synchronize(MisContext* ctx);
int mis_context_wait(MisContext* ctx, MisContext* other);
const char* mis_last_error(const MisContext* ctx);
const char* mis_version(void);
int mis_image_free(MisContext* ctx, MisImage* img);

typedef struct {
    float x, y, size, angle, response;
    int octave;
} MisKeyPoint;

typedef struct {
    int nfeatures;
    float scale_factor;
    int nlevels, edge_threshold, first_level, wta_k, score_type, patch_size, fast_threshold;
} MisOrbParams;

typedef struct {
    int img_idx;
    int img_w, img_h;
    int n;
    MisKeyPoint* keypoints;
    void* descriptors;
    int desc_cols, desc_dtype;
    void* owner_;
} MisFeatures;

void mis_orb_default_params(MisOrbParams* p);
int mis_orb_create(MisContext* ctx, const MisOrbParams* p, int max_width, int max_height, MisOrb** out);
int mis_orb_destroy(MisOrb* orb);
int mis_orb_detect(MisOrb* orb, const MisImage* bgr, MisFeatures* out);
int mis_orb_detect_batch(MisOrb* orb, const MisImage* bgr, int n_images, MisFeatures* out);
int mis_orb_on_enqueued(MisOrb* orb, void (*fn)(void*), void* user);
int mis_features_download(MisContext* ctx, const MisFeatures* f, MisKeyPoint* kps_host, void* desc_host);
int mis_features_upload(MisContext* ctx, int img_w, int img_h, int n, const MisKeyPoint* kps_host,
                        const void* desc_host, int desc_cols, int desc_dtype, MisFeatures* out);
int mis_features_free(MisContext* ctx, MisFeatures* f);
int mis_features_pack(MisContext* ctx, const MisFeatures* feats, int m, int cap, int row_bytes, void* kps_dst, void* desc_dst);
int mis_copy_2d(MisContext* ctx, void* dst, size_t dst_pitch, const void* src, size_t src_pitch, size_t width_bytes, size_t height);
int mis_orb_debug_level(MisOrb* orb, int level, int which, uint8_t* host_out, int* width, int* height);

typedef struct {
    float match_conf;
    int num_matches_thresh1, num_matches_thresh2;
    double ransac_thresh;
    int max_iters;
    double confidence;
} MisMatchParams;

typedef struct { int query_idx, train_idx, img_idx; float distance; } MisDMatch;

typedef struct {
    int src_img_idx, dst_img_idx;
    int n_matches;
    MisDMatch* matches;
    uint8_t* inliers_mask;
    int num_inliers;
    int has_H;
    double H[9];
    double confidence;
} MisMatchesInfo;

void mis_match_default_params(MisMatchParams* p);
int mis_match_all_pairs(MisContext* ctx, const MisFeatures* feats, int n, const MisMatchParams* p, MisMatchesInfo* out);
int mis_match_pairs_sharded(MisContext* ctx, const MisFeatures* feats, int n, const MisMatchParams* p, int rank,
                            int world_size, MisMatchesInfo* out);
int mis_match_pairs_select(MisContext* ctx, const MisFeatures* feats, int n, const MisMatchParams* p, const uint8_t* mask,
                           int range_width, int rank, int world_size, MisMatchesInfo* out);
enum { MIS_MATCH_HOMOGRAPHY = 0, MIS_MATCH_AFFINE_PARTIAL = 1 };
void mis_match_affine_default_params(MisMatchParams* p);
int mis_match_pairs_model(MisContext* ctx, const MisFeatures* feats, int n, const MisMatchParams* p, int model, const uint8_t* mask,
                          int range_width, int rank, int world_size, MisMatchesInfo* out);
int mis_matches_free(MisMatchesInfo* m, int count);
long long mis_match_sequence(MisContext* ctx);
int mis_match_knn_fence(MisContext* ctx, void* stream, long long target_seq, int timeout_ms);
int mis_match_on_enqueued(MisContext* ctx, void (*fn)(void*), void* user);
int mis_knn2(MisContext* ctx, const MisFeatures* query, const MisFeatures* train, int* idx2_host, float* dist2_host);
int mis_find_homography(MisContext* ctx, const float* src_xy, const float* dst_xy, int n, double thresh, int max_iters,
                        double confidence, double H[9], uint8_t* mask, int* ok);
int mis_estimate_affine_partial(MisContext* ctx, const float* src_xy, const float* dst_xy, int n, double thresh, int max_iters,
                                double confidence, int refine_iters, double M[6], uint8_t* mask, int* ok);
int mis_leave_biggest_component(const MisMatchesInfo* pairwise, int n, float conf_threshold, int* indices, int* n_indices);
int mis_leave_biggest_component_conf(const double* confidence, int n, float conf_threshold, int* indices, int* n_indices);

typedef struct {
    double focal, aspect, ppx, ppy;
    double R[9];
    double t[3];
} MisCameraParams;
int mis_bundle_adjust_reproj(MisContext* ctx, const MisFeatures* features, const MisMatchesInfo* pairwise, int n, float conf_thresh,
                             const char* refine_mask, MisCameraParams* cameras);
int mis_wave_correct(double* rmats, int n, int kind);

int mis_warp_roi(float scale, int src_width, int src_height, const float K[9], const float R[9], MisRect* roi);
int mis_warp_roi_batch(MisContext* ctx, float scale, int src_width, int src_height, int n, const float* Ks, const float* Rs, MisRect* rois);
int mis_warp_spherical(MisContext* ctx, const MisImage* src, float scale, const float K[9], const float R[9], int interp,
                       int border, MisImage* dst, MisPoint* tl);
int mis_warp_spherical_fused(MisContext* ctx, const MisImage* src_bgr, float scale, const float K[9], const float R[9],
                             MisImage* dst_s16x3, MisImage* dst_mask, MisPoint* tl);
int mis_warp_spherical_fused_roi(MisContext* ctx, const MisImage* src_bgr, float scale, const float K[9], const float R[9],
                                 const MisRect* roi, MisImage* dst_s16x3, MisImage* dst_mask, MisPoint* tl);
int mis_warp_spherical_fused_batch(MisContext* ctx, const MisImage* srcs_u8x3, int n, float scale, const float* Ks, const float* Rs, const MisRect* rois,
                                   MisImage* dsts_s16x3, MisImage* dmasks_u8, MisPoint* tls);
int mis_warp_spherical_fused_batch_timed(MisContext* ctx, const MisImage* srcs_u8x3, int n, float scale, const float* Ks, const float* Rs,
                                         const MisRect* rois, MisImage* dsts_s16x3, MisImage* dmasks_u8, MisPoint* tls, int repeats, float* avg_us);
int mis_warp_spherical_fused_timed(MisContext* ctx, const MisImage* src_bgr, float scale, const float K[9], const float R[9],
                                   MisImage* dst_s16x3, MisImage* dst_mask, MisPoint* tl, int repeats, float* avg_us);
int mis_warper_roi(int kind, float scale, int src_width, int src_height, const float K[9], const float R[9], MisRect* roi);
int mis_warper_roi_batch(MisContext* ctx, int kind, float scale, int src_width, int src_height, int n, const float* Ks, const float* Rs,
                         MisRect* rois);
int mis_warper_warp(MisContext* ctx, int kind, const MisImage* src, float scale, const float K[9], const float R[9], int interp,
                    int border, MisImage* dst, MisPoint* tl);
int mis_warper_warp_roi(MisContext* ctx, int kind, const MisImage* src, float scale, const float K[9], const float R[9], const MisRect* roi,
                        int interp, int border, MisImage* dst, MisPoint* tl);
int mis_warper_warp_fused(MisContext* ctx, int kind, const MisImage* src_bgr, float scale, const float K[9], const float R[9],
                          MisImage* dst_s16x3, MisImage* dst_mask, MisPoint* tl);
int mis_warper_warp_fused_roi(MisContext* ctx, int kind, const MisImage* src_bgr, float scale, const float K[9], const float R[9],
                              const MisRect* roi, MisImage* dst_s16x3, MisImage* dst_mask, MisPoint* tl);
int mis_warper_warp_fused_batch(MisContext* ctx, int kind, const MisImage* srcs_u8x3, int n, float scale, const float* Ks, const float* Rs,
                                const MisRect* rois, MisImage* dsts_s16x3, MisImage* dmasks_u8, MisPoint* tls);
enum { MIS_MATH_LOG = 0, MIS_MATH_TAN = 1, MIS_MATH_SINH = 2, MIS_MATH_ASIN = 3, MIS_MATH_ATAN = 4, MIS_MATH_EXP = 5 };
int mis_debug_math_f32(MisContext* ctx_or_null, int fn, const float* in, float* out, int n);

typedef struct {
    int nfeatures, n_octave_layers;
    double contrast_threshold, edge_threshold, sigma;
} MisSiftParams;
typedef struct MisSift MisSift;
void mis_sift_default_params(MisSiftParams* p);
int mis_sift_create(MisContext* ctx, const MisSiftParams* params , int max_width, int max_height, MisSift** out);
int mis_sift_destroy(MisSift* sift);
int mis_sift_detect(MisSift* sift, const MisImage* bgr, MisFeatures* out);
int mis_sift_detect_batch(MisSift* sift, const MisImage* bgr, int n_images, MisFeatures* out);
int mis_sift_debug_level(MisSift* sift, const MisImage* bgr, int octave, int layer, int dog, float* host_out, int* width, int* height);
int mis_sift_debug_counts(MisSift* sift, unsigned* counts4);

int mis_resize_linear_exact(MisContext* ctx, const MisImage* src, int dst_w, int dst_h, double fx, double fy, MisImage* dst);
int mis_resize_linear_exact_batch(MisContext* ctx, const MisImage* srcs, int n, int dst_w, int dst_h, double fx, double fy, MisImage* dsts);
int mis_rotate(MisContext* ctx, const MisImage* src, int rotate_code, MisImage* dst);
int mis_seam_mask_apply(MisContext* ctx, const MisImage* seam_mask_warped, MisImage* mask_warped);

#define MIS_EXPOS_NO 0
#define MIS_EXPOS_GAIN 1
#define MIS_EXPOS_GAIN_BLOCKS 2
#define MIS_EXPOS_CHANNELS 3
#define MIS_EXPOS_CHANNELS_BLOCKS 4
typedef struct {
    int type;
    int nr_feeds;
    int block_width, block_height;
    int nr_gain_filtering_iterations;
} MisCompensatorParams;
typedef struct MisCompensator MisCompensator;
void mis_compensator_default_params(MisCompensatorParams* params);
int mis_compensator_create_ex(MisContext* ctx, const MisCompensatorParams* params, MisCompensator** out);
int mis_compensator_create(MisContext* ctx, int block_width, int block_height, int nr_gain_filtering_iterations, MisCompensator** out);
int mis_compensator_destroy(MisCompensator* c);
int mis_compensator_feed(MisCompensator* c, const MisPoint* corners, const MisImage* images, const MisImage* masks, int n);
int mis_compensator_gains(const MisCompensator* c, int index, double gains[3]);
int mis_compensator_gain_map(const MisCompensator* c, int index, float* map_host, int capacity, int* blocks_x, int* blocks_y);
int mis_compensator_gain_map_channels(const MisCompensator* c, int index, float* map_host, int capacity, int* blocks_x, int* blocks_y, int* channels);
int mis_compensator_apply(MisCompensator* c, int index, MisImage* image);
int mis_compensator_debug_stats(const MisCompensator* c, int i, int j, int channel, int* N, double* I_ij, double* I_ji);
int mis_seam_voronoi(MisContext* ctx, const MisPoint* corners, MisImage* masks, int n);
#define MIS_SEAM_DP_COLOR 0
int mis_seam_dp(MisContext* ctx, const MisPoint* corners, const MisImage* images, MisImage* masks, int n, int cost_func);

int mis_blend_config(int blend_type, float blend_strength, int pano_width, int pano_height, int* type_out, int* num_bands,
                     float* sharpness);
int mis_result_roi(const MisPoint* corners, const MisSize* sizes, int n, MisRect* roi);
int mis_blender_create(MisContext* ctx, int type, int num_bands, float sharpness, MisBlender** out);
int mis_blender_destroy(MisBlender* b);
int mis_blender_prepare(MisBlender* b, const MisPoint* corners, const MisSize* sizes, int n);
int mis_blender_num_bands(const MisBlender* b);
int mis_blender_feed(MisBlender* b, const MisImage* img_s16x3, const MisImage* mask_u8, MisPoint tl);
int mis_blender_feed_batch(MisBlender* b, const MisImage* imgs_s16x3, const MisImage* masks_u8, const MisPoint* tls, int n);
int mis_blender_blend(MisBlender* b, MisImage* dst_s16x3, MisImage* dst_mask);
int mis_blender_blend_columns(MisBlender* b, int x0, int x1, MisImage* dst_s16x3, MisImage* dst_mask);
typedef struct { int level, x0, y0, x1, y1; unsigned long long offset; } MisLevelRect;
int mis_blender_pack_rects(MisBlender* b, const MisLevelRect* rects, int n, void* dev_buf, size_t bytes);
int mis_blender_add_rects(MisBlender* b, const MisLevelRect* rects, int n, const void* dev_buf, size_t bytes);
int mis_blender_zero_rects(MisBlender* b, const MisLevelRect* rects, int n);
int mis_compose_frames(MisBlender* b, const MisImage* frames, int n, float scale, const float* Ks, const float* Rs, const MisRect* rois);
int mis_compose_frames_kind(MisBlender* b, int kind, const MisImage* frames, int n, float scale, const float* Ks, const float* Rs,
                            const MisRect* rois);
int mis_blender_feed_rect(const MisBlender* b, int width, int height, MisPoint tl, MisRect* tile);
int mis_blender_level_info(const MisBlender* b, int level, int* width, int* height, void** lap_dev, void** weight_dev);

#ifdef __cplusplus
}
#endif
#endif
```

Measured before the change: 3483.

## Split compose into warp and feed stages, warping right after ORB enqueue

Compose is split into a warp stage, which stages warped frames and masks in pool memory, and a feed stage that pushes them into the blender later. Under speculation, the warp is now enqueued on the compose stream as soon as the ORB batch is enqueued, fenced on a new ORB batch event. Only the feed and blend remain gated on the KNN fence. This lets warping overlap with matching instead of waiting for it, at the cost of holding the staged buffers longer and adding state checks.

```diff
diff --git a/host/job.cpp b/host/job.cpp
--- a/host/job.cpp
+++ b/host/job.cpp
@@ -22,7 +22,12 @@
     JobOutput out;
     check(cctx_, mis_context_wait(cctx_, ctx_), "mis_context_wait");
     const MisImage* work = work_frames(frames);
-    prep_.arm([this] { if (spec_ok_) prepare(everyone_); });
+    prep_.arm([this, &frames] {
+        if (!spec_ok_) return;
+        prepare(everyone_);
+        fence_features();
+        compose_warp(frames, everyone_, everyone_);
+    });
     check(ctx_, mis_orb_on_enqueued(orb_, &Hook::fire, &prep_), "mis_orb_on_enqueued");
     std::vector<MisFeatures> feats(n_);
     std::memset(feats.data(), 0, sizeof(MisFeatures) * n_);
@@ -35,7 +40,7 @@
     match_.arm([this, &frames] {
         if (!spec_ok_) return;
         fence_knn();
-        compose(frames, everyone_, everyone_);
+        compose_feed();
         finalize();
     });
     check(ctx_, mis_match_on_enqueued(ctx_, &Hook::fire, &match_), "mis_match_on_enqueued");
diff --git a/host/job_core.cpp b/host/job_core.cpp
--- a/host/job_core.cpp
+++ b/host/job_core.cpp
@@ -130,6 +130,7 @@
     }
     key_ = c;
     check(cctx_, mis_blender_prepare(blender_, corners.data(), sizes.data(), m), "mis_blender_prepare");
+    staged_ = false;
     return c;
 }
 
@@ -138,7 +139,20 @@
     if (rc < 0) check(ctx_, rc, "mis_match_knn_fence");
 }
 
+void JobCore::fence_features() { check(ctx_, mis_orb_batch_fence(orb_, cstream_), "mis_orb_batch_fence"); }
+
 void JobCore::compose(const std::vector<MisImage>& frames, const std::vector<int>& frame_ids, const std::vector<int>& idx) {
+    compose_warp(frames, frame_ids, idx);
+    compose_feed();
+}
+
+void JobCore::compose_feed() {
+    if (!staged_) return;
+    staged_ = false;
+    check(cctx_, mis_compose_feed_staged(blender_), "mis_compose_feed_staged");
+}
+
+void JobCore::compose_warp(const std::vector<MisImage>& frames, const std::vector<int>& frame_ids, const std::vector<int>& idx) {
     std::vector<MisImage> fr;
     std::vector<float> Ks, Rs;
     std::vector<MisRect> rois;
@@ -151,8 +165,9 @@
         rois.push_back(rois_[it - idx.begin()]);
     }
     if (fr.empty()) return;
-    check(cctx_, mis_compose_frames_kind(blender_, kind_, fr.data(), (int)fr.size(), warp_scale(idx), Ks.data(), Rs.data(), rois.data()),
-          "mis_compose_frames_kind");
+    check(cctx_, mis_compose_warp_kind(blender_, kind_, fr.data(), (int)fr.size(), warp_scale(idx), Ks.data(), Rs.data(), rois.data()),
+          "mis_compose_warp_kind");
+    staged_ = true;
 }
 
 MisMatchParams JobCore::reset_matches() {
diff --git a/host/job_core.hpp b/host/job_core.hpp
--- a/host/job_core.hpp
+++ b/host/job_core.hpp
@@ -43,7 +43,10 @@
     void fence_knn();
     const MisImage* work_frames(const std::vector<MisImage>& frames);
     float warp_scale(const std::vector<int>& idx) const;
+    void fence_features();
     void compose(const std::vector<MisImage>& frames, const std::vector<int>& frame_ids, const std::vector<int>& idx);
+    void compose_warp(const std::vector<MisImage>& frames, const std::vector<int>& frame_ids, const std::vector<int>& idx);
+    void compose_feed();
     MisMatchParams reset_matches();
 
     int w_, h_, n_;
@@ -66,6 +69,7 @@
     std::vector<float> Ks_, Rs_;
     std::vector<MisRect> rois_;
     std::vector<MisMatchesInfo> pairwise_;
+    bool staged_ = false;
 
 private:
     void release();
diff --git a/host/sharded_job.cpp b/host/sharded_job.cpp
--- a/host/sharded_job.cpp
+++ b/host/sharded_job.cpp
@@ -150,7 +150,12 @@
     JobOutput out;
     check(cctx_, mis_context_wait(cctx_, ctx_), "mis_context_wait");
     const MisImage* work = work_frames(frames);
-    prep_.arm([this] { if (spec_ok_) prepare_multi_band(everyone_); });
+    prep_.arm([this, &frames] {
+        if (!spec_ok_) return;
+        prepare_multi_band(everyone_);
+        fence_features();
+        compose_warp(frames, mine_, everyone_);
+    });
     check(ctx_, mis_orb_on_enqueued(orb_, &Hook::fire, &prep_), "mis_orb_on_enqueued");
     std::vector<MisFeatures> local(m);
     std::memset(local.data(), 0, sizeof(MisFeatures) * m);
@@ -180,7 +185,7 @@
     match_.arm([this, &frames] {
         if (!spec_ok_) return;
         fence_knn();
-        compose(frames, mine_, everyone_);
+        compose_feed();
     });
     check(ctx_, mis_match_on_enqueued(ctx_, &Hook::fire, &match_), "mis_match_on_enqueued");
     const int rc = mis_match_pairs_model(ctx_, feats.data(), n_, &mp, model_, nullptr, cfg_.range_width, comm_.rank(), world, pairwise_.data());
diff --git a/image_stitching_amd/_capi.py b/image_stitching_amd/_capi.py
--- a/image_stitching_amd/_capi.py
+++ b/image_stitching_amd/_capi.py
@@ -112,6 +112,7 @@
     "mis_orb_detect": (_i, [_vp, _P(MisImage), _P(MisFeatures)]),
     "mis_orb_detect_batch": (_i, [_vp, _P(MisImage), _i, _P(MisFeatures)]),
     "mis_orb_on_enqueued": (_i, [_vp, _vp, _vp]),
+    "mis_orb_batch_fence": (_i, [_vp, _vp]),
     "mis_features_download": (_i, [_vp, _P(MisFeatures), _vp, _vp]),
     "mis_features_upload": (_i, [_vp, _i, _i, _i, _vp, _vp, _i, _i, _P(MisFeatures)]),
     "mis_features_free": (_i, [_vp, _P(MisFeatures)]),
@@ -184,6 +185,8 @@
     "mis_blender_blend": (_i, [_vp, _P(MisImage), _P(MisImage)]),
     "mis_compose_frames": (_i, [_vp, _P(MisImage), _i, _f, _vp, _vp, _P(MisRect)]),
     "mis_compose_frames_kind": (_i, [_vp, _i, _P(MisImage), _i, _f, _vp, _vp, _P(MisRect)]),
+    "mis_compose_warp_kind": (_i, [_vp, _i, _P(MisImage), _i, _f, _vp, _vp, _P(MisRect)]),
+    "mis_compose_feed_staged": (_i, [_vp]),
     "mis_blender_blend_columns": (_i, [_vp, _i, _i, _P(MisImage), _P(MisImage)]),
     "mis_blender_pack_rects": (_i, [_vp, _P(MisLevelRect), _i, _vp, C.c_size_t]),
     "mis_blender_add_rects": (_i, [_vp, _P(MisLevelRect), _i, _vp, C.c_size_t]),
diff --git a/image_stitching_amd/csrc/blend.hip b/image_stitching_amd/csrc/blend.hip
--- a/image_stitching_amd/csrc/blend.hip
+++ b/image_stitching_amd/csrc/blend.hip
@@ -23,6 +23,10 @@
     bool fresh = false;
     void* scratch = nullptr;
     size_t scratch_bytes = 0;
+    bool staged = false;
+    std::vector<MisImage> st_imgs, st_msks;
+    std::vector<MisPoint> st_tls;
+    std::vector<std::pair<void*, size_t>> st_blocks;
 };
 
 namespace {
@@ -932,6 +936,12 @@
 
 inline dim3 grid2d(int w, int h) { return dim3((w + 63) / 64, (h + 3) / 4); }
 
+void drop_staged(MisBlender* b) {
+    for (auto& bl : b->st_blocks) mis_pool_free(b->ctx, bl.first, bl.second);
+    b->st_blocks.clear(); b->st_imgs.clear(); b->st_msks.clear(); b->st_tls.clear();
+    b->staged = false;
+}
+
 int release(MisBlender* b, bool free_memory) {
     MisContext* ctx = b->ctx;
     if (free_memory && b->pano_mem) {
@@ -1130,6 +1140,7 @@
 extern "C" int mis_blender_destroy(MisBlender* b) {
     if (!b) return MIS_OK;
     hipSetDevice(b->ctx->device);
+    drop_staged(b);
     release(b, true);
     if (b->scratch) { hipStreamSynchronize(b->ctx->stream); hipFree(b->scratch); }
     delete b;
@@ -1143,6 +1154,7 @@
     MisContext* ctx = b->ctx;
     MIS_CHECK(ctx, corners && sizes && n >= 1, MIS_E_INVALID, "prepare needs at least one corner/size");
     MIS_HIP(ctx, hipSetDevice(ctx->device));
+    drop_staged(b);
     int rc = release(b, false);
     if (rc != MIS_OK) return rc;
     mis_result_roi(corners, sizes, n, &b->roi);
@@ -1193,8 +1205,7 @@
     return MIS_OK;
 }
 
-extern "C" int mis_blender_feed(MisBlender* b, const MisImage* img, const MisImage* mask, MisPoint tl) {
-    if (!b) return MIS_E_INVALID;
+static int feed_one(MisBlender* b, const MisImage* img, const MisImage* mask, MisPoint tl) {
     MisContext* ctx = b->ctx;
     MIS_CHECK(ctx, b->prepared, MIS_E_STATE, "feed before prepare");
     int rc = feed_check(b, img, mask, tl);
@@ -1214,14 +1225,19 @@
     return rc;
 }
 
-extern "C" int mis_blender_feed_batch(MisBlender* b, const MisImage* imgs, const MisImage* masks, const MisPoint* tls, int n) {
+extern "C" int mis_blender_feed(MisBlender* b, const MisImage* img, const MisImage* mask, MisPoint tl) {
     if (!b) return MIS_E_INVALID;
+    MIS_CHECK(b->ctx, !b->staged, MIS_E_STATE, "feed while warped frames are staged (mis_compose_feed_staged feeds them)");
+    return feed_one(b, img, mask, tl);
+}
+
+static int feed_batch(MisBlender* b, const MisImage* imgs, const MisImage* masks, const MisPoint* tls, int n) {
     MisContext* ctx = b->ctx;
     MIS_CHECK(ctx, b->prepared, MIS_E_STATE, "feed before prepare");
     MIS_CHECK(ctx, n >= 0 && (n == 0 || (imgs && masks && tls)), MIS_E_INVALID, "null argument");
     if (n == 0) return MIS_OK;
     if (b->type != MIS_BLEND_MULTI_BAND) {
-        for (int k = 0; k < n; k++) { int rc = mis_blender_feed(b, &imgs[k], &masks[k], tls[k]); if (rc != MIS_OK) return rc; }
+        for (int k = 0; k < n; k++) { int rc = feed_one(b, &imgs[k], &masks[k], tls[k]); if (rc != MIS_OK) return rc; }
         return MIS_OK;
     }
     int rc = MIS_OK;
@@ -1233,17 +1249,22 @@
     return feed_multiband_batch(b, imgs, di.data(), dm.data(), tls, n);
 }
 
-extern "C" int mis_compose_frames_kind(MisBlender* b, int kind, const MisImage* frames, int n, float scale, const float* Ks, const float* Rs,
-                                       const MisRect* rois) {
+extern "C" int mis_blender_feed_batch(MisBlender* b, const MisImage* imgs, const MisImage* masks, const MisPoint* tls, int n) {
+    if (!b) return MIS_E_INVALID;
+    MIS_CHECK(b->ctx, !b->staged, MIS_E_STATE, "feed while warped frames are staged (mis_compose_feed_staged feeds them)");
+    return feed_batch(b, imgs, masks, tls, n);
+}
+
+extern "C" int mis_compose_warp_kind(MisBlender* b, int kind, const MisImage* frames, int n, float scale, const float* Ks, const float* Rs,
+                                     const MisRect* rois) {
     if (!b) return MIS_E_INVALID;
     MisContext* ctx = b->ctx;
     MIS_CHECK(ctx, kind >= MIS_WARP_SPHERICAL && kind <= MIS_WARP_STEREOGRAPHIC, MIS_E_UNSUPPORTED, "unknown warp kind %d", kind);
     MIS_CHECK(ctx, b->prepared, MIS_E_STATE, "compose before prepare");
+    MIS_CHECK(ctx, !b->staged, MIS_E_STATE, "compose while warped frames are staged (mis_compose_feed_staged feeds them)");
     MIS_CHECK(ctx, frames && Ks && Rs && rois && n >= 0, MIS_E_INVALID, "null argument");
     MIS_HIP(ctx, hipSetDevice(ctx->device));
-    std::vector<MisImage> imgs(n), msks(n);
-    std::vector<MisPoint> tls(n);
-    std::vector<std::pair<void*, size_t>> blocks;
+    b->st_imgs.assign(n, MisImage{}); b->st_msks.assign(n, MisImage{}); b->st_tls.assign(n, MisPoint{});
     int rc = MIS_OK;
     for (int i = 0; i < n && rc == MIS_OK; i++) {
         const MisRect& r = rois[i];
@@ -1252,14 +1273,30 @@
         const size_t ibytes = ipitch * r.height, mbytes = mpitch * r.height;
         void* blk = nullptr; size_t got = 0;
         if ((rc = mis_pool_alloc(ctx, ibytes + mbytes, &blk, &got)) != MIS_OK) break;
-        blocks.emplace_back(blk, got);
-        imgs[i] = MisImage{blk, r.width, r.height, 3, ipitch, MIS_S16, MIS_MEM_DEVICE};
-        msks[i] = MisImage{(uint8_t*)blk + ibytes, r.width, r.height, 1, mpitch, MIS_U8, MIS_MEM_DEVICE};
-    }
-    if (rc == MIS_OK && n > 0) rc = mis_warper_warp_fused_batch(ctx, kind, frames, n, scale, Ks, Rs, rois, imgs.data(), msks.data(), tls.data());
-    if (rc == MIS_OK) rc = mis_blender_feed_batch(b, imgs.data(), msks.data(), tls.data(), n);
-    for (auto& bl : blocks) mis_pool_free(ctx, bl.first, bl.second);
+        b->st_blocks.emplace_back(blk, got);
+        b->st_imgs[i] = MisImage{blk, r.width, r.height, 3, ipitch, MIS_S16, MIS_MEM_DEVICE};
+        b->st_msks[i] = MisImage{(uint8_t*)blk + ibytes, r.width, r.height, 1, mpitch, MIS_U8, MIS_MEM_DEVICE};
+    }
+    if (rc == MIS_OK && n > 0) rc = mis_warper_warp_fused_batch(ctx, kind, frames, n, scale, Ks, Rs, rois, b->st_imgs.data(), b->st_msks.data(), b->st_tls.data());
+    if (rc != MIS_OK) { drop_staged(b); return rc; }
+    b->staged = true;
+    return MIS_OK;
+}
+
+extern "C" int mis_compose_feed_staged(MisBlender* b) {
+    if (!b) return MIS_E_INVALID;
+    MisContext* ctx = b->ctx;
+    MIS_CHECK(ctx, b->staged, MIS_E_STATE, "no staged frames (mis_compose_warp_kind stages them)");
+    MIS_HIP(ctx, hipSetDevice(ctx->device));
+    const int rc = feed_batch(b, b->st_imgs.data(), b->st_msks.data(), b->st_tls.data(), (int)b->st_imgs.size());
+    drop_staged(b);
     return rc;
+}
+
+extern "C" int mis_compose_frames_kind(MisBlender* b, int kind, const MisImage* frames, int n, float scale, const float* Ks, const float* Rs,
+                                       const MisRect* rois) {
+    const int rc = mis_compose_warp_kind(b, kind, frames, n, scale, Ks, Rs, rois);
+    return rc == MIS_OK ? mis_compose_feed_staged(b) : rc;
 }
 
 extern "C" int mis_compose_frames(MisBlender* b, const MisImage* frames, int n, float scale, const float* Ks, const float* Rs, const MisRect* rois) {
@@ -1269,6 +1306,7 @@
 static int blend_columns(MisBlender* b, int x0, int x1, MisImage* dst, MisImage* dmask) {
     MisContext* ctx = b->ctx;
     MIS_CHECK(ctx, b->prepared, MIS_E_STATE, "blend before prepare");
+    MIS_CHECK(ctx, !b->staged, MIS_E_STATE, "blend while warped frames are staged (mis_compose_feed_staged feeds them)");
     x1 = std::min(x1, b->fw);
     MIS_CHECK(ctx, x0 >= 0 && x0 < x1, MIS_E_INVALID, "empty column range %d..%d (panorama width %d)", x0, x1, b->fw);
     MIS_HIP(ctx, hipSetDevice(ctx->device));
diff --git a/image_stitching_amd/csrc/orb.hip b/image_stitching_amd/csrc/orb.hip
--- a/image_stitching_amd/csrc/orb.hip
+++ b/image_stitching_amd/csrc/orb.hip
@@ -898,6 +898,8 @@
     MisContext* ctx = nullptr;
     void (*enqueued_cb)(void*) = nullptr;
     void* enqueued_user = nullptr;
+    hipEvent_t batch_ev = nullptr;
+    bool batch_recorded = false;
     MisOrbParams p;
     int max_w = 0, max_h = 0;
     int cur_w = 0, cur_h = 0;
@@ -1236,6 +1238,7 @@
     hipStreamSynchronize(o->ctx->stream);
     if (o->mem) hipFree(o->mem);
     if (o->host_counts) hipHostFree(o->host_counts);
+    if (o->batch_ev) hipEventDestroy(o->batch_ev);
     delete o;
     return MIS_OK;
 }
@@ -1273,6 +1276,9 @@
         if ((rc = enqueue_detect_group(o, &dimg[g0], imgs[0].width, imgs[0].height, &out[g0], ng)) != MIS_OK) return fail(rc);
     }
     if (trace) fprintf(stderr, "orb batch: %d frames enqueued in %.0f us\n", n, (double)std::chrono::duration_cast<std::chrono::microseconds>(std::chrono::steady_clock::now() - t_enq0).count());
+    if (!o->batch_ev) MIS_HIP(ctx, hipEventCreateWithFlags(&o->batch_ev, hipEventDisableTiming));
+    MIS_HIP(ctx, hipEventRecord(o->batch_ev, ctx->stream));
+    o->batch_recorded = true;
     if (o->enqueued_cb) {
         void (*cb)(void*) = o->enqueued_cb;
         void* user = o->enqueued_user;
@@ -1310,6 +1316,15 @@
 extern "C" int mis_orb_on_enqueued(MisOrb* o, void (*fn)(void*), void* user) {
     if (!o) return MIS_E_INVALID;
     o->enqueued_cb = fn; o->enqueued_user = user;
+    return MIS_OK;
+}
+
+extern "C" int mis_orb_batch_fence(MisOrb* o, void* stream) {
+    if (!o) return MIS_E_INVALID;
+    if (!o->batch_recorded) return MIS_OK;
+    MisContext* ctx = o->ctx;
+    MIS_HIP(ctx, hipSetDevice(ctx->device));
+    MIS_HIP(ctx, hipStreamWaitEvent((hipStream_t)stream, o->batch_ev, 0));
     return MIS_OK;
 }
 
diff --git a/image_stitching_amd/distributed.py b/image_stitching_amd/distributed.py
--- a/image_stitching_amd/distributed.py
+++ b/image_stitching_amd/distributed.py
@@ -290,6 +290,15 @@
 
     def warp_feed_many(self, frames, cams, rois):
         self.blender.compose_frames(frames, self.warper.scale, cams, rois, self.kind)
+
+    def compose_after_features(self):
+        self.finder.batch_fence(self._compose_stream_handle)
+
+    def warp_stage_many(self, frames, cams, rois):
+        self.blender.compose_warp(frames, self.warper.scale, cams, rois, self.kind)
+
+    def feed_staged(self):
+        self.blender.compose_feed_staged()
 
     def accumulators(self):
         out = []
@@ -447,12 +456,29 @@
         self._compose_indices, self._compose_rois, self._compose_cams = indices, rois, ccams
         return btype, bands
 
-    def stage_compose(self, frames, indices, prepared=None):
+    def _compose_frames(self, frames):
+        eng = self.engine
+        rois, g = self._compose_rois, self._geom
+        mine = [i for i in self.my_frames if i in rois]
+        cframes = {i: eng.resize_frame(frames[i], g.compose_scale) for i in mine} if g.size != tuple(self.frame_size) else frames
+        return mine, cframes
+
+    def stage_compose_warp(self, frames):
+        rois, ccams = self._compose_rois, self._compose_cams
+        mine, cframes = self._compose_frames(frames)
+        if not mine:
+            return False
+        self.engine.warp_stage_many([cframes[i] for i in mine], [ccams[i] for i in mine], [rois[i] for i in mine])
+        return True
+
+    def stage_compose(self, frames, indices, prepared=None, staged=False):
         eng = self.engine
         btype, bands = prepared if prepared is not None else self.stage_compose_prepare(indices)
-        rois, ccams, g = self._compose_rois, self._compose_cams, self._geom
-        mine = [i for i in self.my_frames if i in rois]
-        cframes = {i: eng.resize_frame(frames[i], g.compose_scale) for i in mine} if g.size != tuple(self.frame_size) else frames
+        if staged:
+            eng.feed_staged()
+            return btype, bands
+        rois, ccams = self._compose_rois, self._compose_cams
+        mine, cframes = self._compose_frames(frames)
         if self.seam_needed:
             marks = getattr(self, "marks", None)
             if marks is not None:
@@ -605,12 +631,12 @@
             return False
         return True
 
-    def _compose_on_side_stream(self, frames, indices, prepared=None):
+    def _compose_on_side_stream(self, frames, indices, prepared=None, staged=False):
         eng = self.engine
         if getattr(eng, "compose_stream", None) is None:
-            return self.stage_compose(frames, indices, prepared)
+            return self.stage_compose(frames, indices, prepared, staged)
         with torch.cuda.stream(eng.compose_stream):
-            return self.stage_compose(frames, indices, prepared)
+            return self.stage_compose(frames, indices, prepared, staged)
 
     def run(self, frames):
         marks = self.marks = [("start", time.perf_counter())] if os.environ.get("MIS_JOB_TRACE") else None
@@ -629,14 +655,19 @@
         if spec:
             finder = getattr(self.engine, "finder", None)
             box0 = {}
+            hooked = hasattr(finder, "on_enqueued") and len(self.my_frames) > 0
+            early_warp = hooked and not self.seam_needed and hasattr(finder, "batch_fence") and hasattr(self.engine, "warp_stage_many")
 
             def prep():
                 try:
                     with torch.cuda.stream(self.engine.compose_stream):
                         box0["p"] = self.stage_compose_prepare(list(range(self.n)))
+                        if early_warp:
+                            self.engine.compose_after_features()
+                            box0["staged"] = self.stage_compose_warp(frames)
+                            mark("compose: warps enqueued")
                 except BaseException as e:
                     box0["e"] = e
-            hooked = hasattr(finder, "on_enqueued") and len(self.my_frames) > 0
             if hooked:
                 finder.on_enqueued(prep)
             else:
@@ -650,7 +681,7 @@
                 prep()
             if "e" in box0:
                 raise box0["e"]
-            prepared = box0["p"]
+            prepared, staged = box0["p"], box0.get("staged", False)
             feats = self.stage_gather(local)
         else:
             feats = self.stage_gather(self.stage_features(frames))
@@ -669,7 +700,7 @@
                     if fence is not None:
                         self.engine.compose_after_knn(fence)
                     mark("compose: fence passed")
-                    box["r"] = self._compose_on_side_stream(frames, everyone, prepared)
+                    box["r"] = self._compose_on_side_stream(frames, everyone, prepared, staged)
                     mark("compose: enqueued")
                     if solo:
                         with torch.cuda.stream(self.engine.compose_stream):
diff --git a/image_stitching_amd/stitching.py b/image_stitching_amd/stitching.py
--- a/image_stitching_amd/stitching.py
+++ b/image_stitching_amd/stitching.py
@@ -496,16 +496,24 @@
         x, y, w, h = result_roi(corners, sizes)
         self._size = (w, h)
 
-    def compose_frames(self, frames, scale, cameras, rois, kind=capi.WARP_SPHERICAL):
+    def _compose_call(self, entry, frames, scale, cameras, rois, kind):
         n = len(frames)
-        if n == 0:
-            return
         arr = (capi.MisImage * n)(*[as_image(f) for f in frames])
         Ks = np.ascontiguousarray(np.stack([np.asarray(c["K"], np.float32).reshape(9) for c in cameras]))
         Rs = np.ascontiguousarray(np.stack([np.asarray(c["R"], np.float32).reshape(9) for c in cameras]))
         rr = (capi.MisRect * n)(*[capi.MisRect(int(r[0]), int(r[1]), int(r[2]), int(r[3])) for r in rois])
-        self.ctx.check(self.ctx.lib.mis_compose_frames_kind(self.h, int(kind), arr, n, float(scale), Ks.ctypes.data_as(C.c_void_p),
-                                                            Rs.ctypes.data_as(C.c_void_p), rr))
+        self.ctx.check(entry(self.h, int(kind), arr, n, float(scale), Ks.ctypes.data_as(C.c_void_p), Rs.ctypes.data_as(C.c_void_p), rr))
+
+    def compose_frames(self, frames, scale, cameras, rois, kind=capi.WARP_SPHERICAL):
+        if len(frames) == 0:
+            return
+        self._compose_call(self.ctx.lib.mis_compose_frames_kind, frames, scale, cameras, rois, kind)
+
+    def compose_warp(self, frames, scale, cameras, rois, kind=capi.WARP_SPHERICAL):
+        self._compose_call(self.ctx.lib.mis_compose_warp_kind, frames, scale, cameras, rois, kind)
+
+    def compose_feed_staged(self):
+        self.ctx.check(self.ctx.lib.mis_compose_feed_staged(self.h))
 
     def feed(self, img, mask, tl):
         i, m = as_image(img), as_image(mask)
@@ -669,6 +677,9 @@
         fn, self._enqueued_fn = getattr(self, "_enqueued_fn", None), None
         if fn is not None:
             fn()
+
+    def batch_fence(self, stream):
+        self.ctx.check(self.ctx.lib.mis_orb_batch_fence(self.h, C.c_void_p(getattr(stream, "value", stream))))
 
     def detect_batch(self, imgs):
         n = len(imgs)
diff --git a/include/mistitch.h b/include/mistitch.h
--- a/include/mistitch.h
+++ b/include/mistitch.h
@@ -78,6 +78,7 @@
 int mis_orb_detect(MisOrb* orb, const MisImage* bgr, MisFeatures* out);
 int mis_orb_detect_batch(MisOrb* orb, const MisImage* bgr, int n_images, MisFeatures* out);
 int mis_orb_on_enqueued(MisOrb* orb, void (*fn)(void*), void* user);
+int mis_orb_batch_fence(MisOrb* orb, void* stream);
 int mis_features_download(MisContext* ctx, const MisFeatures* f, MisKeyPoint* kps_host, void* desc_host);
 int mis_features_upload(MisContext* ctx, int img_w, int img_h, int n, const MisKeyPoint* kps_host,
                         const void* desc_host, int desc_cols, int desc_dtype, MisFeatures* out);
@@ -230,6 +231,9 @@
 int mis_compose_frames(MisBlender* b, const MisImage* frames, int n, float scale, const float* Ks, const float* Rs, const MisRect* rois);
 int mis_compose_frames_kind(MisBlender* b, int kind, const MisImage* frames, int n, float scale, const float* Ks, const float* Rs,
                             const MisRect* rois);
+int mis_compose_warp_kind(MisBlender* b, int kind, const MisImage* frames, int n, float scale, const float* Ks, const float* Rs,
+                          const MisRect* rois);
+int mis_compose_feed_staged(MisBlender* b);
 int mis_blender_feed_rect(const MisBlender* b, int width, int height, MisPoint tl, MisRect* tile);
 int mis_blender_level_info(const MisBlender* b, int level, int* width, int* height, void** lap_dev, void** weight_dev);
 
```

After: 3469. About the same (-0.4%).
